# Sangluisme/PSgradientSDF

Hardware: AMD Instinct MI355X
Metric: Gauss-Newton iterations/sec (full PS sweep), 256^3 grid x 50 frames (higher is better)
Workload: dtype f32

## Files before the change

### psgradientsdf_amd/capi.py

```python
from __future__ import annotations

import ctypes as C
import os

import numpy as np

ALBEDO, LIGHT, DIST, POSE, ALL = 1, 2, 4, 8, 15
SH1, SH2, LED = 0, 1, 2
L2, CAUCHY, HUBER, TUKEY, TRUNC_L2 = 0, 1, 2, 3, 4
R_DEPTH, R_NORMAL, R_ALBEDO, R_SHADING, R_RENDERED, R_RESIDUAL, R_VOXEL = 1, 2, 4, 8, 16, 32, 64
R_ALL = 127
_R_PLANES = [("depth", R_DEPTH, 1), ("normal", R_NORMAL, 3), ("albedo", R_ALBEDO, 3), ("shading", R_SHADING, 1),
             ("rendered", R_RENDERED, 3), ("residual", R_RESIDUAL, 3), ("voxel", R_VOXEL, 1)]

_HERE = os.path.dirname(os.path.abspath(__file__))
ENGINE_LIB = os.environ.get("PSGSDF_ENGINE_LIB") or os.path.join(_HERE, "csrc", "libpsgsdf.so")
ENGINE_LIB_DEV = os.path.join(_HERE, "csrc", "libpsgsdf_dev.so")


class GridDesc(C.Structure):
    _fields_ = [("dim", C.c_int32 * 3), ("voxel_size", C.c_float), ("shift", C.c_float * 3), ("truncation", C.c_float)]


class Settings(C.Structure):
# ... 753 lines not shown
        a = np.ascontiguousarray(values, np.float64).copy()
        self._check(self._fn("comm_allreduce_host")(self.ctx, a.ctypes.data_as(C.c_void_p), C.c_int(a.size)), "comm_allreduce_host")
        return a

    def comm_stats(self):
        n = C.c_int64()
        self._check(self._fn("comm_stats")(self.ctx, C.byref(n)), "comm_stats")
        return n.value

    def set_stream(self, stream_ptr):
        self._check(self._fn("set_stream")(self.ctx, C.c_void_p(stream_ptr)), "set_stream")

    def mg_info(self):
        out = (C.c_int32 * 12)()
        self._check(self._fn("mg_info")(self.ctx, out), "mg_info")
        return dict(zip(self._MG_INFO_NAMES, list(out)))

    _MG_INFO_NAMES = ["S", "rows", "row0", "row1", "halo", "F", "rank", "n_ranks", "need_lo", "need_hi", "z0", "z1"]

    def get_tuning(self):
        import json
        f = getattr(self._lib, self._p + "get_tuning"); f.restype = C.c_int
        n = f(self.ctx, None, C.c_size_t(0))
        if n < 0:
            self._check(n, "get_tuning")
        buf = C.create_string_buffer(n + 1)
        f(self.ctx, buf, C.c_size_t(n + 1))
        return json.loads(buf.value.decode())

    def set_profiling(self, on):
        self._check(self._fn("set_profiling")(self.ctx, C.c_int(1 if on else 0)), "set_profiling")

    def watch_kernel(self, name):
        self._check(self._fn("watch_kernel")(self.ctx, name.encode() if name else None), "watch_kernel")

    def reset_kernel_times(self):
        self._check(self._fn("reset_kernel_times")(self.ctx), "reset_kernel_times")

    def kernel_times(self):
        cap = 64
        names = (C.c_char_p * cap)(); ms = (C.c_double * cap)(); n = (C.c_int64 * cap)()
        f = getattr(self._lib, self._p + "kernel_times"); f.restype = C.c_int
        k = f(self.ctx, names, ms, n, C.c_int(cap))
        return {names[i].decode(): (ms[i], n[i]) for i in range(k)}

    def debug_dist_system(self, x=None):
        S = self.info().n_band
        diag = np.empty(S, np.float32); rhs = np.empty(S, np.float32)
        y = np.empty(S, np.float32) if x is not None else None
        xa = np.ascontiguousarray(x, np.float32) if x is not None else None
        self._check(self._fn("debug_dist_system")(self.ctx, diag.ctypes.data_as(C.c_void_p), rhs.ctypes.data_as(C.c_void_p),
                                                   xa.ctypes.data_as(C.c_void_p) if x is not None else None,
                                                   y.ctypes.data_as(C.c_void_p) if x is not None else None), "debug_dist_system")
        return diag, rhs, y

    def debug_time_pcg_pass(self, blocks=0, rows=2, ablate=0, reps=50, stamps=False):
        ms = C.c_double(0)
        st = np.zeros((max(blocks, 1), 8), np.int64) if stamps else None
        self._check(self._fn("debug_time_pcg_pass")(self.ctx, C.c_int(blocks), C.c_int(rows), C.c_int(ablate | (1024 if stamps else 0)), C.c_int(reps), C.byref(ms),
                                                     st.ctypes.data_as(C.c_void_p) if stamps else None), "debug_time_pcg_pass")
        return (ms.value, st) if stamps else ms.value

    def debug_time_pcg_solve(self, passes=16, reps=5):
        ms = C.c_double(0); shape = (C.c_int32 * 2)(); st = (C.c_double * 16)()
        self._check(self._fn("debug_time_pcg_solve")(self.ctx, C.c_int(passes), C.c_int(reps), C.byref(ms), shape, st), "debug_time_pcg_solve")
        return ms.value, (shape[0], shape[1]), [x for x in st]

    def debug_sync_stats(self):
        out = (C.c_int64 * 8)()
        self._check(self._fn("debug_sync_stats")(self.ctx, out), "debug_sync_stats")
        return dict(readbacks_checked=out[0], readbacks_late=out[1], persist_fallbacks=out[2] % 1000000, keyframes_compacted=out[2] // 1000000, speculative_starts=out[3] // 1000000, speculative_undos=out[3] % 1000000,
                    cross_rank_ready=out[4] % 10, halo_pushes=out[4] // 10, cross_rank_solves=out[5], cross_rank_mem_kind=out[6], probe_stale=out[7] // 1000000, probe_timeouts=out[7] % 1000000)

    def debug_rare_rows(self):
        r = C.c_int64(); w = C.c_int64()
        self._check(self._fn("debug_rare_rows")(self.ctx, C.byref(r), C.byref(w)), "debug_rare_rows")
        return r.value, w.value

    def debug_frame_system(self, block):
        i = self.info()
        if block == LIGHT:
            n = i.light_stride; nb = 1 if self._settings.model == LED else i.n_frames
        else:
            n = 6; nb = i.n_frames
        H = np.empty((nb, n, n), np.float64); b = np.empty((nb, n), np.float64)
        self._check(self._fn("debug_frame_system")(self.ctx, C.c_int(block), H.ctypes.data_as(C.c_void_p), b.ctypes.data_as(C.c_void_p)), "debug_frame_system")
        return H, b

    def set_frame_solver(self, mode):
        self._check(self._fn("set_frame_solver")(self.ctx, C.c_int(mode)), "set_frame_solver")

    def frame_solver_stats(self, block):
        it = C.c_int32(); err = C.c_double(); ok = C.c_int32(); ap = C.c_int32()
        self._check(self._fn("get_frame_solver_stats")(self.ctx, C.c_int(block), C.byref(it), C.byref(err), C.byref(ok), C.byref(ap)), "get_frame_solver_stats")
        return {"cg_iters": it.value, "cg_error": err.value, "cg_converged": ok.value, "applied": ap.value}

    def debug_frame_cg(self, H, b, max_it=0):
        H = np.ascontiguousarray(H, np.float32); b = np.ascontiguousarray(b, np.float32)
        nb, n = b.shape
        x = np.empty((nb, n), np.float32); it = C.c_int32(); err = C.c_double(); ok = C.c_int32()
        self._check(self._fn("debug_frame_cg")(self.ctx, C.c_int(nb), C.c_int(n), H.ctypes.data_as(C.c_void_p), b.ctypes.data_as(C.c_void_p), x.ctypes.data_as(C.c_void_p),
                                               C.c_int(max_it), C.byref(it), C.byref(err), C.byref(ok)), "debug_frame_cg")
        return x, it.value, err.value, bool(ok.value)

    def debug_albedo_system(self):
        S = self.info().n_band
        H = np.empty((S, 3), np.float32); b = np.empty((S, 3), np.float32)
        self._check(self._fn("debug_albedo_system")(self.ctx, H.ctypes.data_as(C.c_void_p), b.ctypes.data_as(C.c_void_p)), "debug_albedo_system")
        return H, b


class CommXfer(C.Structure):
    _fields_ = [("ptr_dev", C.c_void_p), ("bytes", C.c_size_t), ("peer", C.c_int)]


ALLREDUCE_FN = C.CFUNCTYPE(C.c_int, C.c_void_p, C.c_void_p, C.c_int, C.c_void_p)
SENDRECV_FN = C.CFUNCTYPE(C.c_int, C.c_void_p, C.POINTER(CommXfer), C.c_int, C.POINTER(CommXfer), C.c_int, C.c_void_p)


class CommOps(C.Structure):
    _fields_ = [("user", C.c_void_p), ("allreduce_f64", ALLREDUCE_FN), ("sendrecv", SENDRECV_FN)]


def comm_unique_id() -> bytes:
    buf = (C.c_uint8 * 128)()
    f = engine_lib().psgsdf_comm_unique_id; f.restype = C.c_int
    rc = f(buf)
    if rc != 0:
        raise PsgsdfError(f"psgsdf_comm_unique_id failed rc={rc} (librccl could not be loaded?)")
    return bytes(buf)


def grid_of(sc) -> GridDesc:
    g = GridDesc()
    g.dim[:] = [int(x) for x in sc.dim]
    g.voxel_size = float(sc.voxel_size)
    g.shift[:] = [float(x) for x in sc.shift]
    g.truncation = float(sc.truncation)
    return g


_engine_lib = {}


def engine_lib(dev: bool = False) -> C.CDLL:
    path = ENGINE_LIB_DEV if dev else ENGINE_LIB
    if path not in _engine_lib:
        if not os.path.exists(path):
            raise PsgsdfError(f"HIP engine {path} is missing: run `python -c 'import __graft_entry__ as g; g.build()'`")
        _engine_lib[path] = C.CDLL(path)
    return _engine_lib[path]


def load_engine(sc_or_grid, K, settings: Settings, device: int = 0, dev: bool = False) -> Api:
    grid = sc_or_grid if isinstance(sc_or_grid, GridDesc) else grid_of(sc_or_grid)
    return Api(engine_lib(dev or os.environ.get("PSGSDF_USE_DEV_LIB") == "1"), "psgsdf_", grid, K, settings, device)
```

### psgradientsdf_amd/csrc/api.hip

```cpp
#include "engine_internal.h"

using namespace psge;

namespace psge {
int host_stage(psgsdf_ctx* c, size_t bytes, void** p) {
    if (c->pin_bytes < bytes) {
        HIPCHK(c, hipStreamSynchronize(c->stream));
        if (c->pin_stage) hipHostFree(c->pin_stage);
        c->pin_stage = nullptr; c->pin_bytes = 0;
        const size_t want = bytes + bytes / 4;
        HIPCHK(c, hipHostMalloc(&c->pin_stage, want, hipHostMallocDefault));
        c->pin_bytes = want;
    }
    *p = c->pin_stage;
    return 0;
}
}

extern "C" {

#ifdef PSGSDF_DEV
const char* psgsdf_version(void) { return "psgsdf-hip gfx950 r5 dev (fault-injection and ablation knobs compiled in: libpsgsdf_dev.so, tests and tools only)"; }
#else
const char* psgsdf_version(void) { return "psgsdf-hip gfx950 r5"; }
#endif

static const char* const kKnobs[] = {
    "PSGSDF_PCG_POLL", "PSGSDF_SPECULATE", "PSGSDF_FOLD_IN_NEXT", "PSGSDF_FUSE_ALBEDO", "PSGSDF_FUSE_PCG_INIT", "PSGSDF_PCG_PERSIST",
    "PSGSDF_PCG_FUSE_APPLY", "PSGSDF_PCG_WINDOW", "PSGSDF_PCG_SOLVE_ROWS", "PSGSDF_PCG_COL16", "PSGSDF_PCG_ROWS", "PSGSDF_PCG_BLOCKS",
    "PSGSDF_FM_SOLVE", "PSGSDF_FRAME_SOLVE", "PSGSDF_FM_ROWS", "PSGSDF_IMG_COMPACT", "PSGSDF_XCD_MAP", "PSGSDF_XCD_STRIPE",
    "PSGSDF_XR", "PSGSDF_XF", "PSGSDF_XS", "PSGSDF_XH", "PSGSDF_XR_MEM", "PSGSDF_XWAIT_LOG2", "PSGSDF_SPECULATE_MR", "PSGSDF_CU_MASK",
    "PSGSDF_WAIT_TIMEOUT_S", "PSGSDF_DESTROY_TIMEOUT_S", "PSGSDF_SOLVE_DUMP", "PSGSDF_AO_CUT", "PSGSDF_COMPARE_CHUNK"};
static const char* const kDevKnobs[] = {"PSGSDF_PCG_ABLATE", "PSGSDF_FAULT_SOLVE", "PSGSDF_FAULT_HALO", "PSGSDF_MBOX_CHECK"};
const char* psgsdf_last_error(const psgsdf_ctx* c) { return c ? c->err : "null context"; }

int psgsdf_create(const psgsdf_grid_desc* grid, const float K[9], const psgsdf_settings* settings, int device, psgsdf_ctx** out) {
    if (!grid || !K || !settings || !out) return PSGSDF_ERR_ARG;
    if (settings->model < 0 || settings->model > 2) return PSGSDF_ERR_ARG;
    int ndev = 0;
    if (hipGetDeviceCount(&ndev) != hipSuccess || ndev <= 0 || device < 0 || device >= ndev) return PSGSDF_ERR_DEVICE;
    if (hipSetDevice(device) != hipSuccess) return PSGSDF_ERR_DEVICE;
    psgsdf_ctx* c = new psgsdf_ctx();
    c->device = device;
    if (const char* e = getenv("PSGSDF_PCG_POLL")) c->pcg_poll = atoi(e) != 0;
    if (const char* e = getenv("PSGSDF_AO_CUT")) c->ao_cut = atoi(e) != 0;
    if (const char* e = getenv("PSGSDF_COMPARE_CHUNK")) c->compare_chunk = std::min(std::max(atoll(e), 1ll), 1ll << 24);
    if (const char* e = getenv("PSGSDF_SPECULATE")) c->speculate = atoi(e) != 0;
    if (const char* e = getenv("PSGSDF_FOLD_IN_NEXT")) c->fold_in_next = atoi(e) != 0;
    if (const char* e = getenv("PSGSDF_FUSE_ALBEDO")) c->fuse_albedo = atoi(e) != 0;
    if (const char* e = getenv("PSGSDF_FUSE_PCG_INIT")) c->fuse_pcg_init = atoi(e) != 0;
    if (const char* e = getenv("PSGSDF_PCG_PERSIST")) c->pcg_persist = atoi(e) != 0;
    if (const char* e = getenv("PSGSDF_AREG_DEVICE")) c->areg_device = atoi(e) != 0;
    if (const char* e = getenv("PSGSDF_PCG_WINDOW")) c->pcg_window = atoi(e) != 0;
    if (const char* e = getenv("PSGSDF_PCG_SOLVE_ROWS")) { const int v = atoi(e); if (v > 0) c->pcg_solve_rows = v; }
    if (const char* e = getenv("PSGSDF_FM_SOLVE")) { c->fm_solve = atoi(e) != 0; c->fm_solve_led = atoi(e) == 1; }
    if (const char* e = getenv("PSGSDF_FRAME_SOLVE")) c->frame_solve = (!strcmp(e, "eigen") || !strcmp(e, "1")) ? 1 : 0;
    if (const char* e = getenv("PSGSDF_XF")) c->xf_enable = atoi(e) != 0;
    if (const char* e = getenv("PSGSDF_XS")) c->xs_enable = atoi(e) != 0;
    if (const char* e = getenv("PSGSDF_XH")) c->xh_enable = atoi(e) != 0;
    if (const char* e = getenv("PSGSDF_XWAIT_LOG2")) { const int l = atoi(e); if (l >= 8 && l <= 30) c->xwait_spins = 1 << l; }
    if (const char* e = getenv("PSGSDF_IMG_COMPACT")) c->img_compact = atoi(e) != 0;
    if (const char* e = getenv("PSGSDF_SPECULATE_MR")) c->speculate_mr = atoi(e) != 0;
    if (const char* e = getenv("PSGSDF_XCD_MAP")) c->xcd_map = atoi(e);
    if (const char* e = getenv("PSGSDF_XCD_STRIPE")) c->xcd_map = (c->xcd_map & 255) | (atoi(e) << 8);
#ifdef PSGSDF_DEV
    if (const char* e = getenv("PSGSDF_PCG_ABLATE")) c->pcg_ablate = atoi(e) & 5;
    if (const char* e = getenv("PSGSDF_MBOX_CHECK")) c->mbox_check = atoi(e) != 0;
    if (const char* e = getenv("PSGSDF_FAULT_SOLVE")) c->fault_solve = atoi(e);
    if (const char* e = getenv("PSGSDF_FAULT_HALO")) c->fault_halo = atoll(e);
#endif
    for (const char* k : kKnobs) if (const char* e = getenv(k)) c->tuning_env.emplace_back(k, e);
    for (const char* k : kDevKnobs) if (const char* e = getenv(k)) {
#ifdef PSGSDF_DEV
        c->tuning_env.emplace_back(k, e);
#else
        c->tuning_ignored.emplace_back(k, e);
#endif
    }
    if (const char* e = getenv("PSGSDF_PCG_FUSE_APPLY")) c->pcg_fuse_apply = atoi(e) != 0;
    if (hipDeviceGetAttribute(&c->num_cu, hipDeviceAttributeMultiprocessorCount, device) != hipSuccess) c->num_cu = 0;
    c->set = *settings; c->reg_n = settings->reg_weight_n; c->reg_l = settings->reg_weight_l; c->reg_r = settings->reg_weight_rho;
    GridP& g = c->grid;
    for (int a = 0; a < 3; ++a) { g.dim[a] = grid->dim[a]; c->shift[a] = grid->shift[a]; }
    g.nvox = (long long)g.dim[0] * g.dim[1] * g.dim[2]; g.koff = 0;
    for (int a = 0; a < 3; ++a) c->gdim[a] = g.dim[a];
    c->gnvox = g.nvox; c->z0 = c->zlo = 0; c->z1 = c->zhi = g.dim[2];
    g.vs = grid->voxel_size; g.vs_inv = 1.f / g.vs; g.T = grid->truncation;
    for (int a = 0; a < 3; ++a) g.origin[a] = c->shift[a] - (float)(0.5 * (double)g.vs) * (float)g.dim[a];
    c->cam.fx = K[0]; c->cam.fy = K[4]; c->cam.cx = K[2]; c->cam.cy = K[5];
    if (const char* e = getenv("PSGSDF_XR")) c->xr_enable = atoi(e) != 0;
    bool stream_ok;
    if (const char* e = getenv("PSGSDF_CU_MASK")) {
        int lo = 0, hi = 0;
        if (sscanf(e, "%d:%d", &lo, &hi) != 2 || lo < 0 || hi <= lo || hi > c->num_cu) { delete c; return PSGSDF_ERR_ARG; }
        std::vector<uint32_t> mask((size_t)(c->num_cu + 31) / 32, 0u);
        for (int i = lo; i < hi; ++i) mask[i / 32] |= 1u << (i % 32);
        stream_ok = hipExtStreamCreateWithCUMask(&c->stream, (uint32_t)mask.size(), mask.data()) == hipSuccess;
        c->cu_mask_lo = lo; c->cu_mask_hi = hi; c->num_cu = hi - lo;
    } else stream_ok = hipStreamCreate(&c->stream) == hipSuccess;
    bool ok = stream_ok
        && hipMalloc(&c->pcg_sc, sizeof(double) * (16 + 8 * (size_t)kPcgMaxBlocks)) == hipSuccess
        && hipMalloc(&c->pcg_part, sizeof(double) * 14 * kPcgMaxBlocks) == hipSuccess
        && hipMalloc(&c->pcg_gran, sizeof(double) * 2 * kSolveGranPlanes * kSolveMaxBlocksHost) == hipSuccess
        && hipMalloc(&c->mg_scal, sizeof(double) * kMgScal) == hipSuccess && hipMalloc(&c->mg_ext, sizeof(double) * 8) == hipSuccess
        && hipMalloc(&c->d_need, 2 * sizeof(int)) == hipSuccess
        && hipMalloc(&c->d_total, sizeof(int)) == hipSuccess
        && hipMalloc(&c->led_light, sizeof(float) * 3) == hipSuccess
        && hipMalloc(&c->fs_stats, sizeof(double) * 8) == hipSuccess && hipMemset(c->fs_stats, 0, sizeof(double) * 8) == hipSuccess
        && hipEventCreate(&c->ev0) == hipSuccess && hipEventCreate(&c->ev1) == hipSuccess;
    if (!ok) { delete c; return PSGSDF_ERR_DEVICE; }
    *out = c;
    return PSGSDF_OK;
}

void psgsdf_destroy(psgsdf_ctx* c) {
    if (!c) return;
    hipSetDevice(c->device);
    if (c->stream) hipStreamSynchronize(c->stream);
    double qt = 15.0; if (const char* e = getenv("PSGSDF_DESTROY_TIMEOUT_S")) qt = atof(e);
    if (xr_quiesce(c, qt)) {
        c->leak_exported = true;
        fprintf(stderr, "psgsdf: rank %d: a peer did not close its mappings of this rank's exchange memory within %.0f s (failed or still running?): that memory is leaked, not freed\n", c->rank, qt);
    }
    free_dense(c);
    hipFree(c->vis_seq); hipFree(c->frame_idx); hipFree(c->img); hipFree(c->img8); hipFree(c->frames); hipFree(c->frames_undo); hipFree(c->led_light); hipFree(c->fs_stats);
    hipFree(c->band_mem); if (!c->leak_exported) hipFree(c->rec_mem); hipFree(c->obs_mem); hipFree(c->stage);
    hipFree(c->ncache); hipFree(c->ntmp); hipFree(c->nout); hipFree(c->ndepth); hipFree(c->track_part); if (c->track_host) hipHostFree(c->track_host); hipFree(c->acc_frame); hipFree(c->frame_part); hipFree(c->frame_done); hipFree(c->part); hipFree(c->pcg_sc); hipFree(c->pcg_part); hipFree(c->pcg_gran); hipFree(c->win_tab); hipFree(c->d_total);
    for (void* p : c->xo_host) if (p) hipHostFree(p);
    if (c->pin_stage) hipHostFree(c->pin_stage);
    if (c->host_buf) hipHostFree(c->host_buf);
    if (c->mbox) hipHostFree(c->mbox);
    if (c->ev0) hipEventDestroy(c->ev0); if (c->ev1) hipEventDestroy(c->ev1);
    for (auto& pr : c->watch_pool) { hipEventDestroy(pr.first); hipEventDestroy(pr.second); }
    if (!c->leak_exported) { hipFree(c->xr); hipFree(c->hx_mem); }
    hipFree(c->xf_table); hipFree(c->vm_order);
    comm_destroy(c);
    hipFree(c->areg_mem); hipFree(c->mg_scal); hipFree(c->mg_ext); hipFree(c->mbox_shadow); hipFree(c->d_need);
    if (c->stream && c->own_stream) hipStreamDestroy(c->stream);
    delete c;
}

static double count_plane(const psgsdf_ctx* c, const float* d, const uint64_t* v, int wpv) {
    const long long plane = (long long)c->gdim[0] * c->gdim[1];
    const float lim = (float)(sqrt(3.0) * (double)c->grid.vs);
    long long m = 0;
    for (long long i = 0; i < plane; ++i) { if (!(fabsf(d[i]) <= lim)) continue; bool seen = false; for (int w = 0; w < wpv && !seen; ++w) seen = v[(size_t)i * wpv + w] != 0; m += seen; }
    return (double)m;
}
static int cut_slabs(psgsdf_ctx* c, std::vector<double>& cnt, int* z0, int* z1) {
    const int nz = c->gdim[2], n = c->n_ranks;
    if (nz < n) return fail(c, PSGSDF_ERR_UNSUPPORTED, "%d z-planes cannot be cut into %d slabs", nz, n);
    if (n > 1) {
        double* d_cnt = nullptr;
        HIPCHK(c, hipMalloc(&d_cnt, sizeof(double) * nz));
        int rc = 0;
        if (hipMemcpyAsync(d_cnt, cnt.data(), sizeof(double) * nz, hipMemcpyHostToDevice, c->stream) != hipSuccess) rc = fail(c, PSGSDF_ERR_DEVICE, "slab histogram upload");
        if (!rc) rc = comm_allreduce(c, d_cnt, nz);
        if (!rc && (hipMemcpyAsync(cnt.data(), d_cnt, sizeof(double) * nz, hipMemcpyDeviceToHost, c->stream) != hipSuccess || hipStreamSynchronize(c->stream) != hipSuccess)) rc = fail(c, PSGSDF_ERR_DEVICE, "slab histogram download");
        hipFree(d_cnt);
        if (rc) return rc;
    }
    double total = 0; for (double x : cnt) total += x;
    if (total <= 0) return fail(c, PSGSDF_ERR_UNSUPPORTED, "the volume has no band candidates to partition");
    std::vector<int> cut(n + 1, 0); cut[n] = nz;
    double run = 0; int r = 1;
    for (int k = 0; k < nz && r < n; ++k) { run += cnt[k]; while (r < n && run >= total * r / n) { cut[r] = k + 1; ++r; } }
    for (int q = 1; q < n; ++q) cut[q] = std::max(cut[q], cut[q - 1] + 1);
    for (int q = n - 1; q >= 1; --q) cut[q] = std::min(cut[q], cut[q + 1] - 1);
    *z0 = cut[c->rank]; *z1 = cut[c->rank + 1];
    return 0;
}
static int choose_slab(psgsdf_ctx* c, const float* dist, const uint64_t* vis_words, int wpv, int* z0, int* z1) {
    const int nz = c->gdim[2], n = c->n_ranks;
    const long long plane = (long long)c->gdim[0] * c->gdim[1];
    std::vector<double> cnt(nz, 0.0);
    for (int k = c->rank; k < nz; k += n) cnt[k] = count_plane(c, dist + (size_t)k * plane, vis_words + (size_t)k * plane * wpv, wpv);
    return cut_slabs(c, cnt, z0, z1);
}

static int upload_planes(psgsdf_ctx* c, int z0, int z1, size_t src_n, size_t src_off, const float* dist, const float* grad_xyz, const float* weight, const float* rgb, const uint64_t* vis_words, int words_per_voxel) {
    { int rc = set_local_grid(c, z0, z1); if (rc) return rc; }
    const long long n = c->grid.nvox;
    free_dense(c);
    if (c->vis_seq) { hipFree(c->vis_seq); c->vis_seq = nullptr; }
    int rc = alloc_dense(c, c->dense, n, 0, true); if (rc) return rc;
    HIPCHK(c, hipMalloc(&c->vis_seq, sizeof(uint64_t) * n * words_per_voxel));
    c->wpv_seq = words_per_voxel;
    HIPCHK(c, hipMemcpyAsync(c->dense.dist, dist + src_off, sizeof(float) * n, hipMemcpyHostToDevice, c->stream));
    for (int a = 0; a < 3; ++a) {
        HIPCHK(c, hipMemcpyAsync(c->dense.g[a], grad_xyz + (size_t)a * src_n + src_off, sizeof(float) * n, hipMemcpyHostToDevice, c->stream));
        HIPCHK(c, hipMemcpyAsync(c->dense.rho[a], rgb + (size_t)a * src_n + src_off, sizeof(float) * n, hipMemcpyHostToDevice, c->stream));
    }
    HIPCHK(c, hipMemcpyAsync(c->dense.weight, weight + src_off, sizeof(float) * n, hipMemcpyHostToDevice, c->stream));
    HIPCHK(c, hipMemcpyAsync(c->vis_seq, vis_words + src_off * words_per_voxel, sizeof(uint64_t) * n * words_per_voxel, hipMemcpyHostToDevice, c->stream));
    HIPCHK(c, hipStreamSynchronize(c->stream));
    c->have_volume = true; c->inited = false;
    return PSGSDF_OK;
}

int psgsdf_upload_volume(psgsdf_ctx* c, const float* dist, const float* grad_xyz, const float* weight, const float* rgb, const uint64_t* vis_words, int words_per_voxel) {
    if (!c || !dist || !grad_xyz || !weight || !rgb || !vis_words || words_per_voxel < 1) return fail(c, PSGSDF_ERR_ARG, "upload_volume: null argument");
    HIPCHK(c, hipSetDevice(c->device));
    int z0 = 0, z1 = c->gdim[2];
    if (c->n_ranks > 1) { int rc = choose_slab(c, dist, vis_words, words_per_voxel, &z0, &z1); if (rc) return rc; }
    const int zlo = std::max(0, z0 - 1);
    return upload_planes(c, z0, z1, (size_t)c->gnvox, (size_t)zlo * c->gdim[0] * c->gdim[1], dist, grad_xyz, weight, rgb, vis_words, words_per_voxel);
}

int psgsdf_slab_plane_count(psgsdf_ctx* c, const float* dist_plane, const uint64_t* vis_plane, int words_per_voxel, double* count) {
    if (!c || !dist_plane || !vis_plane || !count || words_per_voxel < 1) return fail(c, PSGSDF_ERR_ARG, "slab_plane_count: null argument");
    *count = count_plane(c, dist_plane, vis_plane, words_per_voxel);
    return PSGSDF_OK;
}
int psgsdf_plan_slab(psgsdf_ctx* c, const double* plane_counts, int* z0, int* z1) {
    if (!c || !plane_counts || !z0 || !z1) return fail(c, PSGSDF_ERR_ARG, "plan_slab: null argument");
    HIPCHK(c, hipSetDevice(c->device));
    std::vector<double> cnt(plane_counts, plane_counts + c->gdim[2]);
    return cut_slabs(c, cnt, z0, z1);
}
int psgsdf_upload_volume_slab(psgsdf_ctx* c, int z0, int z1, const float* dist, const float* grad_xyz, const float* weight, const float* rgb, const uint64_t* vis_words, int words_per_voxel) {
    if (!c || !dist || !grad_xyz || !weight || !rgb || !vis_words || words_per_voxel < 1) return fail(c, PSGSDF_ERR_ARG, "upload_volume_slab: null argument");
    if (z0 < 0 || z1 > c->gdim[2] || z1 <= z0) return fail(c, PSGSDF_ERR_ARG, "upload_volume_slab: planes [%d, %d) of %d", z0, z1, c->gdim[2]);
    HIPCHK(c, hipSetDevice(c->device));
    const int zlo = std::max(0, z0 - 1), zhi = std::min(c->gdim[2], z1 + 1);
    return upload_planes(c, z0, z1, (size_t)(zhi - zlo) * c->gdim[0] * c->gdim[1], 0, dist, grad_xyz, weight, rgb, vis_words, words_per_voxel);
}

int psgsdf_volume_init(psgsdf_ctx* c, int max_frames) {
    if (!c || max_frames < 1) return fail(c, PSGSDF_ERR_ARG, "volume_init: max_frames");
    if (c->n_ranks > 1 && c->gdim[2] < c->n_ranks) return fail(c, PSGSDF_ERR_UNSUPPORTED, "%d z-planes cannot be cut into %d slabs", c->gdim[2], c->n_ranks);
    { int rc0 = c->n_ranks > 1 ? set_local_grid(c, (int)((long long)c->rank * c->gdim[2] / c->n_ranks), (int)((long long)(c->rank + 1) * c->gdim[2] / c->n_ranks)) : set_local_grid(c, 0, c->gdim[2]); if (rc0) return rc0; }
    HIPCHK(c, hipSetDevice(c->device));
    const long long n = c->grid.nvox;
    free_dense(c);
    if (c->vis_seq) { hipFree(c->vis_seq); c->vis_seq = nullptr; }
    int rc = alloc_dense(c, c->dense, n, 0, true); if (rc) return rc;
    c->wpv_seq = (max_frames + 63) / 64;
    HIPCHK(c, hipMalloc(&c->vis_seq, sizeof(uint64_t) * n * c->wpv_seq));
    launch_fill_f32(c->dense.dist, c->grid.T, n, c->stream);
    for (int a = 0; a < 3; ++a) { HIPCHK(c, hipMemsetAsync(c->dense.g[a], 0, sizeof(float) * n, c->stream)); HIPCHK(c, hipMemsetAsync(c->dense.rho[a], 0, sizeof(float) * n, c->stream)); }
    HIPCHK(c, hipMemsetAsync(c->dense.weight, 0, sizeof(float) * n, c->stream));
    HIPCHK(c, hipMemsetAsync(c->vis_seq, 0, sizeof(uint64_t) * n * c->wpv_seq, c->stream));
    HIPCHK(c, hipStreamSynchronize(c->stream));
    c->have_volume = true; c->inited = false;
    return PSGSDF_OK;
}

int psgsdf_rebalance_slabs(psgsdf_ctx* c) {
    if (!c || !c->have_volume || !c->vis_seq) return fail(c, PSGSDF_ERR_STATE, "rebalance_slabs: volume first");
    if (c->n_ranks <= 1) return PSGSDF_OK;
    if (!c->comm) return fail(c, PSGSDF_ERR_COMM, "rank %d of %d has no communicator (psgsdf_comm_init)", c->rank, c->n_ranks);
    HIPCHK(c, hipSetDevice(c->device));
    const int R = c->n_ranks, nz = c->gdim[2], wpv = c->wpv_seq;
    const size_t plane = (size_t)c->gdim[0] * c->gdim[1];
    const int oz0 = c->z0, oz1 = c->z1, ozlo = c->zlo;
    std::vector<float> hd((size_t)(oz1 - oz0) * plane); std::vector<uint64_t> hv((size_t)(oz1 - oz0) * plane * wpv);
    HIPCHK(c, hipMemcpyAsync(hd.data(), c->dense.dist + (size_t)(oz0 - ozlo) * plane, sizeof(float) * hd.size(), hipMemcpyDeviceToHost, c->stream));
    HIPCHK(c, hipMemcpyAsync(hv.data(), c->vis_seq + (size_t)(oz0 - ozlo) * plane * wpv, sizeof(uint64_t) * hv.size(), hipMemcpyDeviceToHost, c->stream));
    HIPCHK(c, hipStreamSynchronize(c->stream));
    std::vector<double> cnt(nz, 0.0);
    for (int k = oz0; k < oz1; ++k) cnt[k] = count_plane(c, hd.data() + (size_t)(k - oz0) * plane, hv.data() + (size_t)(k - oz0) * plane * wpv, wpv);
    int nz0 = 0, nz1 = nz;
    { int rc = cut_slabs(c, cnt, &nz0, &nz1); if (rc) return rc; }
    std::vector<double> cuts((size_t)4 * R, 0.0);
    cuts[4 * c->rank] = oz0; cuts[4 * c->rank + 1] = oz1; cuts[4 * c->rank + 2] = nz0; cuts[4 * c->rank + 3] = nz1;
    { int rc = host_allreduce(c, cuts, "rebalance_slabs"); if (rc) return rc; }
    DenseView od = c->dense; uint64_t* ovis = c->vis_seq;
    const int nzlo = std::max(0, nz0 - 1), nzhi = std::min(nz, nz1 + 1);
    const long long n = (long long)(nzhi - nzlo) * (long long)plane;
    DenseView nd{};
    uint64_t* nvis = nullptr;
    auto free_new = [&] { hipFree(nd.dist); for (int a = 0; a < 3; ++a) { hipFree(nd.g[a]); hipFree(nd.rho[a]); } hipFree(nd.weight); hipFree(nd.vis); hipFree(nd.row_of); hipFree(nvis); (void)hipGetLastError(); };
    int rc = alloc_dense(c, nd, n, 0, true);
    if (!rc && hipMalloc(&nvis, sizeof(uint64_t) * n * wpv) != hipSuccess) rc = fail(c, PSGSDF_ERR_DEVICE, "rebalance_slabs: out of memory");
    if (rc) { free_new(); return rc; }
    { int rc2 = set_local_grid(c, nz0, nz1); if (rc2) { free_new(); set_local_grid(c, oz0, oz1); return rc2; } }
    c->dense = DenseView{}; c->vis_seq = nullptr;
    float* oarr[8] = {od.dist, od.g[0], od.g[1], od.g[2], od.rho[0], od.rho[1], od.rho[2], od.weight};
    float* narr[8] = {nd.dist, nd.g[0], nd.g[1], nd.g[2], nd.rho[0], nd.rho[1], nd.rho[2], nd.weight};
    std::vector<psgsdf_comm_xfer> sends, recvs;
// ... 362 lines not shown
```

### psgradientsdf_amd/csrc/api_debug.hip

```cpp
#include "engine_internal.h"

using namespace psge;

extern "C" {
int psgsdf_set_profiling(psgsdf_ctx* c, int enabled) { if (!c) return PSGSDF_ERR_ARG; c->profiling = enabled != 0; return PSGSDF_OK; }
int psgsdf_reset_kernel_times(psgsdf_ctx* c) { if (!c) return PSGSDF_ERR_ARG; c->ktimes.clear(); c->watch_used = 0; return PSGSDF_OK; }
int psgsdf_watch_kernel(psgsdf_ctx* c, const char* name) {
    if (!c) return PSGSDF_ERR_ARG;
    hipStreamSynchronize(c->stream);
    std::string w = name ? name : ""; int every = 1;
    const size_t sl = w.find('/');
    if (sl != std::string::npos) { every = std::max(1, atoi(w.c_str() + sl + 1)); w.resize(sl); }
    c->watch = w; c->watch_every = every; c->watch_seen = 0; c->watch_used = 0;
    return PSGSDF_OK;
}
int psgsdf_kernel_times(psgsdf_ctx* c, const char** names, double* ms, int64_t* launches, int cap) {
    if (!c) return 0;
    if (c->watch_used) {
        hipStreamSynchronize(c->stream);
        KTime& k = c->ktimes[c->watch];
        for (size_t i = 0; i < c->watch_used; ++i) { float t = 0; if (hipEventElapsedTime(&t, c->watch_pool[i].first, c->watch_pool[i].second) == hipSuccess) { k.ms += t; k.n += 1; } }
        c->watch_used = 0;
    }
    int n = 0;
// ... 28 lines not shown
    int G, rdef; cgf_shape(band_blocks(c), &G, &rdef);
    if (blocks > 0) G = std::min(blocks, kCgfMaxBlocks);
    if (rows <= 0) rows = rdef;
    launch_cgf_init(a, c->pcg_sc, c->pcg_part, G, c->stream);
    hipEvent_t e0, e1; HIPCHK(c, hipEventCreate(&e0)); HIPCHK(c, hipEventCreate(&e1));
    for (int q = 0; q < 3; ++q) launch_cgf_pass(a, c->pcg_sc, c->pcg_part, G, rows, q, 1 << 30, c->mbox_dev, c->stream, ablate | 16);
    HIPCHK(c, hipEventRecord(e0, c->stream));
    for (int q = 0; q < reps; ++q) launch_cgf_pass(a, c->pcg_sc, c->pcg_part, G, rows, 3 + q, 1 << 30, c->mbox_dev, c->stream, ablate | 16);
    HIPCHK(c, hipEventRecord(e1, c->stream));
    HIPCHK(c, hipStreamSynchronize(c->stream));
    float ms = 0; HIPCHK(c, hipEventElapsedTime(&ms, e0, e1));
    hipEventDestroy(e0); hipEventDestroy(e1);
    *avg_ms = (double)ms / reps;
    if (stamps) {
        HIPCHK(c, hipMemcpy(stamps, c->pcg_sc + 16, sizeof(long long) * 8 * G, hipMemcpyDeviceToHost));
    }
    return PSGSDF_OK;
}

int psgsdf_debug_time_pcg_solve(psgsdf_ctx* c, int passes, int reps, double* ms_per_launch, int32_t* shape, double* stamps ) {
    if (!c || !c->inited || !ms_per_launch || !shape || (passes < 1 && passes != -7) || reps < 1) return fail(c, PSGSDF_ERR_STATE, "init first");
    HIPCHK(c, hipSetDevice(c->device));
    int G = 0, rows = 0;
    if (!cgf_solve_shape(c, &G, &rows)) return fail(c, PSGSDF_ERR_UNSUPPORTED, "the persistent solve does not apply to this context");
    shape[0] = G; shape[1] = rows;
    SweepArgs a = make_args(c, c->reg_l != 0.f);
    a.pcg_fuse_init = 1; a.pcg_init_blocks = band_blocks(c); a.pcg_gran = c->pcg_gran; a.pcg_gran_n = 2 * kSolveGranPlanes * kSolveMaxBlocksHost; a.pcg_asm = 1;
    hipEvent_t e0, e1; HIPCHK(c, hipEventCreate(&e0)); HIPCHK(c, hipEventCreate(&e1));
    float total = 0;
    for (int r = 0; r < reps + 1; ++r) {
        launch_sweep_dist(a, c->stream);
        launch_assemble(a, c->stream);
        HIPCHK(c, hipEventRecord(e0, c->stream));
        a.pcg_epoch = ++c->pcg_solve_serial;
        launch_cgf_solve(a, c->pcg_sc, c->pcg_gran, G, rows, 1 << 30, c->mbox_dev, 0ull, passes, c->stream);
        HIPCHK(c, hipEventRecord(e1, c->stream));
        HIPCHK(c, hipStreamSynchronize(c->stream));
        float ms = 0; HIPCHK(c, hipEventElapsedTime(&ms, e0, e1));
        if (r > 0) total += ms;
        if (c->mbox[3] != 1.0) { hipEventDestroy(e0); hipEventDestroy(e1); return fail(c, PSGSDF_ERR_DEVICE, "persistent solve status %g: a workgroup gave up waiting for the others", c->mbox[3]); }
    }
    hipEventDestroy(e0); hipEventDestroy(e1);
    *ms_per_launch = (double)total / reps;
    if (stamps) for (int i = 0; i < 16; ++i) stamps[i] = c->mbox[8 + i];
    if (const char* dump = getenv("PSGSDF_SOLVE_DUMP")) {
        std::vector<double> h(8 * 256);
        HIPCHK(c, hipMemcpy(h.data(), c->pcg_sc + 16, sizeof(double) * h.size(), hipMemcpyDeviceToHost));
        if (FILE* f = fopen(dump, "w")) { for (int i = 0; i < G; ++i) fprintf(f, "%d %.0f %.0f %.0f %.0f %.0f %.0f %.0f %.0f\n", i, h[i], h[256 + i], h[512 + i], h[768 + i], h[1024 + i], h[1280 + i], h[1536 + i], h[1792 + i]); fclose(f); }
    }
    return PSGSDF_OK;
}

int psgsdf_debug_overlap_probe(psgsdf_ctx* c, int reps, double* out) {
    if (!c || !c->inited || !out || reps < 1) return fail(c, PSGSDF_ERR_STATE, "init first");
    if (c->n_ranks > 1) return fail(c, PSGSDF_ERR_UNSUPPORTED, "overlap probe: one rank");
    HIPCHK(c, hipSetDevice(c->device));
    int G = 0, rows = 0;
    if (!cgf_solve_shape(c, &G, &rows)) return fail(c, PSGSDF_ERR_UNSUPPORTED, "the persistent solve does not apply to this context");
    { int rc = flush(c); if (rc) return rc; }
    SweepArgs a = make_args(c, c->reg_l != 0.f);
    a.pcg_fuse_init = 1; a.pcg_init_blocks = band_blocks(c); a.pcg_gran = c->pcg_gran; a.pcg_gran_n = 2 * kSolveGranPlanes * kSolveMaxBlocksHost; a.pcg_asm = 1;
    SweepArgs quiet = a; quiet.pcg_gran = nullptr; quiet.pcg_gran_n = 0;
    hipStream_t s2; HIPCHK(c, hipStreamCreateWithFlags(&s2, hipStreamNonBlocking));
    hipEvent_t e[4]; for (auto& x : e) HIPCHK(c, hipEventCreate(&x));
    double acc[4] = {0, 0, 0, 0};
    int rc = PSGSDF_OK;
    auto ms = [&](hipEvent_t x, hipEvent_t y) { float t = 0; hipEventElapsedTime(&t, x, y); return (double)t; };
    auto solve = [&](hipStream_t s) { a.pcg_epoch = ++c->pcg_solve_serial; launch_cgf_solve(a, c->pcg_sc, c->pcg_gran, G, rows, 1 << 30, c->mbox_dev, 0ull, 0, s); };
    for (int r = 0; r < reps + 1 && !rc; ++r) {
        hipEventRecord(e[0], c->stream); launch_sweep_dist(a, c->stream); hipEventRecord(e[1], c->stream);
        hipStreamSynchronize(c->stream);
        hipEventRecord(e[2], c->stream); solve(c->stream); hipEventRecord(e[3], c->stream);
        hipStreamSynchronize(c->stream);
        if (c->mbox[3] != 1.0) { rc = fail(c, PSGSDF_ERR_DEVICE, "overlap probe: solve status %g", c->mbox[3]); break; }
        if (r) { acc[0] += ms(e[0], e[1]); acc[1] += ms(e[2], e[3]); }
        hipEventRecord(e[0], c->stream); launch_sweep_dist(a, c->stream); solve(c->stream); hipEventRecord(e[1], c->stream);
        hipStreamSynchronize(c->stream);
        if (r) acc[2] += ms(e[0], e[1]);
        launch_sweep_dist(a, c->stream);
        hipEventRecord(e[0], c->stream); hipStreamWaitEvent(s2, e[0], 0);
        launch_sweep_dist(quiet, c->stream); hipEventRecord(e[1], c->stream);
        solve(s2); hipEventRecord(e[2], s2);
        hipStreamSynchronize(c->stream); hipStreamSynchronize(s2);
        if (c->mbox[3] != 1.0) { rc = fail(c, PSGSDF_ERR_DEVICE, "overlap probe (side by side): solve status %g", c->mbox[3]); break; }
        if (r) acc[3] += std::max(ms(e[0], e[1]), ms(e[0], e[2]));
    }
    for (auto& x : e) hipEventDestroy(x);
    hipStreamDestroy(s2);
    for (int i = 0; i < 4; ++i) out[i] = acc[i] / reps;
    return rc;
}

int psgsdf_debug_rare_rows(psgsdf_ctx* c, int64_t* rows, int64_t* waves) {
    if (!c || !c->inited || !rows || !waves) return fail(c, PSGSDF_ERR_STATE, "init first");
    HIPCHK(c, hipSetDevice(c->device));
    SweepArgs a = make_args(c, c->reg_l != 0.f);
    launch_sweep_dist(a, c->stream);
    launch_assemble(a, c->stream);
    std::vector<int> hx(c->band.S);
    HIPCHK(c, hipMemcpyAsync(hx.data(), c->band.hx, sizeof(int) * hx.size(), hipMemcpyDeviceToHost, c->stream));
    HIPCHK(c, hipStreamSynchronize(c->stream));
    *rows = 0; *waves = 0;
    for (size_t i = 0; i < hx.size(); i += 64) { bool any = false; for (size_t k = i; k < std::min(hx.size(), i + 64); ++k) if (hx[k]) { ++*rows; any = true; } *waves += any; }
    return PSGSDF_OK;
}

int psgsdf_set_frame_solver(psgsdf_ctx* c, int mode) {
    if (!c) return PSGSDF_ERR_ARG;
    if (mode != 0 && mode != 1) return fail(c, PSGSDF_ERR_ARG, "frame solver mode %d (0 = LDL^T per frame, 1 = the reference's global float Jacobi-PCG)", mode);
    c->frame_solve = mode;
    return PSGSDF_OK;
}
int psgsdf_get_frame_solver_stats(psgsdf_ctx* c, int block, int32_t* iterations, double* error, int32_t* converged, int32_t* applied) {
    if (!c) return PSGSDF_ERR_ARG;
    if (block != PSGSDF_LIGHT && block != PSGSDF_POSE) return fail(c, PSGSDF_ERR_ARG, "block must be LIGHT or POSE");
    HIPCHK(c, hipSetDevice(c->device));
    const int kind = block == PSGSDF_POSE ? 1 : 0;
    psgsdf_step_stats st; memset(&st, 0, sizeof(st));
    if (int rc = read_frame_solver_stats(c, kind, &st)) return rc;
    if (iterations) *iterations = st.cg_iters;
    if (error) *error = st.cg_error;
    if (converged) *converged = st.cg_converged;
    if (applied) *applied = st.applied;
    return PSGSDF_OK;
}
int psgsdf_debug_frame_cg(psgsdf_ctx* c, int nb, int n, const float* H, const float* b, float* x, int max_it, int32_t* iterations, double* error, int32_t* converged) {
    if (!c || !H || !b || !x || nb <= 0) return fail(c, PSGSDF_ERR_ARG, "null argument");
    if ((n != 3 && n != 4 && n != 6 && n != 9) || (long long)nb * n > 2048) return fail(c, PSGSDF_ERR_UNSUPPORTED, "block size %d x %d blocks", n, nb);
    HIPCHK(c, hipSetDevice(c->device));
    float *dH = nullptr, *db = nullptr, *dx = nullptr; double* ds = nullptr;
    const size_t nH = (size_t)nb * n * n, nv = (size_t)nb * n;
    int rc = PSGSDF_OK;
    if (hipMalloc(&dH, sizeof(float) * nH) != hipSuccess || hipMalloc(&db, sizeof(float) * nv) != hipSuccess || hipMalloc(&dx, sizeof(float) * nv) != hipSuccess || hipMalloc(&ds, sizeof(double) * 4) != hipSuccess)
        rc = fail(c, PSGSDF_ERR_DEVICE, "out of device memory");
    double st[4] = {0, 0, 0, 0};
    if (!rc && (hipMemcpy(dH, H, sizeof(float) * nH, hipMemcpyHostToDevice) != hipSuccess || hipMemcpy(db, b, sizeof(float) * nv, hipMemcpyHostToDevice) != hipSuccess)) rc = fail(c, PSGSDF_ERR_DEVICE, "upload failed");
    if (!rc && launch_frames_eigen_raw(nb, n, dH, db, dx, ds, max_it, c->stream)) rc = fail(c, PSGSDF_ERR_UNSUPPORTED, "shape");
    if (!rc && (hipStreamSynchronize(c->stream) != hipSuccess || hipMemcpy(x, dx, sizeof(float) * nv, hipMemcpyDeviceToHost) != hipSuccess || hipMemcpy(st, ds, sizeof(st), hipMemcpyDeviceToHost) != hipSuccess))
        rc = fail(c, PSGSDF_ERR_DEVICE, "%s", hipGetErrorString(hipGetLastError()));
    hipFree(dH); hipFree(db); hipFree(dx); hipFree(ds);
    if (rc) return rc;
    if (iterations) *iterations = (int32_t)st[0];
    if (error) *error = st[1];
    if (converged) *converged = (int32_t)st[2];
    return PSGSDF_OK;
}
int psgsdf_debug_frame_system(psgsdf_ctx* c, int block, double* H, double* b) {
    if (!c || !c->inited || !H || !b) return fail(c, PSGSDF_ERR_STATE, "init first");
    HIPCHK(c, hipSetDevice(c->device));
    SweepArgs a = make_args(c, 0);
    const bool led = c->set.model == PSGSDF_LED;
    int n, nb, nh;
    int launched = 0;
    if (block == PSGSDF_LIGHT) { launched = launch_sweep_light(a, c->stream); n = led ? 3 : (c->set.model == PSGSDF_SH2 ? 9 : 4); nb = led ? 1 : c->F; nh = led ? 3 : n * (n + 1) / 2; }
    else if (block == PSGSDF_POSE) { launched = launch_sweep_pose(a, c->stream); n = 6; nb = c->F; nh = 21; }
    else return fail(c, PSGSDF_ERR_ARG, "block must be LIGHT or POSE");
    if (!launched) HIPCHK(c, hipMemsetAsync(c->acc_frame, 0, sizeof(double) * c->acc_frame_n, c->stream));
    std::vector<double> acc(c->acc_frame_n);
    HIPCHK(c, hipMemcpyAsync(acc.data(), c->acc_frame, sizeof(double) * c->acc_frame_n, hipMemcpyDeviceToHost, c->stream));
    HIPCHK(c, hipStreamSynchronize(c->stream));
    if (led && block == PSGSDF_LIGHT) {
        for (int i = 0; i < 9; ++i) H[i] = 0;
        for (int i = 0; i < 3; ++i) { b[i] = 0; for (int f = 0; f < c->F; ++f) { H[i * 3 + i] += acc[(size_t)f * kFrameRow + i]; b[i] += acc[(size_t)f * kFrameRow + 3 + i]; } }
        return PSGSDF_OK;
    }
    for (int k = 0; k < nb; ++k) {
        const double* A = acc.data() + (size_t)k * kFrameRow;
        double* Hk = H + (size_t)k * n * n; double* bk = b + (size_t)k * n;
        for (int i = 0; i < n * n; ++i) Hk[i] = 0;
        int q = 0;
        for (int i = 0; i < n; ++i) for (int j = i; j < n; ++j) { Hk[i * n + j] = A[q]; Hk[j * n + i] = A[q]; ++q; }
        for (int i = 0; i < n; ++i) bk[i] = A[nh + i];
    }
    return PSGSDF_OK;
}

int psgsdf_debug_albedo_system(psgsdf_ctx* c, float* H, float* b) {
    if (!c || !c->inited || !H || !b) return fail(c, PSGSDF_ERR_STATE, "init first");
    HIPCHK(c, hipSetDevice(c->device));
    SweepArgs a = make_args(c, 0);
    launch_sweep_albedo(a, c->stream);
    const int S = c->band.S, Sp = c->band.Spad;
    std::vector<float> h(3 * (size_t)Sp), bb(3 * (size_t)Sp);
    HIPCHK(c, hipMemcpyAsync(h.data(), c->band.aH, sizeof(float) * 3 * Sp, hipMemcpyDeviceToHost, c->stream));
    HIPCHK(c, hipMemcpyAsync(bb.data(), c->band.ab, sizeof(float) * 3 * Sp, hipMemcpyDeviceToHost, c->stream));
    HIPCHK(c, hipStreamSynchronize(c->stream));
    for (int j = 0; j < S; ++j) for (int ch = 0; ch < 3; ++ch) { H[3 * j + ch] = h[(size_t)ch * Sp + j]; b[3 * j + ch] = bb[(size_t)ch * Sp + j]; }
    return PSGSDF_OK;
}

int psgsdf_debug_sync_stats(psgsdf_ctx* c, int64_t out[8]) {
    if (!c || !out) return PSGSDF_ERR_ARG;
    out[0] = c->mbox_checked; out[1] = c->mbox_late; out[2] = c->persist_fallbacks + (c->img_compacted ? 1000000LL : 0); out[3] = c->spec_windows * 1000000LL + c->spec_undos;
    out[4] = (c->xr_ready ? 1 : 0) + 10 * c->n_halo_pushes; out[5] = c->xr_solves; out[6] = c->xr_mem_kind; out[7] = c->xr_probe_stale * 1000000LL + c->xr_probe_timeouts;
    return PSGSDF_OK;
}

int psgsdf_get_tuning(psgsdf_ctx* c, char* json, size_t cap) {
    if (!c) return PSGSDF_ERR_ARG;
    std::string o = "{\"build\": \"";
    o += psgsdf_version(); o += "\", \"env\": {";
    auto esc = [](const std::string& v) { std::string r; for (char ch : v) { if (ch == '"' || ch == '\\') r += '\\'; if ((unsigned char)ch >= 0x20) r += ch; } return r; };
    bool first = true;
    for (auto& kv : c->tuning_env) { o += (first ? "\"" : ", \"") + kv.first + "\": \"" + esc(kv.second) + "\""; first = false; }
    o += "}, \"ignored_dev_only\": {"; first = true;
    for (auto& kv : c->tuning_ignored) { o += (first ? "\"" : ", \"") + kv.first + "\": \"" + esc(kv.second) + "\""; first = false; }
    o += "}, \"effective\": {";
    char buf[1024];
    snprintf(buf, sizeof(buf), "\"pcg_poll\": %d, \"speculate\": %d, \"speculate_mr\": %d, \"fold_in_next\": %d, \"fuse_albedo\": %d, \"fuse_pcg_init\": %d, \"pcg_persist\": %d, "
             "\"pcg_fuse_apply\": %d, \"fm_solve\": %d, \"fm_solve_led\": %d, \"frame_solve\": \"%s\", \"img_compact\": %d, \"xcd_map\": %d, "
             "\"xr\": %d, \"xf\": %d, \"xs\": %d, \"xh\": %d, \"xr_mem_kind\": %d, \"xwait_log2\": %d, \"cu_mask\": [%d, %d], \"mbox_check\": %d, \"pcg_ablate\": %d, \"fault_solve\": %d, \"fault_halo\": %lld, \"ao_cut\": %d, \"compare_chunk\": %lld",
             (int)c->pcg_poll, (int)c->speculate, (int)c->speculate_mr, (int)c->fold_in_next, (int)c->fuse_albedo, (int)c->fuse_pcg_init, (int)c->pcg_persist,
             (int)c->pcg_fuse_apply, (int)c->fm_solve, (int)c->fm_solve_led, c->frame_solve == 1 ? "eigen" : "ldlt", (int)c->img_compact, c->xcd_map,
             (int)c->xr_enable, (int)c->xf_enable, (int)c->xs_enable, (int)c->xh_enable, c->xr_mem_kind, (int)lround(log2((double)c->xwait_spins)), c->cu_mask_lo, c->cu_mask_hi,
             (int)c->mbox_check, c->pcg_ablate, c->fault_solve, c->fault_halo, (int)c->ao_cut, c->compare_chunk);
    o += buf;
    {
        int Gs = 0, Rs = 0;
        const bool shape = cgf_solve_shape(c, &Gs, &Rs);
        const int budget = (shape && c->n_ranks <= 1) ? cgf_solve_window_budget(Rs) : 0;
        const char* why = !c->pcg_window ? "" : c->n_ranks > 1 ? "multi-rank" : c->pcg_ablate ? "timing ablation" : !c->inited ? "no band yet"
                          : !shape ? "no persistent solve on this band" : (c->win_G != Gs || c->win_rows != Rs) ? "no table for this partition" : c->win_max > budget ? "window does not fit" : "";
        snprintf(buf, sizeof(buf), ", \"pcg_window\": %d, \"pcg_solve_rows\": %d, \"solve_window\": {\"workgroups\": %d, \"rows_per_workgroup\": %d, \"window_doubles\": %d, \"budget_doubles\": %d, \"fits\": %d, \"fallback\": \"%s\", \"last_solve_windowed\": %d}",
                 (int)c->pcg_window, c->pcg_solve_rows, shape ? Gs : 0, shape ? Rs : 0, c->win_max, budget, (int)(c->pcg_window && !*why), why, c->last_solve_windowed);
        o += buf;
    }
    o += "}";
    snprintf(buf, sizeof(buf), ", \"last_compare\": {\"queries\": [%lld, %lld], \"pairs\": [%lld, %lld]}", c->cmp_queries[0], c->cmp_queries[1], c->cmp_pairs[0], c->cmp_pairs[1]);
    o += buf;
    snprintf(buf, sizeof(buf), ", \"last_align\": {\"iterations\": %lld, \"evaluations\": %lld, \"queries\": [%lld, %lld], \"pairs\": [%lld, %lld]}", c->aln_iters, c->aln_evals, c->aln_queries[0], c->aln_queries[1],
             c->aln_pairs[0], c->aln_pairs[1]);
    o += buf;
    if (c->n_ranks > 1) {
        snprintf(buf, sizeof(buf), ", \"xr_probe\": {\"rank\": %d, \"n_ranks\": %d, \"kind_chosen\": %d, \"stale_mappings\": %lld, \"fine_grained\": {\"tried\": %lld, \"stale_records_from_lower\": %lld, \"expired_waits_lower\": %lld, \"expired_waits_upper\": %lld}, "
                 "\"uncached\": {\"tried\": %lld, \"stale_records_from_lower\": %lld, \"expired_waits_lower\": %lld, \"expired_waits_upper\": %lld}}",
                 c->rank, c->n_ranks, c->xr_mem_kind, c->xr_stale_maps, c->xr_probe_local[1][3], c->xr_probe_local[1][0], c->xr_probe_local[1][1], c->xr_probe_local[1][2],
                 c->xr_probe_local[2][3], c->xr_probe_local[2][0], c->xr_probe_local[2][1], c->xr_probe_local[2][2]);
        o += buf;
    }
    o += "}";
    if (json && cap) { const size_t n = std::min(cap - 1, o.size()); memcpy(json, o.data(), n); json[n] = 0; }
    return (int)o.size();
}

}
```

### psgradientsdf_amd/csrc/device_common.h

```cpp
#pragma once
#include "engine.h"
#include <float.h>

#ifndef PSG_STRICT
#define PSG_STRICT 0
#endif
#if PSG_STRICT & 1
#pragma clang fp contract(off)
#else
#pragma clang fp contract(fast)
#endif

namespace psg {
#if PSG_STRICT & 8
typedef double obs_acc_t;
#else
typedef float obs_acc_t;
#endif

typedef float f2_t __attribute__((ext_vector_type(2)));
__device__ __forceinline__ float dot3(const float* a, const float* b) { return (a[0] * b[0] + a[1] * b[1]) + a[2] * b[2]; }
__device__ __forceinline__ float norm3(const float* a) { return sqrtf(dot3(a, a)); }
__device__ __forceinline__ void normalized3(const float* v, float* o) {
#pragma clang fp contract(off)
// ... 37 lines not shown
            else hipLaunchKernelGGL((K<2, -1, -1>), grid, block, shmem, stream, __VA_ARGS__); \
        } } while (0)
template <int LOSS = -1>
__device__ __forceinline__ float robust_weight(const Robust& rb, float r) {
#if PSG_STRICT & 2
    switch (LOSS >= 0 ? LOSS : rb.loss) {
        case 1: { float x = r / rb.lambda; return 1.0f / (1.0f + x * x); }
        case 3: { float x = r / rb.lambda; float w = (1.0f - x * x); w = w * w; return (r * r < rb.lambda_sq) ? w : 0.0f; }
        case 2: { float w = rb.lambda * fabsf(1.0f / r); return (r * r < rb.lambda_sq) ? 1.0f : w; }
        case 4: return (r * r < rb.lambda_sq) ? 1.0f : 0.0f;
        default: return 1.0f;
    }
#endif
    switch (LOSS >= 0 ? LOSS : rb.loss) {
        case 1: { float x = r * rb.inv_lambda; return __builtin_amdgcn_rcpf(1.0f + x * x); }
        case 3: { float x = r * rb.inv_lambda; float w = (1.0f - x * x); w = w * w; return (r * r < rb.lambda_sq) ? w : 0.0f; }
        case 2: { float w = rb.lambda * fabsf(__builtin_amdgcn_rcpf(r)); return (r * r < rb.lambda_sq) ? 1.0f : w; }
        case 4: return (r * r < rb.lambda_sq) ? 1.0f : 0.0f;
        default: return 1.0f;
    }
}
template <int LOSS = -1>
__device__ __forceinline__ float robust_loss(const Robust& rb, float r) {
#if PSG_STRICT & 2
    switch (LOSS >= 0 ? LOSS : rb.loss) {
        case 1: { float x = r / rb.lambda; return logf(1.0f + x * x); }
        case 3: { float x = r / rb.lambda; float u = 1.0f - x * x; float v = 1.0f - u * u * u; return (r * r < rb.lambda_sq) ? v : 1.0f; }
        case 2: return (r * r < rb.lambda_sq) ? 0.5f * (r * r) : rb.lambda * (fabsf(r) - 0.5f * rb.lambda * 1.0f);
        case 4: { float x = fminf(fmaxf(r, -rb.lambda), rb.lambda); return x * x; }
        default: return r * r;
    }
#endif
    switch (LOSS >= 0 ? LOSS : rb.loss) {
        case 1: { float x = r * rb.inv_lambda; return __builtin_amdgcn_logf(1.0f + x * x) * 0.693147180559945f; }
        case 3: { float x = r * rb.inv_lambda; float u = 1.0f - x * x; float v = 1.0f - u * u * u; return (r * r < rb.lambda_sq) ? v : 1.0f; }
        case 2: return (r * r < rb.lambda_sq) ? 0.5f * (r * r) : rb.lambda * (fabsf(r) - 0.5f * rb.lambda * 1.0f);
        case 4: { float x = fminf(fmaxf(r, -rb.lambda), rb.lambda); return x * x; }
        default: return r * r;
    }
}

constexpr int kCgfSums = 7;
__device__ __forceinline__ double* fpart(double* part, int k, int kind) { return part + ((size_t)((k & 1) * kCgfSums + kind)) * kPcgMaxBlocks; }

template <int CTRL, int ROW_MASK>
__device__ __forceinline__ double dpp_add(double v) {
    const int lo = __builtin_amdgcn_update_dpp(0, __double2loint(v), CTRL, ROW_MASK, 0xf, false);
    const int hi = __builtin_amdgcn_update_dpp(0, __double2hiint(v), CTRL, ROW_MASK, 0xf, false);
    return v + __hiloint2double(hi, lo);
}
__device__ __forceinline__ double wave_sum(double v) {
    v = dpp_add<0xB1, 0xf>(v);
    v = dpp_add<0x4E, 0xf>(v);
    v = dpp_add<0x141, 0xf>(v);
    v = dpp_add<0x140, 0xf>(v);
    v = dpp_add<0x142, 0xa>(v);
    v = dpp_add<0x143, 0xc>(v);
    return __hiloint2double(__builtin_amdgcn_readlane(__double2hiint(v), 63), __builtin_amdgcn_readlane(__double2loint(v), 63));
}
template <int CTRL>
__device__ __forceinline__ double dpp_get(double v) {
    const int lo = __builtin_amdgcn_update_dpp(0, __double2loint(v), CTRL, 0xf, 0xf, false);
    const int hi = __builtin_amdgcn_update_dpp(0, __double2hiint(v), CTRL, 0xf, 0xf, false);
    return __hiloint2double(hi, lo);
}
__device__ __forceinline__ void wave_sum8(const double (&v)[8], double& t0, double& t1) {
    const int lane = threadIdx.x & 63;
    const bool b0 = lane & 1, b1 = lane & 2;
    double u[4], t[2];
#pragma unroll
    for (int j = 0; j < 4; ++j) { const double keep = b0 ? v[4 + j] : v[j], give = b0 ? v[j] : v[4 + j]; u[j] = keep + dpp_get<0xB1>(give); }
#pragma unroll
    for (int j = 0; j < 2; ++j) { const double keep = b1 ? u[2 + j] : u[j], give = b1 ? u[j] : u[2 + j]; t[j] = keep + dpp_get<0x4E>(give); }
#pragma unroll
    for (int j = 0; j < 2; ++j) {
        t[j] += dpp_get<0x124>(t[j]);
        t[j] += dpp_get<0x128>(t[j]);
        t[j] += __shfl_xor(t[j], 16, 64);
        t[j] += __shfl_xor(t[j], 32, 64);
    }
    t0 = t[0]; t1 = t[1];
}
__device__ __forceinline__ double wave_sum4(const double (&v)[4]) {
    const int lane = threadIdx.x & 63;
    const bool b0 = lane & 1, b1 = lane & 2;
    double u[2];
#pragma unroll
    for (int j = 0; j < 2; ++j) { const double keep = b0 ? v[2 + j] : v[j], give = b0 ? v[j] : v[2 + j]; u[j] = keep + dpp_get<0xB1>(give); }
    const double keep = b1 ? u[1] : u[0], give = b1 ? u[0] : u[1];
    double t = keep + dpp_get<0x4E>(give);
    t += dpp_get<0x124>(t);
    t += dpp_get<0x128>(t);
    t += __shfl_xor(t, 16, 64);
    t += __shfl_xor(t, 32, 64);
    return t;
}
template <int NW>
__device__ __forceinline__ void wave_sum4_store(double t, double* red, int w) {
    const int lane = threadIdx.x & 63;
    if (lane < 4) red[(2 * (lane & 1) + ((lane >> 1) & 1)) * NW + w] = t;
}
template <int NW>
__device__ __forceinline__ void wave_sum8_store(double t0, double t1, double* red, int w) {
    const int lane = threadIdx.x & 63;
    if (lane < 4) { const int base = 4 * (lane & 1) + (lane & 2); red[base * NW + w] = t0; red[(base + 1) * NW + w] = t1; }
}
template <int NV, class T>
__device__ __forceinline__ void wave_sums_to(const T* acc, double* row) {
    const int lane = threadIdx.x & 63;
#pragma unroll
    for (int g = 0; g < (NV + 7) / 8; ++g) {
        double v[8];
#pragma unroll
        for (int q = 0; q < 8; ++q) v[q] = 8 * g + q < NV ? (double)acc[8 * g + q] : 0.0;
        double t0, t1; wave_sum8(v, t0, t1);
        const int k = 8 * g + 4 * (lane & 1) + (lane & 2);
        if (lane < 4) { if (k < NV) row[k] = t0; if (k + 1 < NV) row[k + 1] = t1; }
    }
}
__device__ __forceinline__ float wave_sumf(float v) {
#pragma unroll
    for (int o = 32; o > 0; o >>= 1) v += __shfl_down(v, o, 64);
    return v;
}
__device__ __forceinline__ void block_part_store(double v, double* part_slot, double* red, int bid = -1) {
    v = wave_sum(v);
    int lane = threadIdx.x & 63, w = threadIdx.x >> 6;
    __syncthreads();
    if (lane == 0) red[w] = v;
    __syncthreads();
    if (threadIdx.x == 0) {
        double s = 0;
        for (int i = 0; i < (int)(blockDim.x >> 6); ++i) s += red[i];
        part_slot[bid >= 0 ? bid : (int)blockIdx.x] = s;
    }
}
template <int NT = 0>
__device__ __forceinline__ double block_total(const double* part, int n, double* red) {
    double v = 0;
    if (!NT || threadIdx.x < NT) for (int i = threadIdx.x; i < n; i += NT ? NT : blockDim.x) v += part[i];
    v = wave_sum(v);
    int lane = threadIdx.x & 63, w = threadIdx.x >> 6;
    __syncthreads();
    if (lane == 0 && (!NT || w < NT / 64)) red[w] = v;
    __syncthreads();
    double s = 0;
    for (int i = 0; i < (int)((NT ? NT : blockDim.x) >> 6); ++i) s += red[i];
    return s;
}
__device__ __forceinline__ unsigned xcd_remap(unsigned pid, unsigned G) {
    const unsigned x = pid & 7u, s = pid >> 3, q = G >> 3, rem = G & 7u;
    return x * q + (x < rem ? x : rem) + s;
}
__device__ __forceinline__ void fm_ids(const SweepArgs& a, int& cx, int& f) {
    cx = blockIdx.x; f = blockIdx.y;
    if (a.xcd_map & 1) {
        const unsigned L = xcd_remap(blockIdx.x + gridDim.x * blockIdx.y, gridDim.x * gridDim.y);
        cx = (int)(L / gridDim.y); f = (int)(L - (unsigned)cx * gridDim.y);
    }
}
__device__ __forceinline__ unsigned xcd_remap_striped(unsigned pid, unsigned G, unsigned T) {
    const unsigned Gc = G / (8u * T) * (8u * T);
    if (pid >= Gc) return pid;
    const unsigned x = pid & 7u, s = pid >> 3;
    return ((s / T) * 8u + x) * T + s % T;
}
__device__ __forceinline__ int vm_bid(const SweepArgs& a, int bit = 2, bool per_obs = false) {
    if (bit == 4 && (a.xcd_map & 32) && a.vm_order) return a.vm_order[blockIdx.x];
    if (per_obs && (a.xcd_map & 64) && a.vm_order) return a.vm_order[blockIdx.x];
    if (!(a.xcd_map & bit)) return (int)blockIdx.x;
    const unsigned T = (unsigned)a.xcd_map >> 8;
    return T ? (int)xcd_remap_striped(blockIdx.x, gridDim.x, T) : (int)xcd_remap(blockIdx.x, gridDim.x);
}
#define PART(a, slot) ((a).acc.part + (size_t)(slot) * (a).acc.PB)
__device__ __forceinline__ void mbox_put(double* out, int n, int i, double v, unsigned long long key) {
    out[i] = v;
    if (key) reinterpret_cast<unsigned long long*>(out)[n + i] = (unsigned long long)__double_as_longlong(v) ^ (key + (unsigned long long)i);
}
__device__ __forceinline__ void mbox_commit(unsigned long long key) { if (key) __threadfence_system(); }
__device__ __forceinline__ void store8_system(double* p, double v) { asm volatile("global_store_dwordx2 %0, %1, off sc0 sc1\n\ts_nop 1" :: "v"(p), "v"(v) : "memory"); }
__device__ __forceinline__ void fold_exchange(const XfTable* xf, long long epoch, int n, double* t) {
    const XfTable& x = *xf;
    const int Rk = x.n_ranks, buf = (int)(epoch & 1), lane = (int)(threadIdx.x & 63);
    const double tag = (double)epoch;
    const long long slot = (long long)buf * Rk + x.rank;
    double* const mine = x.region[x.rank];
    for (int s = 0; s < n; ++s) t[s] = __shfl(t[s], 0, 64);
    if (lane == 0) {
        for (int r = 0; r < Rk; ++r) for (int s = 0; s < n; ++s) store8_system(x.region[r] + x.spay + slot * 8 + s, t[s]);
        asm volatile("s_waitcnt vmcnt(0)" ::: "memory");
        for (int r = 0; r < Rk; ++r) __hip_atomic_store(x.region[r] + x.sflg + slot, tag, __ATOMIC_RELAXED, __HIP_MEMORY_SCOPE_SYSTEM);
    }
    bool late = false;
    if (lane < Rk) {
        int spins = 0;
        while (__hip_atomic_load(mine + x.sflg + (long long)buf * Rk + lane, __ATOMIC_RELAXED, __HIP_MEMORY_SCOPE_SYSTEM) != tag) { __builtin_amdgcn_s_sleep(2); if (++spins > x.spin_max) { late = true; break; } }
    }
    const bool any_late = __builtin_amdgcn_ballot_w64(late) != 0ull;
    __builtin_amdgcn_fence(__ATOMIC_ACQUIRE, "");
    for (int s = 0; s < n; ++s) {
        const double v = lane < Rk ? __hip_atomic_load(mine + x.spay + ((long long)buf * Rk + lane) * 8 + s, __ATOMIC_RELAXED, __HIP_MEMORY_SCOPE_SYSTEM) : 0.0;
        double tot = 0.0;
        for (int r = 0; r < Rk; ++r) tot += __shfl(v, r, 64);
        t[s] = any_late ? __builtin_nan("") : tot;
    }
    if (any_late && lane == 0) __hip_atomic_store(mine + kXrLate + 1, tag, __ATOMIC_RELAXED, __HIP_MEMORY_SCOPE_SYSTEM);
}
template <int NT = 0>
__device__ __forceinline__ void fold_pending(const SweepArgs& a, double* red ) {
    if (a.fold.n == 0 || blockIdx.x != 0 || blockIdx.y != 0) return;
    double t[4];
    for (int s = 0; s < a.fold.n; ++s) t[s] = block_total<NT>(PART(a, a.fold.id[s]), a.fold.nblk, red);
    if (threadIdx.x < 64) {
        if (a.fold.xf) fold_exchange(a.fold.xf, a.fold.xf_epoch, a.fold.n, t);
        if (threadIdx.x == 0) {
            for (int s = 0; s < a.fold.n; ++s) mbox_put(a.fold.out, a.fold.n, s, t[s], a.fold.key);
            mbox_commit(a.fold.key);
        }
    }
    __syncthreads();
}

extern __shared__ __align__(16) unsigned char psg_dyn_smem[];
__device__ __forceinline__ const FrameP& frame_at(const FrameP* sf, int f) {
    return *reinterpret_cast<const FrameP*>(reinterpret_cast<const char*>(sf) + __umul24((unsigned)f, (unsigned)sizeof(FrameP)));
}
__device__ __forceinline__ void load_frames(FrameP* sf, const FrameP* frames, int F) {
    const float* src = (const float*)frames; float* dst = (float*)sf;
    for (int i = threadIdx.x; i < F * (int)(sizeof(FrameP) / 4); i += blockDim.x) dst[i] = src[i];
    __syncthreads();
}

struct Proj { float p[3]; float m, n, z_inv; bool ok; };
__device__ __forceinline__ float div_by(float a, float b, float y) { const float q0 = a * y; return __builtin_fmaf(__builtin_fmaf(-q0, b, a), y, q0); }
struct ProjJ { float mj, nj; bool ok; };
__device__ __forceinline__ ProjJ project_jac(const Proj& pr, const Cam& cam) {
#pragma clang fp contract(off)
    ProjJ o;
    o.mj = div_by(cam.fx * pr.p[0], pr.p[2], pr.z_inv) + cam.cx;
    o.nj = div_by(cam.fy * pr.p[1], pr.p[2], pr.z_inv) + cam.cy;
    o.ok = (o.mj >= 0.f && o.mj < (float)cam.W && o.nj >= 0.f && o.nj < (float)cam.H);
    return o;
}

__device__ __forceinline__ Proj project(const float* xs, const FrameP& fp, const Cam& cam) {
#pragma clang fp contract(off)
    Proj o;
    float tmp[3] = {xs[0] - fp.t[0], xs[1] - fp.t[1], xs[2] - fp.t[2]};
#pragma unroll
    for (int i = 0; i < 3; ++i) o.p[i] = (fp.R[0 * 3 + i] * tmp[0] + fp.R[1 * 3 + i] * tmp[1]) + fp.R[2 * 3 + i] * tmp[2];
#if PSG_STRICT & 4
    const float z_inv = (float)(1.0 / (double)o.p[2]);
#else
    const float z_inv = 1.0f / o.p[2];
#endif
    o.z_inv = z_inv;
    o.m = cam.fx * o.p[0] * z_inv + cam.cx;
    o.n = cam.fy * o.p[1] * z_inv + cam.cy;
    o.ok = (o.m >= 0.f && o.m < (float)cam.W && o.n >= 0.f && o.n < (float)cam.H);
    return o;
}

__device__ __forceinline__ const float* pix(const float* img, const Cam& cam, int row, int col) {
    row = row < 0 ? 0 : (row >= cam.H ? cam.H - 1 : row);
    col = col < 0 ? 0 : (col >= cam.W ? cam.W - 1 : col);
    return img + ((size_t)row * cam.W + col) * 3;
}

template <bool GRAD>
__device__ __forceinline__ void interp_taps(const float* a00, const float* a01, const float* a10, const float* a11, float fm, float fn, float gm, float gn, float* I, float* gu, float* gv,
                                            float m = 0.f, float n = 0.f, int x = 0, int y = 0) {
#if PSG_STRICT & 4
    {
#pragma clang fp contract(off)
        const double w1 = ((double)y + 1.0 - (double)n) * (double)(m - (float)x);
        const double w2 = ((double)y + 1.0 - (double)n) * ((double)x + 1.0 - (double)m);
        const float w3 = (n - (float)y) * (m - (float)x);
        const double w4 = (double)(n - (float)y) * ((double)x + 1.0 - (double)m);
#pragma unroll
        for (int ch = 0; ch < 3; ++ch) {
            const float t1 = (float)((double)a10[ch] * w1), t2 = (float)((double)a00[ch] * w2), t3 = a11[ch] * w3, t4 = (float)((double)a01[ch] * w4);
            I[ch] = ((t1 + t2) + t3) + t4;
        }
    }
#else
    const float w1 = (1.0f - fn) * fm, w2 = (1.0f - fn) * (1.0f - fm), w3 = fn * fm, w4 = fn * (1.0f - fm);
#pragma unroll
    for (int ch = 0; ch < 3; ++ch) I[ch] = ((a10[ch] * w1 + a00[ch] * w2) + a11[ch] * w3) + a01[ch] * w4;
#endif
    if (GRAD) {
        const float w01 = gm, w11 = gn, w00 = 1.0f - gm, w10 = 1.0f - gn;
#pragma unroll
        for (int ch = 0; ch < 3; ++ch) {
            gu[ch] = w00 * (a01[ch] - a00[ch]) + w01 * (a11[ch] - a10[ch]);
            gv[ch] = w10 * (a10[ch] - a00[ch]) + w11 * (a11[ch] - a01[ch]);
        }
    }
}
template <bool GRAD, class TEX>
__device__ __forceinline__ void sample_border(const TEX& tex, const Cam& cam, int x, int y, float m, float n, float* I, float* gu, float* gv) {
    float p[3]; tex(x, y, p);
    I[0] = p[0]; I[1] = p[1]; I[2] = p[2];
    if (GRAD) {
        float w01 = m - (float)x, w11 = n - (float)y;
        float w00 = (float)(1.0 - (double)w01), w10 = (float)(1.0 - (double)w11);
        float q_y1[3], q_ym[3], q_x1ym[3], q_x1[3], q_xm[3], q_xmy1[3];
        tex(x, y + 1, q_y1); tex(x, y - 1, q_ym); tex(x + 1, y - 1, q_x1ym); tex(x + 1, y, q_x1); tex(x - 1, y, q_xm); tex(x - 1, y + 1, q_xmy1);
#pragma unroll
        for (int ch = 0; ch < 3; ++ch) {
            if ((x + 1) >= cam.H) gu[ch] = q_y1[ch] - p[ch];
            else { float v0 = -q_ym[ch] + p[ch]; float v1 = -q_x1ym[ch] + q_x1[ch]; gu[ch] = w00 * v0 + w01 * v1; }
            if ((x + 1) >= cam.H && (y + 1) < cam.W) { float v0 = -q_xm[ch] + p[ch]; float v1 = -q_xmy1[ch] + q_y1[ch]; gv[ch] = w10 * v0 + w11 * v1; }
// ... 338 lines not shown
```

### psgradientsdf_amd/csrc/engine.h

```cpp
#pragma once
#include <hip/hip_runtime.h>
#include <stdint.h>

namespace psg {

constexpr int kBlock = 256;
constexpr int kMaxFramesLds = 640;
constexpr int kNQ = 19;
constexpr int kNQCommon = 13;
constexpr int kMaxBasis = 9;

struct FrameP {
    float R[9];
    float t[3];
    float l[9];
    float pad[3];
};

struct Cam { float fx, fy, cx, cy; int W, H; };

struct GridP {
    int dim[3];
    long long nvox;
    float vs, vs_inv;
    float origin[3];
    float T;
    int koff;
};

struct Robust { int loss; float lambda, lambda_sq, inv_lambda; };

struct Band {
    int S, Spad, KW;
    int* lin;
    float* dist;
    float* g[3];
    float* rho[3];
    uint64_t* vis;
    int* nb;
    int* dirb;
    float* nbd;
    int* col;
    unsigned* colp;
    int col16;
    int reach;
    float* gfd[3];
    float4* vp[3];
    float* aH; float* ab;
    float* blk;
    float* H;
    int* hx;
    float* rhs; float* x; float* t;
    float4* rec[2];
    int* obs_ptr;
    int* obs_rows;
    int obs_max;
    long long obs_ptr_total;
};

struct Accum {
    double* frame;
    double* part;
    int PB;
    double* fpart;
    int fcap;
    int* fdone;
};
constexpr int kFrameRow = 64;
constexpr int kPcgMaxBlocks = 2048;
constexpr int kCgfMaxBlocks = 768;

enum { SC_ENERGY = 0, SC_NOBS = 1, SC_EN = 2, SC_EL = 3, SC_ACCEPT = 4, SC_AUX0 = 5, SC_AUX1 = 6, SC_AUX2 = 7, SC_COUNT = 8 };

struct AlbedoReg {
    int* anb;
    int* back;
    float* anrho;
    float* J;
    float* res;
    float* rhs; float* diag; float* diag0; float* x; float* r; float* p; float* q; float* t;
    double* cgs;
    float weight;
};

struct XfTable;
struct FoldReq { int n; int id[4]; int nblk; double* out; unsigned long long key; const XfTable* xf; long long xf_epoch; };

struct ImgSrc {
    const float* f32;
    const unsigned* u8; float scale;
    bool idx32;
};

struct SweepArgs {
    Band b;
    const FrameP* frames;
    ImgSrc im;
    int F;
    Cam cam;
    GridP grid;
    Robust rob;
    Accum acc;
    int model;
    int quirks;
    float reg_n, reg_l;
    int normal_reg, laplacian_reg;
    float damping;
    int row0, row1;
    FoldReq fold;
    AlbedoReg ar;
    double* pcg_part; double* pcg_fs;
    int pcg_asm;
    unsigned pcg_epoch;
    int pcg_ablate;
    int pcg_apply;
    double* pcg_gran; int pcg_gran_n;
    const int* pcg_win;
    int pcg_win_G, pcg_win_rows, pcg_win_max;
    int pcg_fuse_init;
    int pcg_init_blocks;
    int fuse_apply;
    const int* vm_order;
    float* fm_led_light;
    const XfTable* xf;
    long long xf_epoch;
    int xcd_map;
    int fm_solve;
    FrameP* fm_frames; float* fm_undo; double* fm_e_out; unsigned long long fm_e_key;
    const double* gate;
    const double* ext;
};

constexpr int kXrMaxRanks = 32;
constexpr int kXrRankGran = 0, kXrAbort = 2 * 8 * kXrMaxRanks, kXrDoubles = kXrAbort + 8;
constexpr int kXrLate = kXrAbort + 1;
constexpr int kXrNonce = kXrAbort + 7;
struct XrArgs {
    int rank, n_ranks;
    double* region[kXrMaxRanks];
    float4* lo_rec[2]; float4* hi_rec[2];
    float4* lo_base[2];
    int give_lo, give_hi;
    int need_lo, need_hi;
    unsigned epoch;
};
struct XfTable {
    int n_ranks, rank, F, spin_max;
    long long pay, flg;
    long long spay, sflg;
    double* region[32];
};
constexpr int kHxWords = 16;
constexpr unsigned kXrEpochMask = 0x3fffu;

constexpr int kTryPackFlags = 2048;
void launch_normals_cache(int W, int H, int r, double fx_inv, double fy_inv, double cx, double cy, double* work , float* out , hipStream_t s);
void launch_try_pack_f32(const float* rgb, unsigned* rgba, size_t npix, size_t stride, float scale, int* fail , hipStream_t s);
void launch_pack_rgb8(const uint8_t* rgb, unsigned* rgba, size_t npix, hipStream_t s);
void launch_select_vis(const uint64_t* vis_seq, int wpv_seq, uint64_t* vis_key, int KW, const int* frame_idx, int F, long long nvox, hipStream_t s);
void launch_band_flags(const float* dist, const uint64_t* vis_key, int KW, float vs, long long nvox, int* flags, hipStream_t s);
void launch_band_scan(int* flags_inout_rowof, long long nvox, int* block_sums, int* d_total, hipStream_t s);
struct DenseView { float* dist; float* g[3]; float* weight; float* rho[3]; uint64_t* vis; int KW; int* row_of; };
void launch_band_fill(const DenseView& d, const GridP& grid, Band b, int* d_reach, hipStream_t s);
void launch_band_scatter(const DenseView& d, Band b, hipStream_t s);
void launch_derive(const SweepArgs& a, int update_grad, hipStream_t s);
constexpr int kObsChunk = 2048;
void launch_obs_count(const Band& b, int F, int row0, int row1, int* counts, hipStream_t s);
void launch_block_work(const Band& b, int row0, int row1, int* work, hipStream_t s);
void launch_obs_fill(const Band& b, int F, int row0, int row1, const int* offsets, hipStream_t s);
void launch_lower_bound(const int* lin, int S, int target, int* out, hipStream_t s);
struct SlotList { int n; int id[8]; };
void launch_sum_parts(const double* part, int PB, int nblk, const SlotList& slots, double* out, unsigned long long key, hipStream_t s, const XfTable* xf = nullptr, long long xf_epoch = 0);
void launch_frame_cols(const double* frame, int F, int col, double* out, unsigned long long key, hipStream_t s);
void launch_zero_f64(double* p, int n, hipStream_t s);
struct CopySegs { int n; unsigned off[16]; unsigned len[16]; unsigned long long key[16]; };
void launch_copy_segs(const double* src, double* dst, const CopySegs& segs, hipStream_t s);
void launch_marker(double* p, double v, hipStream_t s);
void launch_init_albedo(const SweepArgs& a, hipStream_t s);
void launch_led_light_init(const SweepArgs& a, hipStream_t s);
void launch_energy(const SweepArgs& a, hipStream_t s);
void launch_sweep_albedo(const SweepArgs& a, hipStream_t s);
void launch_apply_albedo(const SweepArgs& a, hipStream_t s);
void launch_restore_albedo(const SweepArgs& a, hipStream_t s);
int launch_sweep_light(const SweepArgs& a, hipStream_t s);
int launch_sweep_pose(const SweepArgs& a, hipStream_t s);
void launch_solve_light(const SweepArgs& a, FrameP* frames, float* led_light, double* e_out, unsigned long long e_key, float* undo, hipStream_t s);
void launch_restore_light(int F, FrameP* frames, float* led_light, const float* undo, hipStream_t s);
void launch_solve_pose(const SweepArgs& a, FrameP* frames, double* e_out, unsigned long long e_key, hipStream_t s);
bool frames_eigen_fits(int model, int F);
void launch_frames_eigen_light(const SweepArgs& a, FrameP* frames, float* led_light, double* e_out, unsigned long long e_key, float* undo, double* stats, hipStream_t s);
void launch_frames_eigen_pose(const SweepArgs& a, FrameP* frames, double* e_out, unsigned long long e_key, double* stats, hipStream_t s);
int launch_frames_eigen_raw(int nb, int n, const float* H, const float* b, float* x, double* stats, int max_it, hipStream_t s);
void launch_sweep_dist(const SweepArgs& a, hipStream_t s);
void launch_assemble(const SweepArgs& a, hipStream_t s);
void launch_cgf_init(const SweepArgs& a, double* fs, double* part, int G, hipStream_t s);
void launch_cgf_pass(const SweepArgs& a, double* fs, double* part, int G, int rows, int k, int kmax, double* mb, hipStream_t s, int ablate = 0);
void launch_cgf_sum(double* part, int G, int k, double* out, hipStream_t s);
constexpr int kSolveGranPlanes = 8;
constexpr int kSolveThreadsHost = 512, kSolveMaxBlocksHost = 256, kSolveMaxRowsHost = 4, kSolveMbSlots = 24;
int cgf_solve_max_blocks(int rows);
void launch_solve_windows(const Band& b, int row0, int row1, int G, int rows_per_wg, int* tab , int* max_total, hipStream_t s);
int cgf_solve_window_budget(int rows_per_wg);
int launch_cgf_solve(const SweepArgs& a, double* fs, double* gran, int G, int rows_per_wg, int kmax, double* mb, unsigned long long mb_key, int force_passes, hipStream_t s, const XrArgs* xr = nullptr);
void launch_areg_tables(const DenseView& d, const GridP& g, const SweepArgs& a, hipStream_t s);
void launch_areg_build(const SweepArgs& a, hipStream_t s);
void launch_areg_system(const SweepArgs& a, hipStream_t s);
void launch_areg_jx(const SweepArgs& a, const float* p, float* t, hipStream_t s);
void launch_areg_jt(const SweepArgs& a, const float* p, const float* t, float* q, hipStream_t s);
void launch_areg_cg_init(const SweepArgs& a, hipStream_t s);
void launch_areg_cg_iteration(const SweepArgs& a, int i, int nblk, float thr, hipStream_t s);
void launch_areg_cg_update(const SweepArgs& a, float alpha, hipStream_t s);
void launch_areg_cg_dir(const SweepArgs& a, float beta, hipStream_t s);
void launch_apply_albedo_delta(const SweepArgs& a, const float* delta, hipStream_t s);
void launch_matvec(const SweepArgs& a, const float* x, float* y, hipStream_t s);
void launch_apply_dist(const SweepArgs& a, hipStream_t s);
void launch_upsample(const DenseView& src, const DenseView& dst, const GridP& g_old, hipStream_t s);
void launch_fill_f32(float* p, float v, long long n, hipStream_t s);
void launch_normals(const float* depth, const float* cache, int W, int H, int r, double* tmp, float* out, hipStream_t s);
void launch_track(const DenseView& d, const GridP& g, const Cam& cam, const FrameP& fp, const float* depth, float z_min, float z_max, double* part, int nblk, int gdimz, int zown0, int zown1, hipStream_t s);
void launch_integrate(const DenseView& d, uint64_t* vis_seq, int wpv_seq, const GridP& g, const Cam& cam, const FrameP& fp,
                      const float* rgb, const float* depth, const float* normals, int counter, float z_min, float z_max, hipStream_t s);

constexpr int kRenderBrick = 8;
constexpr int kRenderTile = 8;
constexpr int kRenderStats = 9;
enum { RP_DEPTH = 0, RP_NORMAL, RP_ALBEDO, RP_SHADING, RP_RENDERED, RP_RESIDUAL, RP_VOXEL, RP_COUNT };
enum { RF_DEPTH = 0, RF_NORMAL = 1, RF_ALBEDO = 4, RF_SHADING = 7, RF_RENDERED = 8, RF_VOXEL = 11, RF_OFF_BAND = 12, RF_COUNT = 13 };
struct RenderArgs {
    DenseView d;
    const float4* vp[3];
    GridP grid;
    const FrameP* frames;
    ImgSrc im; int img_w, img_h;
    Robust rob;
    const unsigned char* bricks;
    const int* bbox;
    int nb[3];
    Cam cam;
    int frame;
    int light_frame;
    FrameP pose;
    int tiles_x, tiles_y;
    float* planes[RP_COUNT];
    double* part;
    int zr[2];
    int slab;
    int f0;
    double* mask;
    unsigned char* mine;
    double* rec;
    long long rec_px;
    int rf[RF_COUNT];
    int n_rf;
};
void launch_render_bricks(const DenseView& d, const GridP& g, float thr, int z0, int z1, unsigned char* bricks, int* bbox, double* marks, hipStream_t s);
void launch_render_box(const double* marks, const int* nb, unsigned char* bricks, int* bbox, hipStream_t s);
void launch_render(const RenderArgs& a, int model, hipStream_t s);
void launch_render_report(const RenderArgs& a, int model, int F, hipStream_t s);
void launch_render_fold(const double* part, int tiles, int F, double* out , hipStream_t s);
void launch_render_ranks(const RenderArgs& a, int model, bool report, int chunk, hipStream_t s);
void launch_render_keep(const RenderArgs& a, hipStream_t s);
void launch_render_composite(const RenderArgs& a, bool report, int chunk, hipStream_t s);

struct WMeshGrid {
    const float* dist; const float* weight; const float* g[3]; const float* rho[3];
    const float* hg[3]; const float* hrho[3];
    int nx, ny, zlo, zh;
    int lo[3], d[3];
    int zc0;
    long long nown;
    float voxel[3], origin[3];
    int poff[3];
};
void launch_wmesh_mark(const WMeshGrid& g, long long ncell, int* cnt, int* flag, hipStream_t s);
void launch_wmesh_or(int* dst, const int* src, long long n, hipStream_t s);
void launch_wmesh_faces(const WMeshGrid& g, long long ncell, const int* offs, int n_faces, const int* num, int first, const int* num_up, int first_up, int* faces, hipStream_t s);
void launch_wmesh_verts(const WMeshGrid& g, const int* num, int n_verts, float* xyz, float* nrm, unsigned char* rgb, hipStream_t s);

void launch_band_fit(const SweepArgs& a, int* n_obs, double* loss, float* sum_r2, hipStream_t s);
void launch_wmesh_fit(const WMeshGrid& g, const int* num, int n_verts, const int* row_of, int row0, int row1, const int* n_obs, const double* loss, const float* sum_r2,
                      int* v_n, float* v_rms, float* v_loss, hipStream_t s);

enum { MC_FIRST = 0, MC_VERTS, MC_FACES, MC_EDGES, MC_BOUNDARY, MC_NONMANIFOLD, MC_AREA, kMcompStats = 8 };
void launch_mcomp_init(int* parent, int nv, hipStream_t s);
void launch_mcomp_hook(const int* faces, int nf, int* parent, hipStream_t s);
void launch_mcomp_flatten(int* parent, int nv, int* flag, hipStream_t s);
void launch_mcomp_vstats(const int* parent, const int* num, int nv, const float* xyz, int* vcomp, long long* stat, unsigned* blo, unsigned* bhi, hipStream_t s);
void launch_mcomp_fstats(const int* faces, int nf, const int* vcomp, const float* xyz, double vs2 , long long* stat, hipStream_t s);
void launch_mcomp_edges(const int* faces, int nf, unsigned long long* keys, int* uses, unsigned long long cap, hipStream_t s);
void launch_mcomp_ecount(const unsigned long long* keys, const int* uses, unsigned long long cap, const int* vcomp, long long* stat, hipStream_t s);
void launch_mcomp_keep(const int* kept, const int* vcomp, int nv, const int* faces, int nf, int* vflag, int* fflag, hipStream_t s);
void launch_mcomp_compact(const int* kept, const int* vcomp, int nv, const int* faces, int nf, const int* vnum, const int* fnum, const float* xyz, const float* nrm,
                          const unsigned char* rgb, float* oxyz, float* onrm, unsigned char* orgb, int* ovcomp, int* ofaces, hipStream_t s);


}
```

### psgradientsdf_amd/csrc/engine.hip

```cpp
#include "engine_internal.h"
#include <chrono>
#include <sched.h>

namespace psge {

int wait_mapped(psgsdf_ctx* c, const std::function<bool()>& ready, const char* what) {
    using clk = std::chrono::steady_clock;
    static const double limit_s = [] { const char* e = getenv("PSGSDF_WAIT_TIMEOUT_S"); double v = e ? atof(e) : 0.0; return v > 0.0 ? v : 120.0; }();
    clk::time_point t0{}, next_query{};
    bool timing = false;
    for (unsigned spin = 1;; ++spin) {
        if (ready()) return 0;
        if (spin & 0x3ffu) continue;
        const clk::time_point now = clk::now();
        if (!timing) { timing = true; t0 = now; next_query = now + std::chrono::milliseconds(20); continue; }
        if (now - t0 > std::chrono::milliseconds(2)) sched_yield();
        if (now < next_query) continue;
        next_query = now + std::chrono::milliseconds(20);
        const hipError_t q = hipStreamQuery(c->stream);
        if (q == hipSuccess) return ready() ? 0 : 1;
        if (q != hipErrorNotReady) return fail(c, PSGSDF_ERR_DEVICE, "%s: stream error while waiting: %s", what, hipGetErrorString(q));
        if (std::chrono::duration<double>(now - t0).count() > limit_s)
            return fail(c, PSGSDF_ERR_DEVICE, "%s: nothing published within %.0f s (PSGSDF_WAIT_TIMEOUT_S)", what, limit_s);
    }
// ... 152 lines not shown
    const long long ep = xs ? ++c->xs_epoch : 0;
    if (n <= 4 && c->fold_in_next) {
        c->pending_fold.n = n; for (int i = 0; i < n; ++i) c->pending_fold.id[i] = slots[i];
        c->pending_fold.nblk = band_blocks(c); c->pending_fold.out = dst; c->pending_fold.key = dkey; c->pending_fold.xf = xf; c->pending_fold.xf_epoch = ep;
    } else {
        SlotList sl; sl.n = n; for (int i = 0; i < n; ++i) sl.id[i] = slots[i];
        launch_sum_parts(c->part, c->PB, band_blocks(c), sl, dst, dkey, c->stream, xf, ep);
    }
    if (xs) c->deferred.push_back({c->mbox + off, n, key, [c, consume](const double* v) { if (std::isnan(v[0])) c->xf_timeout = true; consume(v); }});
    else c->deferred.push_back({c->mbox + off, n, key, std::move(consume)});
    return 0;
}
int read_frame_energy_deferred(psgsdf_ctx* c, int col_e, std::function<void(double, double)> consume) {
    size_t off; unsigned long long key;
    { int rc = mbox_reserve(c, 2, &off, &key); if (rc) return rc; }
    launch_frame_cols(c->acc_frame, c->F, col_e, c->mbox_dev + off, key, c->stream);
    c->deferred.push_back({c->mbox + off, 2, key, [consume](const double* v) { consume(v[0], v[1]); }});
    return 0;
}
int reserve_frame_energy_deferred(psgsdf_ctx* c, std::function<void(double, double)> consume, double** dev_slot, unsigned long long* key_out) {
    size_t off; unsigned long long key;
    { int rc = mbox_reserve(c, 2, &off, &key); if (rc) return rc; }
    *dev_slot = c->mbox_dev + off; *key_out = key;
    c->deferred.push_back({c->mbox + off, 2, key, [consume](const double* v) { consume(v[0], v[1]); }});
    return 0;
}
int ensure_host_buf(psgsdf_ctx* c, size_t n) {
    if (n <= c->host_buf_n) return 0;
    if (c->host_buf) hipHostFree(c->host_buf);
    c->host_buf = nullptr; c->host_buf_n = 0;
    HIPCHK(c, hipHostMalloc(&c->host_buf, sizeof(double) * n));
    c->host_buf_n = n;
    return 0;
}

void free_dense(psgsdf_ctx* c) {
    hipFree(c->dense.dist); for (int a = 0; a < 3; ++a) { hipFree(c->dense.g[a]); hipFree(c->dense.rho[a]); }
    hipFree(c->dense.weight); hipFree(c->dense.vis); hipFree(c->dense.row_of); hipFree(c->block_sums);
    c->dense = DenseView{}; c->block_sums = nullptr;
}
int alloc_dense(psgsdf_ctx* c, DenseView& d, long long nvox, int KW, bool with_rowof) {
    HIPCHK(c, hipMalloc(&d.dist, sizeof(float) * nvox));
    for (int a = 0; a < 3; ++a) { HIPCHK(c, hipMalloc(&d.g[a], sizeof(float) * nvox)); HIPCHK(c, hipMalloc(&d.rho[a], sizeof(float) * nvox)); }
    HIPCHK(c, hipMalloc(&d.weight, sizeof(float) * nvox));
    d.KW = KW;
    if (KW > 0) HIPCHK(c, hipMalloc(&d.vis, sizeof(uint64_t) * nvox * KW));
    if (with_rowof) HIPCHK(c, hipMalloc(&d.row_of, sizeof(int) * nvox));
    return 0;
}

int build_band(psgsdf_ctx* c) {
    if (!c->deferred.empty() || c->pending_fold.n) { int rc = flush(c); if (rc) return rc; }
    if (xr_quiesce(c, 120.0)) return fail(c, PSGSDF_ERR_COMM, "band rebuild: a rank never closed its mappings of this rank's record planes (lost or failed peer?)");
    if (c->n_ranks > 1 && c->comm) { int rc = xr_probe(c); if (rc) return rc; }
    c->persist_off = false;
    const long long nvox = c->grid.nvox;
    const int KW = c->dense.KW;
    if (!c->block_sums) HIPCHK(c, hipMalloc(&c->block_sums, sizeof(int) * ((nvox + 1023) / 1024 + 1)));
    timed(c, "band_flags", [&] { launch_band_flags(c->dense.dist, c->dense.vis, KW, c->grid.vs, nvox, c->dense.row_of, c->stream); });
    timed(c, "band_scan", [&] { launch_band_scan(c->dense.row_of, nvox, c->block_sums, c->d_total, c->stream); });
    int S = 0;
    HIPCHK(c, hipMemcpyAsync(&S, c->d_total, sizeof(int), hipMemcpyDeviceToHost, c->stream));
    HIPCHK(c, hipStreamSynchronize(c->stream));
    const int Spad = ((S + kBlock - 1) / kBlock) * kBlock + kBlock;
    const size_t n4 = 1 + 1 + 3 + 3 + 6 + 6 + kNQ + 12 + 6 + 14 + kNQ + 4 + 9 + 1 + 3;
    const size_t bytes = (n4 * 4 + (size_t)KW * 8) * Spad + 256;
    if (c->band_mem) { hipFree(c->band_mem); c->band_mem = nullptr; }
    if (c->rec_mem) { hipFree(c->rec_mem); c->rec_mem = nullptr; }
    HIPCHK(c, hipMalloc(&c->band_mem, bytes));
    HIPCHK(c, hipMemsetAsync(c->band_mem, 0, bytes, c->stream));
    { int rc = xr_alloc(c, &c->rec_mem, 2 * sizeof(float4) * (size_t)Spad, false); if (rc) return rc; }
    HIPCHK(c, hipMemsetAsync(c->rec_mem, 0, 2 * sizeof(float4) * (size_t)Spad, c->stream));
    c->band_bytes = bytes;
    char* p = (char*)c->band_mem;
    auto take = [&](size_t elems, size_t esz) { void* r = p; p += elems * esz * Spad; return r; };
    Band& b = c->band;
    b.S = S; b.Spad = Spad; b.KW = KW;
    b.vis = (uint64_t*)take(KW, 8);
    b.rec[0] = (float4*)c->rec_mem; b.rec[1] = b.rec[0] + Spad;
    b.lin = (int*)take(1, 4);
    b.dist = (float*)take(1, 4);
    for (int a = 0; a < 3; ++a) b.g[a] = (float*)take(1, 4);
    for (int a = 0; a < 3; ++a) b.rho[a] = (float*)take(1, 4);
    b.nb = (int*)take(6, 4); b.nbd = (float*)take(6, 4); b.col = (int*)take(kNQ, 4); b.colp = (unsigned*)take(9, 4); b.dirb = (int*)take(1, 4);
    for (int a = 0; a < 3; ++a) b.gfd[a] = (float*)take(1, 4);
    for (int a = 0; a < 3; ++a) b.vp[a] = (float4*)take(4, 4);
    b.aH = (float*)take(3, 4); b.ab = (float*)take(3, 4);
    b.blk = (float*)take(14, 4); b.H = (float*)take(kNQ, 4);
    b.hx = (int*)take(1, 4);
    b.rhs = (float*)take(1, 4); b.x = (float*)take(1, 4); b.t = (float*)take(1, 4);
    if ((size_t)(p - (char*)c->band_mem) > bytes) return fail(c, PSGSDF_ERR_DEVICE, "band arena overrun: %zu > %zu bytes", (size_t)(p - (char*)c->band_mem), bytes);
    HIPCHK(c, hipMemsetAsync(c->d_total, 0, sizeof(int), c->stream));
    timed(c, "band_fill", [&] { launch_band_fill(c->dense, c->grid, b, c->d_total, c->stream); });
    {
        int reach = 0;
        HIPCHK(c, hipMemcpyAsync(&reach, c->d_total, sizeof(int), hipMemcpyDeviceToHost, c->stream));
        HIPCHK(c, hipStreamSynchronize(c->stream));
        b.col16 = reach <= 32767; b.reach = reach;
        if (const char* e = getenv("PSGSDF_PCG_COL16")) if (atoi(e) == 0) b.col16 = 0;
    }
    {
        c->row0 = 0; c->row1 = S;
        c->halo = 0; c->need[0] = c->need[1] = 0; c->give[0] = c->give[1] = 0; c->halo_active = false;
        if (c->n_ranks > 1 && !c->comm) return fail(c, PSGSDF_ERR_COMM, "rank %d of %d has no communicator (psgsdf_comm_init)", c->rank, c->n_ranks);
        if (3 * c->n_ranks > kMgScal) return fail(c, PSGSDF_ERR_UNSUPPORTED, "at most %d ranks", kMgScal / 3);
        if (c->n_ranks > 1) {
            const long long plane = (long long)c->grid.dim[0] * c->grid.dim[1];
            int rr[2] = {0, S};
            if (S > 0) {
                launch_lower_bound(b.lin, S, (int)((c->z0 - c->zlo) * plane), c->d_need, c->stream);
                launch_lower_bound(b.lin, S, (int)((c->z1 - c->zlo) * plane), c->d_need + 1, c->stream);
                HIPCHK(c, hipMemcpyAsync(rr, c->d_need, 2 * sizeof(int), hipMemcpyDeviceToHost, c->stream));
                HIPCHK(c, hipStreamSynchronize(c->stream));
            }
            c->row0 = rr[0]; c->row1 = rr[1];
            c->need[0] = c->row0; c->need[1] = S - c->row1; c->halo = std::max(c->need[0], c->need[1]);
            std::vector<double> info(3 * (size_t)c->n_ranks, 0.0);
            info[3 * c->rank] = c->need[0]; info[3 * c->rank + 1] = c->need[1]; info[3 * c->rank + 2] = c->row1 - c->row0;
            HIPCHK(c, hipMemcpyAsync(c->mg_scal, info.data(), sizeof(double) * info.size(), hipMemcpyHostToDevice, c->stream));
            int rcc = comm_allreduce(c, c->mg_scal, (int)info.size()); if (rcc) return rcc;
            HIPCHK(c, hipMemcpyAsync(info.data(), c->mg_scal, sizeof(double) * info.size(), hipMemcpyDeviceToHost, c->stream));
            HIPCHK(c, hipStreamSynchronize(c->stream));
            const int own = c->row1 - c->row0;
            if (c->rank > 0) c->give[0] = std::min((int)info[3 * (c->rank - 1) + 1], own);
            if (c->rank < c->n_ranks - 1) c->give[1] = std::min((int)info[3 * (c->rank + 1)], own);
            c->S_global = 0;
            for (int r = 0; r < c->n_ranks; ++r) {
                if (info[3 * r] != 0.0 || info[3 * r + 1] != 0.0) c->halo_active = true;
                if (info[3 * r + 2] == 0.0) return fail(c, PSGSDF_ERR_UNSUPPORTED, "rank %d of %d owns no band rows: use fewer ranks", r, c->n_ranks);
                c->S_global += (long long)info[3 * r + 2];
            }
            int hrc = comm_halo(c, b.dirb, 1, 1); if (hrc) return hrc;
            if ((hrc = xr_setup(c, info))) return hrc;
        } else c->S_global = S;
    }
    if (c->areg_mem) { hipFree(c->areg_mem); c->areg_mem = nullptr; c->ar = AlbedoReg{}; }
    if (c->reg_r != 0.f) {
        const size_t planes = 3 + 1 + 9 + 12 + 3 + 8 * 3 + 1;
        HIPCHK(c, hipMalloc(&c->areg_mem, planes * 4 * (size_t)Spad));
        HIPCHK(c, hipMemsetAsync(c->areg_mem, 0, planes * 4 * (size_t)Spad, c->stream));
        char* q = (char*)c->areg_mem;
        auto tk = [&](size_t n) { void* r = q; q += n * 4 * (size_t)Spad; return r; };
        AlbedoReg& ar = c->ar;
        ar.anb = (int*)tk(3); ar.back = (int*)tk(1); ar.anrho = (float*)tk(9); ar.J = (float*)tk(12); ar.res = (float*)tk(3);
        ar.rhs = (float*)tk(3); ar.diag = (float*)tk(3); ar.diag0 = (float*)tk(3); ar.x = (float*)tk(3); ar.r = (float*)tk(3); ar.p = (float*)tk(3); ar.q = (float*)tk(3); ar.t = (float*)tk(3); ar.cgs = (double*)tk(1);
        SweepArgs at{}; at.b = b; at.ar = ar;
        launch_areg_tables(c->dense, c->grid, at, c->stream);
        if (int hrc = comm_halo(c, ar.back, 1, 1)) return hrc;
    }
    {
        const int nch = (c->row1 - c->row0 + kObsChunk - 1) / kObsChunk, F = c->F;
        if (c->obs_mem) { hipFree(c->obs_mem); c->obs_mem = nullptr; }
        b.obs_ptr = nullptr; b.obs_rows = nullptr; b.obs_max = 0; b.obs_ptr_total = 0;
        if (nch > 0 && F > 0) {
            int* d_counts = nullptr;
            HIPCHK(c, hipMalloc(&d_counts, sizeof(int) * (size_t)nch * F));
            launch_obs_count(b, F, c->row0, c->row1, d_counts, c->stream);
            std::vector<int> cnt((size_t)nch * F), off((size_t)nch * F), ptr(F + 1);
            HIPCHK(c, hipMemcpyAsync(cnt.data(), d_counts, sizeof(int) * cnt.size(), hipMemcpyDeviceToHost, c->stream));
            HIPCHK(c, hipStreamSynchronize(c->stream));
            int run = 0, mx = 0;
            for (int f = 0; f < F; ++f) { ptr[f] = run; for (int k = 0; k < nch; ++k) { off[(size_t)f * nch + k] = run; run += cnt[(size_t)f * nch + k]; } mx = std::max(mx, run - ptr[f]); }
            ptr[F] = run;
            HIPCHK(c, hipMalloc(&c->obs_mem, sizeof(int) * ((size_t)run + F + 2)));
            b.obs_ptr = (int*)c->obs_mem; b.obs_rows = b.obs_ptr + (F + 1); b.obs_max = mx; b.obs_ptr_total = run;
            HIPCHK(c, hipMemcpyAsync(b.obs_ptr, ptr.data(), sizeof(int) * (F + 1), hipMemcpyHostToDevice, c->stream));
            HIPCHK(c, hipMemcpyAsync(d_counts, off.data(), sizeof(int) * off.size(), hipMemcpyHostToDevice, c->stream));
            launch_obs_fill(b, F, c->row0, c->row1, d_counts, c->stream);
            HIPCHK(c, hipStreamSynchronize(c->stream));
            hipFree(d_counts);
        }
    }
    {
        if (c->vm_order) { hipFree(c->vm_order); c->vm_order = nullptr; }
        const int nb = (c->row1 - c->row0 + kBlock - 1) / kBlock;
        if (nb > 1) {
            int* d_work = nullptr;
            HIPCHK(c, hipMalloc(&d_work, sizeof(int) * nb));
            launch_block_work(b, c->row0, c->row1, d_work, c->stream);
            std::vector<int> work(nb), order(nb);
            HIPCHK(c, hipMemcpyAsync(work.data(), d_work, sizeof(int) * nb, hipMemcpyDeviceToHost, c->stream));
            HIPCHK(c, hipStreamSynchronize(c->stream));
            for (int i = 0; i < nb; ++i) order[i] = i;
            std::stable_sort(order.begin(), order.end(), [&](int x, int y) { return work[x] > work[y]; });
            HIPCHK(c, hipMalloc(&c->vm_order, sizeof(int) * nb));
            HIPCHK(c, hipMemcpyAsync(c->vm_order, order.data(), sizeof(int) * nb, hipMemcpyHostToDevice, c->stream));
            HIPCHK(c, hipStreamSynchronize(c->stream));
            hipFree(d_work);
        }
    }
    {
        c->win_G = c->win_rows = c->win_max = 0;
        int Gs = 0, Rs = 0;
        if (c->pcg_window && c->n_ranks <= 1 && cgf_solve_shape(c, &Gs, &Rs)) {
            if (!c->win_tab) HIPCHK(c, hipMalloc(&c->win_tab, sizeof(int) * (6 * kSolveMaxBlocksHost + 1)));
            int* d_max = c->win_tab + 6 * kSolveMaxBlocksHost;
            launch_solve_windows(b, c->row0, c->row1, Gs, Rs, c->win_tab, d_max, c->stream);
            int mx = 0;
            HIPCHK(c, hipMemcpyAsync(&mx, d_max, sizeof(int), hipMemcpyDeviceToHost, c->stream));
            HIPCHK(c, hipStreamSynchronize(c->stream));
            c->win_G = Gs; c->win_rows = Rs; c->win_max = mx;
        }
    }
    c->any_empty_slab = false;
    if (c->n_ranks > 1 && c->comm) {
        std::vector<double> e(1, (c->row1 <= c->row0 || b.obs_max <= 0) ? 1.0 : 0.0);
        if (int hrc = host_allreduce(c, e, "empty slabs")) return hrc;
        c->any_empty_slab = e[0] != 0.0;
    }
    {
        if (c->frame_part) { hipFree(c->frame_part); c->frame_part = nullptr; }
        if (c->frame_done) { hipFree(c->frame_done); c->frame_done = nullptr; }
        c->frame_cap = (b.obs_max + kBlock * 4 - 1) / (kBlock * 4) + 1;
        const int F = std::max(c->F, 1);
        HIPCHK(c, hipMalloc(&c->frame_part, sizeof(double) * (size_t)F * c->frame_cap * kFrameRow));
        HIPCHK(c, hipMalloc(&c->frame_done, sizeof(int) * (F + 1)));
        HIPCHK(c, hipMemsetAsync(c->frame_done, 0, sizeof(int) * (F + 1), c->stream));
    }
    if (c->part) { hipFree(c->part); c->part = nullptr; }
    c->PB = Spad / kBlock + 1;
    HIPCHK(c, hipMalloc(&c->part, sizeof(double) * SC_COUNT * c->PB));
    HIPCHK(c, hipMemsetAsync(c->part, 0, sizeof(double) * SC_COUNT * c->PB, c->stream));
    {
        const size_t need = 4096;
        if (need > c->mbox_alloc) {
            if (c->mbox) hipHostFree(c->mbox);
            c->mbox = nullptr; c->mbox_n = 0; c->mbox_alloc = 0;
            HIPCHK(c, hipHostMalloc(&c->mbox, sizeof(double) * need, hipHostMallocMapped));
            HIPCHK(c, hipHostGetDevicePointer((void**)&c->mbox_dev, c->mbox, 0));
            c->mbox_alloc = need; c->mbox_n = need - 2;
            memset(c->mbox, 0, sizeof(double) * need); c->flush_seq = 0;
        }
        if (slab_mode(c) && !c->mbox_shadow) {
            HIPCHK(c, hipMalloc(&c->mbox_shadow, sizeof(double) * c->mbox_alloc));
            HIPCHK(c, hipMemsetAsync(c->mbox_shadow, 0, sizeof(double) * c->mbox_alloc, c->stream));
        }
        c->mbox_used = 0; c->deferred.clear(); c->mg_segs.clear();
    }
    return ensure_host_buf(c, (size_t)SC_COUNT * c->PB + (size_t)c->F * kFrameRow + 4096 + 64);
}

int derive(psgsdf_ctx* c, int update_grad) {
    SweepArgs a = make_args(c, 0);
    timed(c, "derive", [&] { launch_derive(a, update_grad, c->stream); });
    const int slots[2] = {SC_EN, SC_EL}; double s[2];
    int rc = read_parts(c, slots, 2, s); if (rc) return rc;
    c->en_sum = s[0]; c->el_sum = s[1];
    return 0;
}


int ps_energy(psgsdf_ctx* c, double* E, int64_t* nobs) {
    SweepArgs a = make_args(c, 0);
    take_fold(c, a, (1u << SC_ENERGY) | (1u << SC_NOBS) | (1u << SC_AUX0) | (1u << SC_AUX1) | (1u << SC_AUX2));
    timed(c, "energy", [&] { launch_energy(a, c->stream); });
    const int slots[2] = {SC_ENERGY, SC_NOBS}; double s[2];
    int rc = read_parts(c, slots, 2, s); if (rc) return rc;
    *E = band_mean(c, s[0]); if (nobs) *nobs = (int64_t)s[1];
    return 0;
}

}
```

### psgradientsdf_amd/csrc/engine_internal.h

```cpp
#pragma once
#include "engine.h"
#include "../../include/psgsdf.h"

#include <math.h>
#include <float.h>
#include <stdarg.h>
#include <stdio.h>
#include <stdlib.h>
#include <string.h>
#include <algorithm>
#include <functional>
#include <memory>
#include <map>
#include <string>
#include <vector>

namespace psge {
constexpr int kMgScal = 96;
struct KTime { double ms = 0; int64_t n = 0; };
struct Comm;
struct MgSeg { unsigned off, n; unsigned long long key; };
struct Deferred { const double* src; int n; unsigned long long key; std::function<void(const double*)> consume; };
enum XoSlot {
    XO_MESH_XYZ, XO_MESH_RGB,
    XO_PC_XYZN, XO_PC_RGB,
    XO_SDF,
    XO_IMESH_XYZ, XO_IMESH_NORMALS, XO_IMESH_RGB, XO_IMESH_FACES,
    XO_VERTEX_COMPONENT, XO_COMPONENTS,
    XO_LOD_VERTEX_MAP,
    XO_FIT_NOBS, XO_FIT_LOSS, XO_FIT_R2,
    XO_VFIT_NOBS, XO_VFIT_RMS, XO_VFIT_LOSS,
    XO_BAKE_UV, XO_BAKE_ALBEDO, XO_BAKE_NORMAL, XO_BAKE_DISPLACEMENT, XO_BAKE_VOXEL, XO_BAKE_FACE,
    XO_AO_DIRS, XO_AO_MASK, XO_AO_OCCLUSION,
    XO_BAKE_AO_MASK, XO_BAKE_AO_OCCLUSION,
    XO_PHOTO, XO_PHOTO_RGB, XO_PHOTO_NOBS, XO_PHOTO_STATUS,
    XO_CMP_VDIST, XO_CMP_VNEAREST, XO_CMP_VSIDE, XO_CMP_RDIST, XO_CMP_RNEAREST, XO_CMP_RSIDE,
    XO_ALN_XYZ,
    XO_CURV_VALID, XO_CURV_MEAN, XO_CURV_GAUSS, XO_CURV_K1, XO_CURV_K2, XO_CURV_DIR1,
    XO_VCURV_VALID, XO_VCURV_MEAN, XO_VCURV_GAUSS, XO_VCURV_K1, XO_VCURV_K2,
    XO_BAKE_CURV_MEAN, XO_BAKE_CURV_VALID,
    XO_FILL_LIN, XO_FILL_DIST, XO_FILL_GRAD, XO_FILL_RGB, XO_FILL_ROUND,
    XO_FILL_VERTEX,
    XO_COUNT
};
}
using psge::KTime;
using namespace psg;

struct psgsdf_ctx {
    int device = 0;
    hipStream_t stream = nullptr;
    psgsdf_settings set{};
    float reg_n = 0, reg_l = 0;
    GridP grid{};
    int gdim[3]{}; long long gnvox = 0;
    int z0 = 0, z1 = 0;
    int zlo = 0, zhi = 0;
    long long S_global = 0;
    float shift[3]{};
    Cam cam{};
    DenseView dense{};
    uint64_t* vis_seq = nullptr; int wpv_seq = 0;
    int* block_sums = nullptr; int* d_total = nullptr;
    bool have_volume = false;
    int F = 0;
    int* frame_idx = nullptr;
    float* img = nullptr;
    FrameP* frames = nullptr;
    std::vector<FrameP> frames_h;
    float* led_light = nullptr;
    bool have_frames = false;
    void* band_mem = nullptr; size_t band_bytes = 0;
    void* rec_mem = nullptr;
    void* obs_mem = nullptr;
    float* stage = nullptr; size_t stage_px = 0;
    void* pin_stage = nullptr; size_t pin_bytes = 0;
    float* ncache = nullptr; double* ntmp = nullptr; float* nout = nullptr; float* ndepth = nullptr; int ncache_w = 0, ncache_h = 0;
    double* track_part = nullptr; double* track_host = nullptr;
    Band band{};
    bool inited = false;
    double* acc_frame = nullptr; size_t acc_frame_n = 0;
    double* frame_part = nullptr; int frame_cap = 0;
    int* frame_done = nullptr;
    double* part = nullptr; int PB = 0;
    double* pcg_sc = nullptr; int pcg_cap = 4096;
    double* pcg_part = nullptr;
    double* pcg_gran = nullptr;
    unsigned pcg_solve_serial = 0;
    int pcg_ablate = 0;
    bool pcg_fuse_apply = true;
    bool pcg_persist = true;
    bool pcg_window = true;
    int pcg_solve_rows = 0;
    int* win_tab = nullptr;
    int win_G = 0, win_rows = 0, win_max = 0;
    int last_solve_windowed = -1;
    bool persist_off = false;
    int num_cu = 0;
    int last_cg_iters = 0;
    bool want_counts = true;
    double* host_buf = nullptr; size_t host_buf_n = 0;
    double* mbox = nullptr; double* mbox_dev = nullptr; size_t mbox_n = 0, mbox_used = 0;
    size_t mbox_alloc = 0; double flush_seq = 0;
    std::vector<psge::Deferred> deferred;
    unsigned long long mbox_serial = 0;
    bool mbox_check = true;
    psgsdf_iter_cb observer = nullptr; void* observer_user = nullptr;
    int on_iter_period = 1;
    bool speculate = true;
    bool spec_undo = false, spec_albedo_saved = false, spec_light_saved = false;
    FrameP* frames_undo = nullptr;
    long long spec_windows = 0, spec_undos = 0;
    int fault_solve = 0, solves_seen = 0;
    long long persist_fallbacks = 0;
    long long mbox_checked = 0, mbox_late = 0;
    double en_sum = 0, el_sum = 0;
    int rank = 0, n_ranks = 1;
    int row0 = 0, row1 = 0, halo = 0;
    psge::Comm* comm = nullptr;
    bool xr_enable = true;
    bool xr_ready = false; long long xr_solves = 0;
    double* xr = nullptr;
    int xr_mem_kind = -1;
    long long xr_probe_stale = 0, xr_probe_timeouts = 0;
    long long xr_probe_local[3][4] = {{0, 0, 0, 0}, {0, 0, 0, 0}, {0, 0, 0, 0}};
    bool xr_mapped = false;
    std::shared_ptr<void> comm_keep;
    unsigned long long xr_openers = 0;
    long long xr_serial = 0, xr_closed_off = 0;
    void* xo_host[psge::XO_COUNT] = {}; size_t xo_bytes[psge::XO_COUNT] = {};
    long long xr_stale_maps = 0;
    bool leak_exported = false;
    std::vector<double*> xr_peer;
    void* band_peer[2] = {nullptr, nullptr};
    std::vector<void*> xr_opened;
    XrArgs xr_args{};
    int cu_mask_lo = -1, cu_mask_hi = -1;
    double* mg_scal = nullptr;
    double* mg_ext = nullptr;
    double* mbox_shadow = nullptr;
    std::vector<psge::MgSeg> mg_segs;
    int give[2] = {0, 0};
    bool halo_active = false;
    long long n_collectives = 0;
    float reg_r = 0.f;
    void* areg_mem = nullptr; AlbedoReg ar{};
    bool areg_device = true; int areg_last_iters = 0;
    double er_sum = 0;
    FoldReq pending_fold{};
    bool fuse_pcg_init = true;
    bool fuse_albedo = true;
    bool fold_in_next = true;
    int xwait_spins = 1 << 24;
    long long fault_halo = 0;
    bool xh_enable = true;
    void* hx_mem = nullptr;
    char* hx_peer[2] = {nullptr, nullptr};
    size_t hx_peer_par[2] = {0, 0}, hx_peer_off[2] = {0, 0}, hx_par = 0;
    long long hx_flag_off = 0, hx_epoch = 0, n_halo_pushes = 0;
    bool hx_ready = false;
    bool xs_enable = true;
    long long xs_epoch = 0;
    bool xf_enable = true;
    XfTable* xf_table = nullptr;
    long long xf_epoch = 0;
    size_t xr_doubles = 0;
    bool any_empty_slab = false;
    bool xf_timeout = false;
    bool img_compact = true;
    bool img_compacted = false;
    bool speculate_mr = true;
    int* vm_order = nullptr;
    int xcd_map = 163;
    bool fm_solve = true;
    bool fm_solve_led = true;
    bool fm_solved = false;
    int frame_solve = 0;
    double* fs_stats = nullptr;
    double fs_last[2][4] = {{0, 0, 1, 1}, {0, 0, 1, 1}};
    bool albedo_applied = false;
    unsigned* img8 = nullptr; float img_scale = 0.f;
    double* frame_e_slot = nullptr; unsigned long long frame_e_key = 0;
    bool ao_cut = true;
    long long compare_chunk = 1ll << 24;
    long long cmp_pairs[2] = {0, 0}, cmp_queries[2] = {0, 0};
    long long aln_evals = 0, aln_iters = 0, aln_pairs[2] = {0, 0}, aln_queries[2] = {0, 0};
    bool pcg_poll = true;
    int need[2] = {0, 0}; int* d_need = nullptr;
    bool own_stream = true;
    bool profiling = false;
    std::map<std::string, KTime> ktimes;
    std::vector<const char*> kt_names;
    hipEvent_t ev0 = nullptr, ev1 = nullptr;
    std::string watch;
    std::vector<std::pair<hipEvent_t, hipEvent_t>> watch_pool;
    size_t watch_used = 0; int watch_every = 1; size_t watch_seen = 0;
    std::vector<std::pair<std::string, std::string>> tuning_env, tuning_ignored;
    char err[512] = {0};
};

namespace psge {
using namespace psg;

int fail(psgsdf_ctx* c, int code, const char* fmt, ...);
inline unsigned long long dbits(double v) { unsigned long long u; memcpy(&u, &v, 8); return u; }
#define HIPCHK(c, expr) do { hipError_t _e = (expr); if (_e != hipSuccess) return fail(c, PSGSDF_ERR_DEVICE, "%s: %s (%s:%d)", #expr, hipGetErrorString(_e), __FILE__, __LINE__); } while (0)

struct DevMem {
    explicit DevMem(psgsdf_ctx* wait_for = nullptr) : c(wait_for) {}
    DevMem(const DevMem&) = delete;
    DevMem& operator=(const DevMem&) = delete;
    ~DevMem() { if (c) hipStreamSynchronize(c->stream); for (void* q : p) hipFree(q); }
    template <class T> bool get(T** out, size_t count) {
        void* q = nullptr;
        const bool ok = hipMalloc(&q, std::max<size_t>(8, sizeof(T) * count)) == hipSuccess;
        if (ok) p.push_back(q);
        *out = (T*)q;
        return ok;
    }
private:
    psgsdf_ctx* c; std::vector<void*> p;
};

template <class Fn> void timed(psgsdf_ctx* c, const char* name, Fn&& fn) {
    if (!c->profiling) {
        if (!c->watch.empty() && c->watch == name && (c->watch_seen++ % c->watch_every) == 0) {
            if (c->watch_used == c->watch_pool.size()) {
                hipEvent_t a, b; hipEventCreate(&a); hipEventCreate(&b); c->watch_pool.emplace_back(a, b);
            }
            auto& pr = c->watch_pool[c->watch_used++];
            hipEventRecord(pr.first, c->stream);
            fn();
            hipEventRecord(pr.second, c->stream);
            return;
        }
        fn(); return;
// ... 72 lines not shown
```

### psgradientsdf_amd/csrc/loop.hip

```cpp
#include "engine_internal.h"
#include <climits>

namespace psge {

constexpr int kCgfSumsHost = 7;
void cgf_shape(int nblk, int* G, int* rows) {
    nblk = std::max(1, nblk);
    int r = 1, cap = kCgfMaxBlocks;
    if (const char* e = getenv("PSGSDF_PCG_ROWS")) { int v = atoi(e); if (v >= 1 && v <= 2) r = v; }
    if (const char* e = getenv("PSGSDF_PCG_BLOCKS")) { int v = atoi(e); if (v > 0 && v <= kCgfMaxBlocks) cap = v; }
    const int per = (nblk + r - 1) / r;
    const int trips = (per + cap - 1) / cap;
    *G = (per + trips - 1) / trips; *rows = r;
}

bool cgf_solve_shape(psgsdf_ctx* c, int* G, int* rows_per_wg, bool any_ranks) {
    if (!c->pcg_persist || c->persist_off || (c->n_ranks > 1 && !c->xr_ready && !any_ranks) || !c->band.col16 || !c->fuse_pcg_init || c->num_cu <= 0 || band_blocks(c) > kPcgMaxBlocks) return false;
    const int n = c->row1 - c->row0, cap = std::min(c->num_cu, kSolveMaxBlocksHost);
    if (n <= 0) return false;
    int g = std::min(cap, (n + kSolveThreadsHost - 1) / kSolveThreadsHost);
    g = std::max(8, g / 8 * 8);
    if (g > cap) g = cap;
    int per = ((n + g - 1) / g + 63) / 64 * 64;
    if (c->pcg_solve_rows > 0 && c->n_ranks <= 1) {
// ... 89 lines not shown
        for (int q = 0; q < n; ++q) {
            if (mr) { int rc = comm_halo(c, c->band.rec[(k + q + 1) & 1], 1, 4); if (rc) return rc; }
            timed(c, "pcg_pass", [&] { launch_cgf_pass(ap, c->pcg_sc, c->pcg_part, G, rows, k + q, cap, c->mbox_dev + off + q, c->stream); });
            if (mr) {
                launch_cgf_sum(c->pcg_part, G, k + q, c->mg_ext, c->stream);
                int rc = comm_allreduce(c, c->mg_ext, kCgfSumsHost); if (rc) return rc;
            }
        }
        if (tail && c->pcg_poll && !c->profiling) { tail(c->pcg_sc + (gate_on_converged ? 2 : 1)); if (tail_ran) *tail_ran = true; }
        bool drained = !c->pcg_poll;
        if (drained) { int rc = flush(c); if (rc) return rc; }
        for (int q = 0; q < n && iters < 0; ++q) {
            const int kk = k + q;
            if (!drained && st[q] == -1.0) {
                const int w = wait_mapped(c, [st, q] { return st[q] != -1.0; }, "pcg_solve");
                if (w < 0) return w;
                drained = w == 1;
            }
            double v = st[q];
            if (v == -1.0) {
                HIPCHK(c, hipStreamSynchronize(c->stream));
                v = st[q];
            }
            if (v == -1.0) return fail(c, PSGSDF_ERR_DEVICE, "PCG kernel %d published nothing", kk);
            if (std::isnan(v)) return fail(c, PSGSDF_ERR_DEVICE, "PCG kernel %d published NaN: the distance system (or the sums another rank contributed) contains NaN", kk);
            if (kk == 0) {
                rhsN = (float)v;
                if (rhsN == 0.f) { iters = 0; break; }
                threshold = fmaxf(FLT_EPSILON * FLT_EPSILON * rhsN, FLT_MIN);
                rn2_last = rhsN;
                continue;
            }
            rn2_last = (float)v;
            if (rn2_last < threshold) iters = kk - 1;
            else if (kk == cap) iters = cap;
        }
        if (!drained && c->pending_fold.n) { int rc = flush(c); if (rc) return rc; drained = true; }
        if (!drained) { int rc = deliver(c); if (rc) return rc; }
        if (rhsN == 0.f) { *iters_out = 0; *success_out = 1; *err_out = 0; c->last_cg_iters = 0; return 0; }
        if (iters >= 0) break;
        k += n;
        chunk = 4;
    }
    double err = sqrt((double)rn2_last / (double)rhsN);
    *iters_out = iters; *err_out = err; *success_out = err <= (double)FLT_EPSILON;
    c->last_cg_iters = iters;
    return 0;
}

int albedo_reg_energy(psgsdf_ctx* c, double* Er) {
    SweepArgs a = make_args(c, 0);
    int rc = comm_halo(c, c->band.rho[0], 3, 1); if (rc) return rc;
    launch_areg_build(a, c->stream);
    const int slots[1] = {SC_AUX0}; double s[1];
    if ((rc = read_parts(c, slots, 1, s))) return rc;
    c->er_sum = s[0]; *Er = band_mean(c, s[0]);
    return 0;
}
int albedo_reg_solve(psgsdf_ctx* c, const SweepArgs& a, int* iters_out, int* ok_out, double* err_out) {
    const AlbedoReg& ar = a.ar;
    int rc = comm_halo(c, c->band.rho[0], 3, 1); if (rc) return rc;
    launch_areg_build(a, c->stream);
    if ((rc = comm_halo(c, ar.J, 15, 1))) return rc;
    launch_areg_system(a, c->stream);
    launch_areg_cg_init(a, c->stream);
    const int two[2] = {SC_AUX0, SC_AUX1}, one[1] = {SC_AUX0}; double s[2];
    if ((rc = read_parts(c, two, 2, s))) return rc;
    const float rhsN = (float)s[0];
    *iters_out = 0; *ok_out = 1; *err_out = 0;
    if (rhsN == 0.f) return 0;
    const float thr = fmaxf(FLT_EPSILON * FLT_EPSILON * rhsN, FLT_MIN);
    float res2 = rhsN, absNew = (float)s[1];
    const int maxIters = c->set.cg_max_it > 0 ? c->set.cg_max_it : (int)std::min<long long>(6 * c->S_global, INT_MAX);
    int i = 0;
    if (res2 >= thr && c->areg_device && !slab_mode(c)) {
        const double init[5] = {0.0, 0.0, (double)rhsN, s[1], 0.0};
        HIPCHK(c, hipMemcpyAsync(ar.cgs, init, sizeof(init), hipMemcpyHostToDevice, c->stream));
        HIPCHK(c, hipStreamSynchronize(c->stream));
        const int nblk = band_blocks(c);
        int chunk = std::min(64, std::max(4, c->areg_last_iters + 2));
        double got[5] = {0, 0, 0, 0, 0};
        while (i < maxIters) {
            const int n = std::min(chunk, maxIters - i);
            for (int q = 0; q < n; ++q) launch_areg_cg_iteration(a, i + q, nblk, thr, c->stream);
            HIPCHK(c, hipMemcpyAsync(got, ar.cgs, sizeof(got), hipMemcpyDeviceToHost, c->stream));
            HIPCHK(c, hipStreamSynchronize(c->stream));
            res2 = (float)got[2];
            if (got[0] != 0.0) { i = (int)got[1]; break; }
            i += n; chunk = 4;
        }
        if (!(res2 == res2)) return fail(c, PSGSDF_ERR_DEVICE, "the regularised albedo solve produced NaN");
        c->areg_last_iters = i;
    } else if (res2 >= thr) {
        while (i < maxIters) {
            if ((rc = comm_halo(c, ar.p, 3, 1))) return rc;
            launch_areg_jx(a, ar.p, ar.t, c->stream);
            if ((rc = comm_halo(c, ar.t, 3, 1))) return rc;
            launch_areg_jt(a, ar.p, ar.t, ar.q, c->stream);
            if ((rc = read_parts(c, one, 1, s))) return rc;
            const float alpha = absNew / (float)s[0];
            launch_areg_cg_update(a, alpha, c->stream);
            if ((rc = read_parts(c, two, 2, s))) return rc;
            res2 = (float)s[0];
            if (res2 < thr) break;
            const float absOld = absNew; absNew = (float)s[1];
            launch_areg_cg_dir(a, absNew / absOld, c->stream);
            ++i;
        }
    }
    *iters_out = i; *err_out = sqrt((double)res2 / (double)rhsN); *ok_out = *err_out <= (double)FLT_EPSILON;
    return 0;
}

int step_begin(psgsdf_ctx* c, int block, int laplacian_reg, psgsdf_step_stats* st, std::function<void(double, double)> deferred_consumer, bool may_apply) {
    memset(st, 0, sizeof(*st));
    st->block = block;
    SweepArgs a = make_args(c, laplacian_reg);
    const bool led = c->set.model == PSGSDF_LED;
    double e_sum = 0, nobs = 0;
    int rc;
    switch (block) {
        case PSGSDF_ALBEDO: case PSGSDF_DIST: {
            if (block == PSGSDF_ALBEDO) {
                c->albedo_applied = may_apply && c->reg_r == 0.f && c->fuse_albedo;
                a.fuse_apply = c->albedo_applied ? (c->spec_undo ? 2 : 1) : 0;
                if (c->albedo_applied && c->spec_undo) c->spec_albedo_saved = true;
                take_fold(c, a, (1u << SC_ENERGY) | (1u << SC_NOBS) | (c->albedo_applied ? (1u << SC_ACCEPT) : 0u));
                timed(c, "sweep_albedo", [&] { launch_sweep_albedo(a, c->stream); });
            }
            else {
                materialize_fold(c);
                { int Gs, Rs; if (c->fuse_pcg_init && band_blocks(c) <= kPcgMaxBlocks && cgf_solve_shape(c, &Gs, &Rs)) { a.pcg_gran = c->pcg_gran; a.pcg_gran_n = 2 * kSolveGranPlanes * kSolveMaxBlocksHost; a.pcg_asm = 1; } }
                timed(c, "sweep_dist", [&] { launch_sweep_dist(a, c->stream); });
            }
            const int slots[2] = {SC_ENERGY, SC_NOBS}; double s[2];
            if (deferred_consumer) return read_parts_deferred(c, slots, 2, [deferred_consumer](const double* v) { deferred_consumer(v[0], v[1]); });
            if ((rc = read_parts(c, slots, 2, s))) return rc;
            e_sum = s[0]; nobs = s[1];
            break;
        }
        case PSGSDF_LIGHT: case PSGSDF_POSE: {
            int col, launched = 0;
            const bool xf = c->n_ranks > 1 && c->xf_enable && c->xr_ready && c->xf_table && !c->any_empty_slab;
            const bool fuse = deferred_consumer && c->fm_solve && c->frame_solve == 0 && (!slab_mode(c) || c->n_ranks == 1 || xf) && !c->profiling && (block == PSGSDF_POSE || !led || c->fm_solve_led) && c->row1 > c->row0 && c->band.obs_max > 0;
            double* fm_slot = nullptr; unsigned long long fm_key = 0;
            if (fuse) {
                if ((rc = reserve_frame_energy_deferred(c, xf ? std::function<void(double, double)>([c, deferred_consumer](double e, double n) { if (std::isnan(e)) c->xf_timeout = true; deferred_consumer(e, n); }) : deferred_consumer, &fm_slot, &fm_key))) return rc;
                a.fm_solve = 1; a.fm_frames = c->frames; a.fm_led_light = c->led_light; a.fm_e_out = fm_slot; a.fm_e_key = fm_key;
                if (xf) { a.xf = c->xf_table; a.xf_epoch = ++c->xf_epoch; }
                a.fm_undo = (block == PSGSDF_LIGHT && c->spec_undo) ? (float*)c->frames_undo : nullptr;
            }
            if (block == PSGSDF_LIGHT) {
                take_fold(c, a, 0u);
                timed(c, "sweep_light", [&] { launched = launch_sweep_light(a, c->stream); });
                const int n = led ? 3 : (c->set.model == PSGSDF_SH2 ? 9 : 4), nh = led ? 3 : n * (n + 1) / 2;
                col = nh + n;
            } else { take_fold(c, a, 0u); timed(c, "sweep_pose", [&] { launched = launch_sweep_pose(a, c->stream); }); col = 27; }
            if (fuse) {
                if (launched) { c->fm_solved = true; return 0; }
                c->frame_e_slot = fm_slot; c->frame_e_key = fm_key;
            }
            if (!launched) {
                HIPCHK(c, hipMemsetAsync(c->acc_frame, 0, sizeof(double) * c->acc_frame_n, c->stream));
                fold_by_kernel(c, a.fold);
            }
            if (fuse) return 0;
            if ((rc = comm_allreduce(c, c->acc_frame, c->F * kFrameRow))) return rc;
            if (deferred_consumer) return reserve_frame_energy_deferred(c, deferred_consumer, &c->frame_e_slot, &c->frame_e_key);
            if ((rc = read_frame_energy(c, col, &e_sum, &nobs))) return rc;
            break;
        }
        default: return fail(c, PSGSDF_ERR_ARG, "unknown block %d", block);
    }
    st->e_in = band_mean(c, e_sum);
    st->n_obs = (int64_t)nobs;
    return 0;
}
int read_frame_solver_stats(psgsdf_ctx* c, int kind, psgsdf_step_stats* st) {
    HIPCHK(c, hipMemcpyAsync(c->fs_last[kind], c->fs_stats + 4 * kind, sizeof(double) * 4, hipMemcpyDeviceToHost, c->stream));
    HIPCHK(c, hipStreamSynchronize(c->stream));
    if (st) { st->cg_iters = (int)c->fs_last[kind][0]; st->cg_error = c->fs_last[kind][1]; st->cg_converged = (int)c->fs_last[kind][2]; st->applied = (int)c->fs_last[kind][3]; }
    return 0;
}
int step_finish(psgsdf_ctx* c, int block, int laplacian_reg, psgsdf_step_stats* st, bool defer_reg_sums) {
    SweepArgs a = make_args(c, laplacian_reg);
    const bool led = c->set.model == PSGSDF_LED;
    int rc;
    switch (block) {
        case PSGSDF_ALBEDO: {
            const int slots[1] = {SC_ACCEPT}; double s[1];
            if (c->reg_r != 0.f) {
                int iters = 0, ok = 1; double err = 0;
                if ((rc = albedo_reg_solve(c, a, &iters, &ok, &err))) return rc;
                const int apply = (led || ok) ? 1 : 0;
                if (apply) timed(c, "apply_albedo", [&] { launch_apply_albedo_delta(a, c->ar.x, c->stream); });
                if (apply && c->want_counts) { if ((rc = read_parts(c, slots, 1, s))) return rc; st->n_accepted = (int64_t)s[0]; }
                st->cg_iters = iters; st->cg_converged = ok; st->cg_error = err; st->applied = apply;
                break;
            }
            if (!c->albedo_applied) {
                take_fold(c, a, 1u << SC_ACCEPT);
                timed(c, "apply_albedo", [&] { launch_apply_albedo(a, c->stream); });
            }
            c->albedo_applied = false;
            if (c->want_counts) { if ((rc = read_parts(c, slots, 1, s))) return rc; st->n_accepted = (int64_t)s[0]; }
            st->cg_iters = 1; st->cg_converged = 1; st->applied = 1;
            break;
        }
        case PSGSDF_LIGHT:
            if (c->fm_solved) c->fm_solved = false;
            else if (c->frame_solve == 1) {
                if (!frames_eigen_fits(c->set.model, c->F)) return fail(c, PSGSDF_ERR_UNSUPPORTED, "PSGSDF_FRAME_SOLVE=eigen holds at most 2048 unknowns in its one workgroup (%d keyframes)", c->F);
                timed(c, "solve_light_eigen", [&] { launch_frames_eigen_light(a, c->frames, c->led_light, c->frame_e_slot, c->frame_e_key, c->spec_undo ? (float*)c->frames_undo : nullptr, c->fs_stats, c->stream); });
            }
            else timed(c, "solve_light", [&] { launch_solve_light(a, c->frames, c->led_light, c->frame_e_slot, c->frame_e_key, c->spec_undo ? (float*)c->frames_undo : nullptr, c->stream); });
            if (c->spec_undo) c->spec_light_saved = true;
            c->frame_e_slot = nullptr; c->frame_e_key = 0;
            st->cg_converged = 1; st->applied = 1; st->n_accepted = led ? 1 : c->F;
            if (c->frame_solve == 1 && c->want_counts) { if ((rc = read_frame_solver_stats(c, 0, st))) return rc; }
            break;
        case PSGSDF_POSE:
            if (c->fm_solved) c->fm_solved = false;
            else if (c->frame_solve == 1) {
                if (!frames_eigen_fits(c->set.model, c->F)) return fail(c, PSGSDF_ERR_UNSUPPORTED, "PSGSDF_FRAME_SOLVE=eigen holds at most 2048 unknowns in its one workgroup (%d keyframes)", c->F);
                timed(c, "solve_pose_eigen", [&] { launch_frames_eigen_pose(a, c->frames, c->frame_e_slot, c->frame_e_key, c->fs_stats + 4, c->stream); });
            }
            else timed(c, "solve_pose", [&] { launch_solve_pose(a, c->frames, c->frame_e_slot, c->frame_e_key, c->stream); });
            c->frame_e_slot = nullptr; c->frame_e_key = 0;
            st->cg_converged = 1; st->applied = 1; st->n_accepted = c->F;
            if (c->frame_solve == 1 && c->want_counts) { if ((rc = read_frame_solver_stats(c, 1, st))) return rc; st->n_accepted = st->applied ? c->F : 0; }
            break;
        case PSGSDF_DIST: {
            take_fold(c, a, 0u);
            if (c->fuse_pcg_init && band_blocks(c) <= kPcgMaxBlocks) { a.pcg_fuse_init = 1; a.pcg_init_blocks = band_blocks(c); }
            bool apply_in_solve = false;
            { int Gs, Rs; if (a.pcg_fuse_init && cgf_solve_shape(c, &Gs, &Rs)) { a.pcg_gran = c->pcg_gran; a.pcg_gran_n = 2 * kSolveGranPlanes * kSolveMaxBlocksHost; a.pcg_asm = 1; apply_in_solve = c->pcg_fuse_apply && Gs <= band_blocks(c); } }
            if ((rc = comm_halo(c, c->band.blk, 14, 1))) return rc;
            if (!a.pcg_asm) { timed(c, "assemble", [&] { launch_assemble(a, c->stream); }); a.fold.n = 0; }
            int iters = 0, ok = 1; double err = 0;
            const bool only_on_success = !led && c->set.ref_quirks;
            if (apply_in_solve) a.pcg_apply = only_on_success ? 2 : 1;
            bool tail_ran = false; int tail_rc = 0;
            auto tail = [&](const double* gate) {
                SweepArgs ag = a; ag.fold.n = 0; ag.gate = gate;
                if (!a.pcg_apply) timed(c, "apply_dist", [&] { launch_apply_dist(ag, c->stream); });
                if (int hrc = comm_halo(c, c->band.dist, 1, 1)) tail_rc = hrc;
                SweepArgs a2 = make_args(c, 0); a2.gate = gate;
                timed(c, "derive", [&] { launch_derive(a2, 1, c->stream); });
            };
            if ((rc = pcg_solve(c, a, &iters, &ok, &err, tail, only_on_success, &tail_ran))) return rc;
            if (tail_rc) return tail_rc;
            int apply = 1;
            if (only_on_success && !ok) apply = 0;
            if (apply) {
                if (!tail_ran) { tail(nullptr); if (tail_rc) return tail_rc; }
                const int slots[3] = {SC_ACCEPT, SC_EN, SC_EL}; double s[3];
                if (defer_reg_sums) { if ((rc = read_parts_deferred(c, slots, 3, [c](const double* v) { c->en_sum = v[1]; c->el_sum = v[2]; }))) return rc; }
                else { if ((rc = read_parts(c, slots, 3, s))) return rc; st->n_accepted = (int64_t)s[0]; c->en_sum = s[1]; c->el_sum = s[2]; }
            }
            st->cg_iters = iters; st->cg_converged = ok; st->cg_error = err; st->applied = apply;
            break;
        }
        default: return fail(c, PSGSDF_ERR_ARG, "unknown block %d", block);
    }
    return 0;
}
int do_step(psgsdf_ctx* c, int block, int laplacian_reg, psgsdf_step_stats* st) {
    psgsdf_step_stats tmp; if (!st) st = &tmp;
    int rc = step_begin(c, block, laplacian_reg, st); if (rc) return rc;
    return step_finish(c, block, laplacian_reg, st);
}


void close_iteration(psgsdf_ctx* c, LoopState& L, psgsdf_iter_stats* rec, int pending_slot, float E, bool early_exit_semantics) {
    L.E = E;
    if (pending_slot >= 0) rec->e_after[pending_slot] = (double)E;
    rec->e_n = L.E_n; rec->e_l = L.E_l; rec->e_r = L.E_r;
    rec->e_total = (double)total_energy(c, L.E, L.E_n, L.E_l, L.E_r);
    rec->reg_weight_n = c->reg_n; rec->reg_weight_l = c->reg_l;
    float Et = (float)rec->e_total;
    rec->rel_diff = (double)(fabsf(L.E_prev - Et) / L.E_prev);
    rec->converged = rec->rel_diff < (double)c->set.conv_threshold;
    rec->diverged = early_exit_semantics ? (!rec->converged && (L.E_prev < Et)) : (L.E_prev < Et);
}

int run_loop(psgsdf_ctx* c, int flags, LoopState& L, int max_iters, bool full, psgsdf_iter_stats* stats, int stats_cap, int* n_done, int* result,
             psgsdf_iter_cb on_iter, void* user) {
    const bool led = c->set.model == PSGSDF_LED;
    const int order[4] = {led ? PSGSDF_LIGHT : PSGSDF_ALBEDO, led ? PSGSDF_ALBEDO : PSGSDF_LIGHT, PSGSDF_DIST, PSGSDF_POSE};
    psgsdf_iter_stats rec; memset(&rec, 0, sizeof(rec));
    psgsdf_iter_stats prev; int prev_slot = -1; bool have_prev = false;
    struct CountsOff { psgsdf_ctx* c; bool old; CountsOff(psgsdf_ctx* c_) : c(c_), old(c_->want_counts) { c->want_counts = false; } ~CountsOff() { c->want_counts = old; } } counts_off(c);
    int done = 0, iter = 0; if (result) *result = 0;
    bool stop = false;
    auto finalize = [&](psgsdf_iter_stats& r, int it) -> int {
        const bool term = full && (r.converged || r.diverged);
        float E_last = (float)r.e_total;
        if (full && !term && it == 5 && c->set.upsample) {
            if (c->reg_l == 0.0f) c->reg_l = 1.0f;
            L.laplacian_reg = 1;
            int rc = do_upsample(c); if (rc) return rc;
            L.E_l = (float)band_mean(c, c->el_sum);
            c->reg_l *= L.E / L.E_l;
            E_last = total_energy(c, L.E, L.E_n, L.E_l, L.E_r);
            r.upsampled = 1;
        }
        if (full && !term && c->set.upsample && (led ? it == 15 : it > 15)) c->reg_l = 0.0f;
        L.E_prev = E_last;
        if (stats && done < stats_cap) stats[done] = r;
        done++;
// ... 169 lines not shown
```

### psgradientsdf_amd/csrc/sweeps.hip

```cpp
#include "device_common.h"

#ifndef PSG_FM_PIPE
#define PSG_FM_PIPE 3
#endif
#ifndef PSG_POSE_WAVES
#define PSG_POSE_WAVES 1
#endif

namespace psg {

__global__ void __launch_bounds__(kBlock) k_init_albedo(SweepArgs a) {
#pragma clang fp contract(off)
    FrameP* sf = reinterpret_cast<FrameP*>(psg_dyn_smem);
    load_frames(sf, a.frames, a.F);
    const Band& b = a.b;
    int j = a.row0 + blockIdx.x * blockDim.x + threadIdx.x;
    if (j >= a.row1) return;
    const float4 p0 = b.vp[0][j];
    float xs[3] = {p0.x, p0.y, p0.z};
    int count = 0; float rho[3] = {0, 0, 0};
    FOR_EACH_VISIBLE_FRAME(b, j, a.F, f) {
        Proj pr = project(xs, frame_at(sf, f), a.cam);
        if (!pr.ok) continue;
        float I[3];
        sample<false>(a.im, f, a.cam, pr.m, pr.n, I, nullptr, nullptr);
        rho[0] += I[0]; rho[1] += I[1]; rho[2] += I[2]; count++;
    }
    if (count) {
#pragma unroll
        for (int k = 0; k < 3; ++k) set_rho(b, j, k, rho[k] / (float)count);
    }
}
void launch_init_albedo(const SweepArgs& a, hipStream_t s) {
    if (a.row1 > a.row0) hipLaunchKernelGGL(k_init_albedo, dim3((a.row1 - a.row0 + kBlock - 1) / kBlock), dim3(kBlock), a.F * sizeof(FrameP), s, a);
}

template <int MODEL, int LOSS, int IMG, bool LED_INIT = false>
__global__ void __launch_bounds__(kBlock) k_energy(SweepArgs a) {
    { __shared__ double fred[kBlock / 64]; fold_pending(a, fred); }
    constexpr int NB = ModelTraits<MODEL>::NB;
    FrameP* sf = reinterpret_cast<FrameP*>(psg_dyn_smem);
    __shared__ double red[kBlock / 64];
    load_frames(sf, a.frames, a.F);
    const Band& b = a.b;
    const int bid = vm_bid(a, 2, true);
    int j = a.row0 + bid * blockDim.x + threadIdx.x;
    double E = 0, nobs = 0, sI[3] = {0, 0, 0}, sR[3] = {0, 0, 0};
    obs_acc_t Ef = 0;
    if (j < a.row1) {
        Vox v; load_vox(b, j, v);
        float shfd[kMaxBasis];
        if (!ModelTraits<MODEL>::LED) SH<NB == 3 ? 4 : NB>(v.nfd, shfd);
        FOR_EACH_VISIBLE_FRAME(b, j, a.F, f) {
            const FrameP& fp = frame_at(sf, f);
            Proj pr = project(v.xs, fp, a.cam);
            if (!pr.ok) continue;
            float I[3], ren[3];
            sample<false, IMG>(a.im, f, a.cam, pr.m, pr.n, I, nullptr, nullptr);
            rendered<MODEL>(fp, pr, v.nfd, shfd, v.rho, ren);
            if (LED_INIT) {
#pragma unroll
                for (int ch = 0; ch < 3; ++ch) { sI[ch] += (double)I[ch]; sR[ch] += (double)ren[ch]; }
            } else {
                float l = 0.f;
#pragma unroll
                for (int ch = 0; ch < 3; ++ch) l += robust_loss<LOSS>(a.rob, I[ch] - ren[ch]);
                Ef += (obs_acc_t)l; nobs += 1.0;
            }
        }
    }
    E = (double)Ef;
    if (LED_INIT) {
        block_part_store(sI[0], PART(a, SC_AUX0), red, bid); block_part_store(sI[1], PART(a, SC_AUX1), red, bid); block_part_store(sI[2], PART(a, SC_AUX2), red, bid);
        block_part_store(sR[0], PART(a, SC_EN), red, bid); block_part_store(sR[1], PART(a, SC_EL), red, bid); block_part_store(sR[2], PART(a, SC_ACCEPT), red, bid);
    } else {
        block_part_store(E, PART(a, SC_ENERGY), red, bid);
        block_part_store(nobs, PART(a, SC_NOBS), red, bid);
    }
}
void launch_energy(const SweepArgs& a, hipStream_t s) {
    if (a.row1 <= a.row0) return;
    dim3 g((a.row1 - a.row0 + kBlock - 1) / kBlock), bl(kBlock);
    PSG_LAUNCH_SWEEP(k_energy, a, false, g, bl, a.F * sizeof(FrameP), s, a);
}
void launch_led_light_init(const SweepArgs& a, hipStream_t s) {
    if (a.row1 > a.row0) hipLaunchKernelGGL((k_energy<2, -1, -1, true>), dim3((a.row1 - a.row0 + kBlock - 1) / kBlock), dim3(kBlock), a.F * sizeof(FrameP), s, a);
}

template <int MODEL, int LOSS, int IMG>
__global__ void __launch_bounds__(kBlock) k_sweep_albedo(SweepArgs a) {
    { __shared__ double fred[kBlock / 64]; fold_pending(a, fred); }
    constexpr int NB = ModelTraits<MODEL>::NB;
    FrameP* sf = reinterpret_cast<FrameP*>(psg_dyn_smem);
    __shared__ double red[kBlock / 64];
    load_frames(sf, a.frames, a.F);
    const Band& b = a.b;
    const int bid = vm_bid(a, 2, true);
    int j = a.row0 + bid * blockDim.x + threadIdx.x;
    double E = 0, nobs = 0, cnt = 0;
    if (j < a.row1) {
        Vox v; load_vox(b, j, v);
        float shfd[kMaxBasis], shg[kMaxBasis];
        if (!ModelTraits<MODEL>::LED) { SH<NB == 3 ? 4 : NB>(v.nfd, shfd); SH<NB == 3 ? 4 : NB>(v.gn, shg); }
        obs_acc_t Hd[3] = {0, 0, 0}, bd[3] = {0, 0, 0};
        obs_acc_t Ef = 0; int nobs_i = 0;
        FOR_EACH_VISIBLE_FRAME(b, j, a.F, f) {
            const FrameP& fp = frame_at(sf, f);
            Proj pr = project(v.xs, fp, a.cam);
            if (!pr.ok) continue;
            float I[3], ren[3], J[3];
            sample<false, IMG>(a.im, f, a.cam, pr.m, pr.n, I, nullptr, nullptr);
            rendered<MODEL>(fp, pr, v.nfd, shfd, v.rho, ren);
            rho_jac<MODEL>(fp, pr, v.gn, shg, J);
            float l = 0.f;
#pragma unroll
            for (int ch = 0; ch < 3; ++ch) {
                float r = I[ch] - ren[ch]; float w = robust_weight<LOSS>(a.rob, r);
                float jw = J[ch] * w;
                Hd[ch] += (obs_acc_t)(jw * J[ch]); bd[ch] += (obs_acc_t)(jw * r);
                l += robust_loss<LOSS>(a.rob, r);
            }
            Ef += (obs_acc_t)l; nobs_i += 1;
        }
        E = (double)Ef; nobs = (double)nobs_i;
        if (a.fuse_apply) {
            if (a.fuse_apply == 2) {
#pragma unroll
                for (int ch = 0; ch < 3; ++ch) b.aH[(size_t)ch * b.Spad + j] = v.rho[ch];
            }
#pragma unroll
            for (int ch = 0; ch < 3; ++ch) {
                float h = (float)Hd[ch];
                if (a.damping != 0.0f) h += a.damping * h;
                const float delta = (h != 0.f) ? (float)bd[ch] / h : 0.f;
                const float nv = v.rho[ch] - delta;
                if (nv > 0.0f && nv < 1.0f) { set_rho(b, j, ch, nv); cnt += 1.0; }
            }
        } else {
#pragma unroll
            for (int ch = 0; ch < 3; ++ch) { b.aH[(size_t)ch * b.Spad + j] = (float)Hd[ch]; b.ab[(size_t)ch * b.Spad + j] = (float)bd[ch]; }
        }
    }
    block_part_store(E, PART(a, SC_ENERGY), red, bid);
    block_part_store(nobs, PART(a, SC_NOBS), red, bid);
    if (a.fuse_apply) block_part_store(cnt, PART(a, SC_ACCEPT), red, bid);
}
void launch_sweep_albedo(const SweepArgs& a, hipStream_t s) {
    if (a.row1 <= a.row0) return;
    dim3 g((a.row1 - a.row0 + kBlock - 1) / kBlock), bl(kBlock);
    PSG_LAUNCH_SWEEP(k_sweep_albedo, a, false, g, bl, a.F * sizeof(FrameP), s, a);
}
__global__ void __launch_bounds__(kBlock) k_apply_albedo(SweepArgs a) {
    { __shared__ double fred[kBlock / 64]; fold_pending(a, fred); }
    __shared__ double red[kBlock / 64];
    const Band& b = a.b;
    int j = a.row0 + blockIdx.x * blockDim.x + threadIdx.x;
    double cnt = 0;
    if (j < a.row1) {
#pragma unroll
        for (int ch = 0; ch < 3; ++ch) {
            float h = b.aH[(size_t)ch * b.Spad + j];
            if (a.damping != 0.0f) h += a.damping * h;
            float delta = (h != 0.f) ? b.ab[(size_t)ch * b.Spad + j] / h : 0.f;
            float v = b.rho[ch][j] - delta;
            if (v > 0.0f && v < 1.0f) { set_rho(b, j, ch, v); cnt += 1.0; }
        }
    }
    block_part_store(cnt, PART(a, SC_ACCEPT), red);
}
__global__ void __launch_bounds__(kBlock) k_restore_albedo(SweepArgs a) {
    const Band& b = a.b;
    int j = a.row0 + blockIdx.x * blockDim.x + threadIdx.x;
    if (j >= a.row1) return;
#pragma unroll
    for (int ch = 0; ch < 3; ++ch) set_rho(b, j, ch, b.aH[(size_t)ch * b.Spad + j]);
}
void launch_restore_albedo(const SweepArgs& a, hipStream_t s) {
    if (a.row1 > a.row0) hipLaunchKernelGGL(k_restore_albedo, dim3((a.row1 - a.row0 + kBlock - 1) / kBlock), dim3(kBlock), 0, s, a);
}
void launch_apply_albedo(const SweepArgs& a, hipStream_t s) {
    if (a.row1 > a.row0) hipLaunchKernelGGL(k_apply_albedo, dim3((a.row1 - a.row0 + kBlock - 1) / kBlock), dim3(kBlock), 0, s, a);
}

static int fm_rows(const SweepArgs& a, int slots_per_cu) {
    if (const char* e = getenv("PSGSDF_FM_ROWS")) { int v = atoi(e); if (v >= 4 && v <= 64) return v; }
    const long long total = a.b.obs_ptr_total > 0 ? a.b.obs_ptr_total : (long long)a.b.obs_max * a.F;
    const long long slots = 256LL * slots_per_cu;
    long long r = (total + (long long)(0.92 * slots) * kBlock - 1) / ((long long)(0.92 * slots) * kBlock);
    return (int)std::min<long long>(std::max<long long>(r, 4), 64);
}

template <int N> __device__ void solve_spd(const double* Hin, const double* bin, double* x);

__device__ __forceinline__ double ldrow(const double* p) { return __hip_atomic_load(p, __ATOMIC_RELAXED, __HIP_MEMORY_SCOPE_AGENT); }
template <int NB>
__device__ __forceinline__ void frame_solve_light_sh(FrameP* frames, int f, const double* acc, float* undo) {
    constexpr int NH = NB * (NB + 1) / 2;
    if (undo) for (int i = 0; i < 9; ++i) undo[f * 9 + i] = frames[f].l[i];
    double Hd[NB * NB], bd[NB], xd[NB];
    int q = 0;
    for (int i = 0; i < NB; ++i) for (int k = i; k < NB; ++k) { double v = (double)(float)ldrow(acc + q++); Hd[i * NB + k] = v; Hd[k * NB + i] = v; }
    for (int i = 0; i < NB; ++i) bd[i] = (double)(float)ldrow(acc + NH + i);
    solve_spd<NB>(Hd, bd, xd);
    for (int i = 0; i < NB; ++i) frames[f].l[i] -= (float)xd[i];
}
__device__ __forceinline__ void frame_solve_pose(const SweepArgs& a, FrameP* frames, int f, const double* acc) {
    double Hd[36], bd[6], xd[6];
    int q = 0;
    for (int i = 0; i < 6; ++i) for (int k = i; k < 6; ++k) {
        float v = (float)ldrow(acc + q++);
        if (i == k && a.damping != 0.0f) v += a.damping * v;
        Hd[i * 6 + k] = (double)v; Hd[k * 6 + i] = (double)v;
    }
    for (int i = 0; i < 6; ++i) bd[i] = (double)(float)ldrow(acc + 21 + i);
    solve_spd<6>(Hd, bd, xd);
    float xi[6];
    for (int i = 0; i < 6; ++i) xi[i] = (float)xd[i];
    pose_update(frames, f, xi);
}

template <int NV, int KIND, int MODEL>
__device__ __forceinline__ void frame_tail(const SweepArgs& a, double* lds, bool solve_all) {
    if (solve_all) {
        for (int ff = threadIdx.x; ff < a.F; ff += blockDim.x) {
            const double* row = a.acc.frame + (size_t)ff * kFrameRow;
            if (KIND == 0) { if (!ModelTraits<MODEL>::LED) frame_solve_light_sh<ModelTraits<MODEL>::NB == 3 ? 4 : ModelTraits<MODEL>::NB>(a.fm_frames, ff, row, a.fm_undo); }
            else frame_solve_pose(a, a.fm_frames, ff, row);
        }
        __syncthreads();
    }
    if (KIND == 0 && ModelTraits<MODEL>::LED) {
        constexpr int NHL = 3;
        __shared__ float s_dl[3];
        if (a.fm_undo) {
            for (int i = threadIdx.x; i < a.F * 9; i += blockDim.x) a.fm_undo[i] = a.fm_frames[i / 9].l[i % 9];
            if (threadIdx.x < 3) a.fm_undo[a.F * 9 + threadIdx.x] = a.fm_led_light[threadIdx.x];
        }
        __shared__ double srow[6 * kMaxFramesLds];
        for (int i = threadIdx.x; i < 6 * a.F; i += blockDim.x) { const int ff = i / 6, c6 = i % 6; srow[c6 * kMaxFramesLds + ff] = __hip_atomic_load(a.acc.frame + (size_t)ff * kFrameRow + (c6 < 3 ? c6 : NHL + c6 - 3), __ATOMIC_RELAXED, __HIP_MEMORY_SCOPE_AGENT); }
        __syncthreads();
        if (threadIdx.x < 3) {
            const int ch = threadIdx.x;
            double hs = 0, bs = 0;
            for (int ff = 0; ff < a.F; ++ff) { hs += srow[ch * kMaxFramesLds + ff]; bs += srow[(3 + ch) * kMaxFramesLds + ff]; }
            float h = (float)hs; const float bb = (float)bs;
            if (a.damping != 0.0f) h += a.damping * h;
            double Hd[1] = {(double)h}, bd[1] = {(double)bb}, xd[1];
            solve_spd<1>(Hd, bd, xd);
            s_dl[ch] = (float)xd[0];
        }
        __syncthreads();
        for (int ff = threadIdx.x; ff < a.F; ff += blockDim.x) {
#pragma unroll
            for (int ch = 0; ch < 3; ++ch) { const float nl = a.fm_frames[ff].l[ch] - s_dl[ch]; a.fm_frames[ff].l[ch] = nl; if (ff == 0) a.fm_led_light[ch] = nl; }
        }
    }
    if (a.fm_e_out) {
        constexpr int col_e = NV - 2;
        double e = 0, n = 0;
        for (int ff = threadIdx.x; ff < a.F; ff += blockDim.x) {
            e += __hip_atomic_load(a.acc.frame + (size_t)ff * kFrameRow + col_e, __ATOMIC_RELAXED, __HIP_MEMORY_SCOPE_AGENT);
            n += __hip_atomic_load(a.acc.frame + (size_t)ff * kFrameRow + col_e + 1, __ATOMIC_RELAXED, __HIP_MEMORY_SCOPE_AGENT);
        }
        e = wave_sum(e); n = wave_sum(n);
        const int lane = threadIdx.x & 63, w = threadIdx.x >> 6;
        __syncthreads();
        if (lane == 0) { lds[2 * w] = e; lds[2 * w + 1] = n; }
        __syncthreads();
        if (threadIdx.x == 0) { double te = 0, tn = 0; for (int i = 0; i < (int)(blockDim.x >> 6); ++i) { te += lds[2 * i]; tn += lds[2 * i + 1]; } mbox_put(a.fm_e_out, 2, 0, te, a.fm_e_key); mbox_put(a.fm_e_out, 2, 1, tn, a.fm_e_key); mbox_commit(a.fm_e_key); }
    }
}

template <int NV, int KIND, int MODEL>
__device__ __forceinline__ void frame_rows_publish(const SweepArgs& a, int cx, int f, double* lds ) {
    __shared__ int s_last;
    double* dst = a.acc.fpart + ((size_t)f * a.acc.fcap + cx) * kFrameRow;
    if (threadIdx.x < NV) {
        double s = 0;
        for (int i = 0; i < kBlock / 64; ++i) s += lds[i * NV + threadIdx.x];
        __hip_atomic_store(dst + threadIdx.x, s, __ATOMIC_RELAXED, __HIP_MEMORY_SCOPE_AGENT);
    }
    if (threadIdx.x < 64) {
        asm volatile("s_waitcnt vmcnt(0)" ::: "memory");
        if (threadIdx.x == 0) s_last = __hip_atomic_fetch_add(a.acc.fdone + f, 1, __ATOMIC_RELAXED, __HIP_MEMORY_SCOPE_AGENT) == (int)gridDim.x - 1;
    }
    __syncthreads();
    if (!s_last) return;
    if (threadIdx.x == 0) __hip_atomic_store(a.acc.fdone + f, 0, __ATOMIC_RELAXED, __HIP_MEMORY_SCOPE_AGENT);
    const bool solve = a.fm_solve != 0;
    if (threadIdx.x < NV) {
        const double* p = a.acc.fpart + (size_t)f * a.acc.fcap * kFrameRow + threadIdx.x;
        double s = 0;
        for (int c = 0; c < (int)gridDim.x; c += 16) {
            double v[16];
#pragma unroll
            for (int j = 0; j < 16; ++j) v[j] = c + j < (int)gridDim.x ? __hip_atomic_load(p + (size_t)(c + j) * kFrameRow, __ATOMIC_RELAXED, __HIP_MEMORY_SCOPE_AGENT) : 0.0;
#pragma unroll
            for (int j = 0; j < 16; ++j) s += v[j];
        }
        if (solve && a.xf) {
            const XfTable& t = *a.xf;
            const int Rk = t.n_ranks, buf = (int)(a.xf_epoch & 1);
            const long long slot = ((long long)buf * Rk + t.rank) * t.F + f;
            for (int r = 0; r < Rk; ++r) store8_system(t.region[r] + t.pay + slot * kFrameRow + threadIdx.x, s);
            asm volatile("s_waitcnt vmcnt(0)" ::: "memory");
            if (threadIdx.x == 0) for (int r = 0; r < Rk; ++r) __hip_atomic_store(t.region[r] + t.flg + slot, (double)a.xf_epoch, __ATOMIC_RELAXED, __HIP_MEMORY_SCOPE_SYSTEM);
        }
        else if (solve) { __hip_atomic_store(a.acc.frame + (size_t)f * kFrameRow + threadIdx.x, s, __ATOMIC_RELAXED, __HIP_MEMORY_SCOPE_AGENT); lds[threadIdx.x] = s; }
        else a.acc.frame[(size_t)f * kFrameRow + threadIdx.x] = s;
    }
    if (!solve) return;
    if (a.xf) return;
    __syncthreads();
    if (threadIdx.x == 0) {
        if (KIND == 0) { if (!ModelTraits<MODEL>::LED) frame_solve_light_sh<ModelTraits<MODEL>::NB == 3 ? 4 : ModelTraits<MODEL>::NB>(a.fm_frames, f, lds, a.fm_undo); }
        else frame_solve_pose(a, a.fm_frames, f, lds);
    }
    if (threadIdx.x < 64) {
        asm volatile("s_waitcnt vmcnt(0)" ::: "memory");
        if (threadIdx.x == 0) s_last = __hip_atomic_fetch_add(a.acc.fdone + a.F, 1, __ATOMIC_RELAXED, __HIP_MEMORY_SCOPE_AGENT) == (int)gridDim.y - 1;
    }
    __syncthreads();
    if (!s_last) return;
    if (threadIdx.x == 0) __hip_atomic_store(a.acc.fdone + a.F, 0, __ATOMIC_RELAXED, __HIP_MEMORY_SCOPE_AGENT);
    frame_tail<NV, KIND, MODEL>(a, lds, false);
}

constexpr int kGatherFrames = 16;
template <int NV, int KIND, int MODEL>
__global__ void __launch_bounds__(kBlock) k_frame_gather(SweepArgs a) {
    __shared__ double lds[(kBlock / 64) * NV > 2 * (kBlock / 64) ? (kBlock / 64) * NV : 2 * (kBlock / 64)];
    __shared__ unsigned char s_late[kGatherFrames];
    __shared__ int s_last;
    const XfTable& t = *a.xf;
    const int Rk = t.n_ranks, buf = (int)(a.xf_epoch & 1);
    const double tag = (double)a.xf_epoch;
    double* const mine = t.region[t.rank];
    const int f0 = blockIdx.x * kGatherFrames, nf = min(kGatherFrames, a.F - f0);
    if (threadIdx.x < kGatherFrames) s_late[threadIdx.x] = 0;
    __syncthreads();
    for (int q = threadIdx.x; q < nf * Rk; q += blockDim.x) {
        const int ff = f0 + q / Rk, r = q - (q / Rk) * Rk;
        const double* fp = mine + t.flg + ((long long)buf * Rk + r) * t.F + ff;
        int spins = 0; bool late = false;
        while (__hip_atomic_load(fp, __ATOMIC_RELAXED, __HIP_MEMORY_SCOPE_SYSTEM) != tag) { __builtin_amdgcn_s_sleep(2); if (++spins > t.spin_max) { late = true; break; } }
        if (late) {
            s_late[ff - f0] = 1;
            __hip_atomic_store(mine + kXrLate, tag, __ATOMIC_RELAXED, __HIP_MEMORY_SCOPE_SYSTEM);
            __hip_atomic_store(mine + kXrLate + 3, (double)(r * 1000 + ff), __ATOMIC_RELAXED, __HIP_MEMORY_SCOPE_SYSTEM);
        }
    }
    __builtin_amdgcn_fence(__ATOMIC_ACQUIRE, "");
    __syncthreads();
    for (int i = threadIdx.x; i < nf * NV; i += blockDim.x) {
        const int fl = i / NV, l = i - fl * NV, ff = f0 + fl;
        const double* p0 = mine + t.pay + ((long long)buf * Rk * t.F + ff) * kFrameRow + l;
        double tot = 0.0;
        for (int r0 = 0; r0 < Rk; r0 += 8) {
            double v[8];
#pragma unroll
            for (int j = 0; j < 8; ++j) v[j] = r0 + j < Rk ? __hip_atomic_load(p0 + (long long)(r0 + j) * t.F * kFrameRow, __ATOMIC_RELAXED, __HIP_MEMORY_SCOPE_SYSTEM) : 0.0;
#pragma unroll
            for (int j = 0; j < 8; ++j) tot += v[j];
        }
        if (s_late[fl]) tot = __builtin_nan("");
        __hip_atomic_store(a.acc.frame + (size_t)ff * kFrameRow + l, tot, __ATOMIC_RELAXED, __HIP_MEMORY_SCOPE_AGENT);
    }
    asm volatile("s_waitcnt vmcnt(0)" ::: "memory");
    __syncthreads();
    if (threadIdx.x == 0) s_last = __hip_atomic_fetch_add(a.acc.fdone + a.F, 1, __ATOMIC_RELAXED, __HIP_MEMORY_SCOPE_AGENT) == (int)gridDim.x - 1;
    __syncthreads();
    if (!s_last) return;
    if (threadIdx.x == 0) __hip_atomic_store(a.acc.fdone + a.F, 0, __ATOMIC_RELAXED, __HIP_MEMORY_SCOPE_AGENT);
    frame_tail<NV, KIND, MODEL>(a, lds, true);
}
template <int KIND>
static void launch_frame_gather(const SweepArgs& a, hipStream_t s) {
    const dim3 g((a.F + kGatherFrames - 1) / kGatherFrames), bl(kBlock);
    constexpr int NVP = 21 + 6 + 2;
    if (KIND == 1) {
        if (a.model == 0) hipLaunchKernelGGL((k_frame_gather<NVP, 1, 0>), g, bl, 0, s, a);
        else if (a.model == 1) hipLaunchKernelGGL((k_frame_gather<NVP, 1, 1>), g, bl, 0, s, a);
        else hipLaunchKernelGGL((k_frame_gather<NVP, 1, 2>), g, bl, 0, s, a);
    } else {
        if (a.model == 0) hipLaunchKernelGGL((k_frame_gather<16, 0, 0>), g, bl, 0, s, a);
        else if (a.model == 1) hipLaunchKernelGGL((k_frame_gather<56, 0, 1>), g, bl, 0, s, a);
        else hipLaunchKernelGGL((k_frame_gather<8, 0, 2>), g, bl, 0, s, a);
    }
}

template <int MODEL, int LOSS, int IMG>
__global__ void __launch_bounds__(kBlock) k_sweep_light(SweepArgs a, int rows) {
    { __shared__ double fred[kBlock / 64]; fold_pending(a, fred); }
    constexpr int NB = ModelTraits<MODEL>::NB;
    constexpr bool LED = ModelTraits<MODEL>::LED;
    constexpr int NH = LED ? 3 : NB * (NB + 1) / 2;
    constexpr int NV = NH + NB + 2;
    __shared__ FrameP sfp;
    __shared__ double lds[(kBlock / 64) * NV];
    int cx, f; fm_ids(a, cx, f);
    if (threadIdx.x < (int)(sizeof(FrameP) / 4)) ((float*)&sfp)[threadIdx.x] = ((const float*)(a.frames + f))[threadIdx.x];
    __syncthreads();
    const Band& b = a.b;
    const FrameP& fp = sfp;
    ImgSrc img = a.im;
    if (img.u8) img.u8 += (size_t)f * a.cam.H * a.cam.W; else img.f32 += (size_t)f * a.cam.H * a.cam.W * 3;
    img.idx32 = true;
    obs_acc_t acc[NV];
#pragma unroll
    for (int k = 0; k < NV; ++k) acc[k] = 0;
    const int beg = b.obs_ptr[f], end = b.obs_ptr[f + 1];
    auto accumulate = [&](const Vox& v, const Proj& pr, const float* I) {
        float shfd[kMaxBasis], shg[kMaxBasis];
        if (!LED) { SH<NB == 3 ? 4 : NB>(v.nfd, shfd); SH<NB == 3 ? 4 : NB>(v.gn, shg); }
        float ren[3];
        rendered<MODEL>(fp, pr, v.nfd, shfd, v.rho, ren);
        float refl = 0.f;
        if (LED) { float Rp[3]; mul3(fp.R, pr.p, Rp); refl = dot3(v.gn, Rp); float pn = norm3(pr.p); double pd = (double)pn; refl /= (float)(pd * pd * pd); }
        float l = 0.f, w2 = 0.f, r1 = 0.f;
#pragma unroll
        for (int ch = 0; ch < 3; ++ch) {
            float r = I[ch] - ren[ch]; float w = robust_weight<LOSS>(a.rob, r);
            l += robust_loss<LOSS>(a.rob, r);
            if (LED) {
                float J = refl * v.rho[ch]; float jw = J * w;
                acc[ch] += (obs_acc_t)(jw * J); acc[NH + ch] += (obs_acc_t)(jw * r);
            } else {
#if PSG_STRICT & 16
                float Jc[kMaxBasis];
#pragma unroll
                for (int i = 0; i < NB; ++i) Jc[i] = -v.rho[ch] * shg[i];
                int q = 0;
#pragma unroll
                for (int i = 0; i < NB; ++i) {
                    const float jw = Jc[i] * w;
#pragma unroll
                    for (int k = i; k < NB; ++k) acc[q++] += (obs_acc_t)(jw * Jc[k]);
                    acc[NH + i] += (obs_acc_t)(jw * r);
                }
#else
                w2 += w * (v.rho[ch] * v.rho[ch]);
                r1 -= w * (v.rho[ch] * r);
#endif
            }
        }
#if !(PSG_STRICT & 16)
        if (!LED) {
            int q = 0;
#pragma unroll
            for (int i = 0; i < NB; ++i) {
                const float sw = shg[i] * w2;
#pragma unroll
                for (int k = i; k < NB; ++k) acc[q++] += (obs_acc_t)(sw * shg[k]);
                acc[NH + i] += (obs_acc_t)(shg[i] * r1);
            }
        }
#endif
        acc[NH + NB] += (obs_acc_t)l; acc[NH + NB + 1] += 1;
    };
    const int e0 = beg + cx * (kBlock * rows) + threadIdx.x;
    if constexpr (IMG >= 0 && !(PSG_STRICT & 4) && (PSG_FM_PIPE & 1)) {
        fm_for_each_obs<IMG>(b, fp, a.cam, img, e0, end, rows, [&](const ObsPend<IMG>& P) {
            float I[3];
            taps_colour<IMG, false>(img, a.cam, P.ts, P.pr.m, P.pr.n, P.pr.m, P.pr.n, I, nullptr, nullptr);
            accumulate(P.v, P.pr, I);
            return true;
        }, [&](const Vox&, const Proj&) {});
    } else {
    int e = e0;
    int j_cur = e < end ? b.obs_rows[e] : -1;
    int j_nxt = (rows > 1 && e + kBlock < end) ? b.obs_rows[e + kBlock] : -1;
    Vox vn;
    if (j_cur >= 0) load_vox(b, j_cur, vn);
    for (int it = 0; it < rows && j_cur >= 0; ++it, e += kBlock) {
        const Vox v = vn;
        const int j_nn = (it + 2 < rows && e + 2 * kBlock < end) ? b.obs_rows[e + 2 * kBlock] : -1;
        if (j_nxt >= 0) load_vox(b, j_nxt, vn);
        j_cur = j_nxt; j_nxt = j_nn;
        Proj pr = project(v.xs, fp, a.cam);
        if (!pr.ok) continue;
        float I[3];
        sample<false, IMG>(img, 0, a.cam, pr.m, pr.n, I, nullptr, nullptr);
        accumulate(v, pr, I);
    }
    }
    const int w = threadIdx.x >> 6;
    wave_sums_to<NV>(acc, lds + w * NV);
    __syncthreads();
    frame_rows_publish<NV, 0, MODEL>(a, cx, f, lds);
}
int launch_sweep_light(const SweepArgs& a, hipStream_t s) {
    if (a.b.S <= 0 || a.F <= 0 || a.b.obs_max <= 0) return 0;
    const int rows = fm_rows(a, a.model == 1 ? 3 : ((PSG_FM_PIPE & 1) ? 4 : 5));
    const int chunk = kBlock * rows;
    dim3 g((a.b.obs_max + chunk - 1) / chunk, a.F), bl(kBlock);
    PSG_LAUNCH_SWEEP(k_sweep_light, a, true, g, bl, 0, s, a, rows);
    if (a.xf && a.fm_solve) launch_frame_gather<0>(a, s);
    return (int)g.x;
}

template <int MODEL, int LOSS, int IMG>
__global__ void __launch_bounds__(kBlock, PSG_POSE_WAVES) k_sweep_pose(SweepArgs a, int rows) {
    { __shared__ double fred[kBlock / 64]; fold_pending(a, fred); }
    constexpr int NB = ModelTraits<MODEL>::NB;
    constexpr bool LED = ModelTraits<MODEL>::LED;
    constexpr int NV = 21 + 6 + 2;
    __shared__ FrameP sfp;
    __shared__ double lds[(kBlock / 64) * NV];
    int cx, f; fm_ids(a, cx, f);
    if (threadIdx.x < (int)(sizeof(FrameP) / 4)) ((float*)&sfp)[threadIdx.x] = ((const float*)(a.frames + f))[threadIdx.x];
    __syncthreads();
    const Band& b = a.b;
    const FrameP& fp = sfp;
    ImgSrc img = a.im;
    if (img.u8) img.u8 += (size_t)f * a.cam.H * a.cam.W; else img.f32 += (size_t)f * a.cam.H * a.cam.W * 3;
    img.idx32 = true;
    obs_acc_t acc[NV];
#pragma unroll
    for (int k = 0; k < NV; ++k) acc[k] = 0;
    const int beg = b.obs_ptr[f], end = b.obs_ptr[f + 1];
    auto accumulate = [&](const Vox& v, const Proj& pr, const ProjJ& pj, const float* I, const float* gu, const float* gv) {
        float shfd[kMaxBasis];
        if (!LED) SH<NB == 3 ? 4 : NB>(v.nfd, shfd);
        float ren[3];
        rendered<MODEL>(fp, pr, v.nfd, shfd, v.rho, ren);
        const PiRows pi = pi_rows(a.cam, pr);
        const float* p = pr.p;
        float J[18];
#if PSG_STRICT & 16
        {
            float G[9];
#pragma unroll
            for (int ch = 0; ch < 3; ++ch) { G[ch * 3 + 0] = gu[ch] * pi.p00 + gv[ch] * 0.0f; G[ch * 3 + 1] = gu[ch] * 0.0f + gv[ch] * pi.p11; G[ch * 3 + 2] = gu[ch] * pi.p02 + gv[ch] * pi.p12; }
            const float sk[9] = {0, -p[2], p[1], p[2], 0, -p[0], -p[1], p[0], 0};
#pragma unroll
            for (int ch = 0; ch < 3; ++ch)
#pragma unroll
                for (int k = 0; k < 3; ++k) {
                    const float sg = (G[ch * 3 + 0] * fp.R[k * 3 + 0] + G[ch * 3 + 1] * fp.R[k * 3 + 1]) + G[ch * 3 + 2] * fp.R[k * 3 + 2];
                    J[ch * 6 + k] = -sg;
                    J[ch * 6 + 3 + k] = (G[ch * 3 + 0] * sk[0 * 3 + k] + G[ch * 3 + 1] * sk[1 * 3 + k]) + G[ch * 3 + 2] * sk[2 * 3 + k];
                }
            if (LED) {
                const float pn = norm3(p); const double pd = (double)pn; const float l3 = (float)(pd * pd * pd);
#pragma unroll
                for (int ch = 0; ch < 3; ++ch) {
                    const float sl = -(v.rho[ch] * fp.l[ch] / l3);
#pragma unroll
                    for (int k = 0; k < 3; ++k) J[ch * 6 + k] += sl * v.gn[k];
                }
            }
        }
#else
        float U[3], V[3]; pi_rows_world(pi, fp.R, U, V);
        const float AS[3] = {-(pi.p02 * p[1]), pi.p02 * p[0] - pi.p00 * p[2], pi.p00 * p[1]};
        const float BS[3] = {pi.p11 * p[2] - pi.p12 * p[1], pi.p12 * p[0], -(pi.p11 * p[0])};
        if (!LED) {
            float A6[6], B6[6];
#pragma unroll
            for (int k = 0; k < 3; ++k) { A6[k] = -U[k]; B6[k] = -V[k]; A6[3 + k] = AS[k]; B6[3 + k] = BS[k]; }
            float aa = 0.f, ab = 0.f, bb = 0.f, ra = 0.f, rb = 0.f, l = 0.f;
#pragma unroll
            for (int ch = 0; ch < 3; ++ch) {
                const float r = I[ch] - ren[ch]; float w = robust_weight<LOSS>(a.rob, r);
                l += robust_loss<LOSS>(a.rob, r);
                w = pj.ok ? w : 0.f;
                const float wu = w * gu[ch], wv = w * gv[ch];
                aa += wu * gu[ch]; ab += wu * gv[ch]; bb += wv * gv[ch]; ra += wu * r; rb += wv * r;
            }
            int q = 0;
#pragma unroll
            for (int i = 0; i < 6; ++i) {
                const float Pi = aa * A6[i] + ab * B6[i], Qi = ab * A6[i] + bb * B6[i];
#pragma unroll
                for (int k = i; k < 6; ++k) { acc[q] += (obs_acc_t)(Pi * A6[k]); acc[q] += (obs_acc_t)(Qi * B6[k]); ++q; }
                acc[21 + i] += (obs_acc_t)(ra * A6[i]); acc[21 + i] += (obs_acc_t)(rb * B6[i]);
            }
            acc[27] += (obs_acc_t)l; acc[28] += 1;
            return;
        }
#pragma unroll
        for (int ch = 0; ch < 3; ++ch)
#pragma unroll
            for (int k = 0; k < 3; ++k) {
                J[ch * 6 + k] = -(gu[ch] * U[k] + gv[ch] * V[k]);
                J[ch * 6 + 3 + k] = gu[ch] * AS[k] + gv[ch] * BS[k];
            }
        {
            float pn = norm3(p); double pd = (double)pn; float l3 = (float)(pd * pd * pd);
            const float yl3 = 1.0f / l3;
#pragma unroll
            for (int ch = 0; ch < 3; ++ch) {
                float s = -div_by(v.rho[ch] * fp.l[ch], l3, yl3);
#pragma unroll
                for (int k = 0; k < 3; ++k) J[ch * 6 + k] += s * v.gn[k];
            }
        }
#endif
        float l = 0.f;
#pragma unroll
        for (int ch = 0; ch < 3; ++ch) {
            float r = I[ch] - ren[ch]; float w = robust_weight<LOSS>(a.rob, r);
            l += robust_loss<LOSS>(a.rob, r);
            w = pj.ok ? w : 0.f;
            int q = 0;
#pragma unroll
            for (int i = 0; i < 6; ++i) {
                float jw = J[ch * 6 + i] * w;
#pragma unroll
                for (int k = i; k < 6; ++k) acc[q++] += (obs_acc_t)(jw * J[ch * 6 + k]);
                acc[21 + i] += (obs_acc_t)(jw * r);
            }
        }
        acc[27] += (obs_acc_t)l; acc[28] += 1;
    };
    const int e0 = beg + cx * (kBlock * rows) + threadIdx.x;
    if constexpr (IMG >= 0 && !(PSG_STRICT & 4) && (PSG_FM_PIPE & 2)) {
        fm_for_each_obs<IMG>(b, fp, a.cam, img, e0, end, rows, [&](const ObsPend<IMG>& P) {
            const ProjJ pj = project_jac(P.pr, a.cam);
            float I[3], gu[3], gv[3];
            if (!taps_colour<IMG, true>(img, a.cam, P.ts, P.pr.m, P.pr.n, pj.mj, pj.nj, I, gu, gv)) return false;
            accumulate(P.v, P.pr, pj, I, gu, gv);
            return true;
        }, [&](const Vox& v, const Proj& pr) {
            const ProjJ pj = project_jac(pr, a.cam);
            float I[3], gu[3], gv[3];
            sample<true, IMG>(img, 0, a.cam, pr.m, pr.n, pj.mj, pj.nj, I, gu, gv);
            accumulate(v, pr, pj, I, gu, gv);
        });
    } else {
    int e = e0;
    int j_cur = e < end ? b.obs_rows[e] : -1;
    int j_nxt = (rows > 1 && e + kBlock < end) ? b.obs_rows[e + kBlock] : -1;
    Vox vn;
    if (j_cur >= 0) load_vox(b, j_cur, vn);
    for (int it = 0; it < rows && j_cur >= 0; ++it, e += kBlock) {
        const Vox v = vn;
        const int j_nn = (it + 2 < rows && e + 2 * kBlock < end) ? b.obs_rows[e + 2 * kBlock] : -1;
        if (j_nxt >= 0) load_vox(b, j_nxt, vn);
        j_cur = j_nxt; j_nxt = j_nn;
        Proj pr = project(v.xs, fp, a.cam);
        if (!pr.ok) continue;
        float I[3], gu[3], gv[3];
        const ProjJ pj = project_jac(pr, a.cam);
        sample<true, IMG>(img, 0, a.cam, pr.m, pr.n, pj.mj, pj.nj, I, gu, gv);
        accumulate(v, pr, pj, I, gu, gv);
    }
    }
    const int w = threadIdx.x >> 6;
    wave_sums_to<NV>(acc, lds + w * NV);
    __syncthreads();
    frame_rows_publish<NV, 1, MODEL>(a, cx, f, lds);
}
int launch_sweep_pose(const SweepArgs& a, hipStream_t s) {
    if (a.b.S <= 0 || a.F <= 0 || a.b.obs_max <= 0) return 0;
    const int rows = fm_rows(a, ((PSG_FM_PIPE & 2) && PSG_POSE_WAVES < 4) ? 3 : 4);
    const int chunk = kBlock * rows;
    dim3 g((a.b.obs_max + chunk - 1) / chunk, a.F), bl(kBlock);
    PSG_LAUNCH_SWEEP(k_sweep_pose, a, true, g, bl, 0, s, a, rows);
    if (a.xf && a.fm_solve) launch_frame_gather<1>(a, s);
    return (int)g.x;
}

template <int N>
__device__ void solve_spd(const double* Hin, const double* bin, double* x) {
    double L[N * N], D[N], y[N];
    double scale = 0;
    for (int i = 0; i < N; ++i) scale = fmax(scale, fabs(Hin[i * N + i]));
    const double tiny = scale * 1e-12;
    for (int i = 0; i < N * N; ++i) L[i] = 0;
    for (int j = 0; j < N; ++j) {
        double d = Hin[j * N + j];
        for (int k = 0; k < j; ++k) d -= L[j * N + k] * L[j * N + k] * D[k];
        D[j] = d; L[j * N + j] = 1.0;
        for (int i = j + 1; i < N; ++i) {
            double s = Hin[i * N + j];
            for (int k = 0; k < j; ++k) s -= L[i * N + k] * L[j * N + k] * D[k];
            L[i * N + j] = (d > tiny) ? s / d : 0.0;
        }
    }
    for (int i = 0; i < N; ++i) { double s = bin[i]; for (int k = 0; k < i; ++k) s -= L[i * N + k] * y[k]; y[i] = s; }
    for (int i = 0; i < N; ++i) y[i] = (D[i] > tiny) ? y[i] / D[i] : 0.0;
    for (int i = N - 1; i >= 0; --i) { double s = y[i]; for (int k = i + 1; k < N; ++k) s -= L[k * N + i] * x[k]; x[i] = s; }
}

__device__ __forceinline__ void frame_rows_finish(const SweepArgs& a, int col_e, double* e_out, unsigned long long e_key, double* red) {
    __syncthreads();
    if (e_out) {
        double e = 0, n = 0;
        for (int f = threadIdx.x; f < a.F; f += blockDim.x) { e += a.acc.frame[(size_t)f * kFrameRow + col_e]; n += a.acc.frame[(size_t)f * kFrameRow + col_e + 1]; }
        e = wave_sum(e); n = wave_sum(n);
        const int lane = threadIdx.x & 63, w = threadIdx.x >> 6;
        if (lane == 0) { red[2 * w] = e; red[2 * w + 1] = n; }
        __syncthreads();
        if (threadIdx.x == 0) { double te = 0, tn = 0; for (int i = 0; i < (int)(blockDim.x >> 6); ++i) { te += red[2 * i]; tn += red[2 * i + 1]; } mbox_put(e_out, 2, 0, te, e_key); mbox_put(e_out, 2, 1, tn, e_key); mbox_commit(e_key); }
        __syncthreads();
    }
}

template <int MODEL>
__global__ void __launch_bounds__(kBlock) k_solve_light(SweepArgs a, FrameP* frames, float* led_light, double* e_out, unsigned long long e_key, float* undo) {
    if (undo) {
        for (int i = threadIdx.x; i < a.F * 9; i += blockDim.x) undo[i] = frames[i / 9].l[i % 9];
        if (threadIdx.x < 3) undo[a.F * 9 + threadIdx.x] = led_light[threadIdx.x];
        __syncthreads();
    }
    constexpr int NB = ModelTraits<MODEL>::NB;
    constexpr bool LED = ModelTraits<MODEL>::LED;
    constexpr int NH = LED ? 3 : NB * (NB + 1) / 2;
    __shared__ double red[2 * kBlock / 64];
    if (LED) {
        constexpr int kStage = 512;
        __shared__ double srow[6 * kStage];
        const bool staged = a.F <= kStage;
        if (staged) {
            for (int i = threadIdx.x; i < 6 * a.F; i += blockDim.x) { const int ff = i / 6, c6 = i % 6; srow[c6 * kStage + ff] = a.acc.frame[(size_t)ff * kFrameRow + (c6 < 3 ? c6 : NH + c6 - 3)]; }
            __syncthreads();
        }
        float dl[3];
#pragma unroll
        for (int ch = 0; ch < 3; ++ch) {
            double hs = 0, bs = 0;
            if (staged) { for (int ff = 0; ff < a.F; ++ff) { hs += srow[ch * kStage + ff]; bs += srow[(3 + ch) * kStage + ff]; } }
            else for (int ff = 0; ff < a.F; ++ff) { hs += a.acc.frame[(size_t)ff * kFrameRow + ch]; bs += a.acc.frame[(size_t)ff * kFrameRow + NH + ch]; }
            float h = (float)hs, bb = (float)bs;
            if (a.damping != 0.0f) h += a.damping * h;
            double Hd[1] = {(double)h}, bd[1] = {(double)bb}, xd[1];
            solve_spd<1>(Hd, bd, xd);
            dl[ch] = (float)xd[0];
        }
        for (int f = threadIdx.x; f < a.F; f += blockDim.x) {
#pragma unroll
            for (int ch = 0; ch < 3; ++ch) { const float nl = frames[f].l[ch] - dl[ch]; frames[f].l[ch] = nl; if (f == 0) led_light[ch] = nl; }
        }
    } else {
        for (int f = threadIdx.x; f < a.F; f += blockDim.x) frame_solve_light_sh<NB>(frames, f, a.acc.frame + (size_t)f * kFrameRow, nullptr);
    }
    frame_rows_finish(a, NH + NB, e_out, e_key, red);
}
__global__ void __launch_bounds__(kBlock) k_restore_light(int F, FrameP* frames, float* led_light, const float* undo) {
    for (int i = threadIdx.x; i < F * 9; i += blockDim.x) frames[i / 9].l[i % 9] = undo[i];
    if (threadIdx.x < 3) led_light[threadIdx.x] = undo[F * 9 + threadIdx.x];
}
void launch_restore_light(int F, FrameP* frames, float* led_light, const float* undo, hipStream_t s) { if (F > 0) hipLaunchKernelGGL(k_restore_light, dim3(1), dim3(kBlock), 0, s, F, frames, led_light, undo); }
void launch_solve_light(const SweepArgs& a, FrameP* frames, float* led_light, double* e_out, unsigned long long e_key, float* undo, hipStream_t s) {
    if (a.F <= 0) return;
    dim3 g(1), bl(kBlock);
    if (a.model == 0) hipLaunchKernelGGL((k_solve_light<0>), g, bl, 0, s, a, frames, led_light, e_out, e_key, undo);
    else if (a.model == 1) hipLaunchKernelGGL((k_solve_light<1>), g, bl, 0, s, a, frames, led_light, e_out, e_key, undo);
    else hipLaunchKernelGGL((k_solve_light<2>), g, bl, 0, s, a, frames, led_light, e_out, e_key, undo);
}

__global__ void __launch_bounds__(kBlock) k_solve_pose(SweepArgs a, FrameP* frames, double* e_out, unsigned long long e_key) {
    __shared__ double red[2 * kBlock / 64];
    for (int f = threadIdx.x; f < a.F; f += blockDim.x) frame_solve_pose(a, frames, f, a.acc.frame + (size_t)f * kFrameRow);
    frame_rows_finish(a, 27, e_out, e_key, red);
}
void launch_solve_pose(const SweepArgs& a, FrameP* frames, double* e_out, unsigned long long e_key, hipStream_t s) {
    if (a.F > 0) hipLaunchKernelGGL(k_solve_pose, dim3(1), dim3(kBlock), 0, s, a, frames, e_out, e_key);
}

}
```

Measured before the change: 3183.

## Deal frame-major sweep workgroups per frame from observation counts and occupancy

Replaces the uniform 2D grid (max-observations chunks × frames) for the light and pose sweeps with a 1D grid built from a host-computed table. Each frame gets its own workgroup count and rows per workgroup, chosen from its observation count so the total fits the occupancy-derived slot budget. This removes empty or idle workgroups on frames with few observations and improves load balance. The cost is an occupancy query, a table upload and a stream sync when the band changes, one extra indirection per workgroup, and a new failure path when no table is available.

```diff
diff --git a/psgradientsdf_amd/capi.py b/psgradientsdf_amd/capi.py
--- a/psgradientsdf_amd/capi.py
+++ b/psgradientsdf_amd/capi.py
@@ -929,6 +929,21 @@
     return _engine_lib[path]
 
 
+def debug_fm_deal(counts, slots: int, fcap: int, knob_rows: int = 0):
+    n = np.ascontiguousarray(counts, dtype=np.int32)
+    F = int(n.size)
+    f = engine_lib().psgsdf_debug_fm_deal; f.restype = C.c_longlong
+    f.argtypes = [C.c_void_p, C.c_int, C.c_longlong, C.c_int, C.c_int, C.c_void_p, C.c_void_p, C.c_longlong, C.c_void_p]
+    fr = np.zeros((F, 3), np.int32); info = np.zeros(5, np.int32)
+    G = f(n.ctypes.data, F, int(slots), int(fcap), int(knob_rows), fr.ctypes.data, None, 0, info.ctypes.data)
+    if G < 0:
+        return None
+    wg = np.zeros((int(G), 2), np.int32)
+    assert f(n.ctypes.data, F, int(slots), int(fcap), int(knob_rows), fr.ctypes.data, wg.ctypes.data, int(G), info.ctypes.data) == G
+    return {"first": fr[:, 0].copy(), "k": fr[:, 1].copy(), "rows": fr[:, 2].copy(), "wg": wg, "r": int(info[0]), "slots": int(info[1]),
+            "workgroups": int(info[2]), "rows_min": int(info[3]), "rows_max": int(info[4])}
+
+
 def load_engine(sc_or_grid, K, settings: Settings, device: int = 0, dev: bool = False) -> Api:
     grid = sc_or_grid if isinstance(sc_or_grid, GridDesc) else grid_of(sc_or_grid)
     return Api(engine_lib(dev or os.environ.get("PSGSDF_USE_DEV_LIB") == "1"), "psgsdf_", grid, K, settings, device)
diff --git a/psgradientsdf_amd/csrc/api.hip b/psgradientsdf_amd/csrc/api.hip
--- a/psgradientsdf_amd/csrc/api.hip
+++ b/psgradientsdf_amd/csrc/api.hip
@@ -125,7 +125,7 @@
     free_dense(c);
     hipFree(c->vis_seq); hipFree(c->frame_idx); hipFree(c->img); hipFree(c->img8); hipFree(c->frames); hipFree(c->frames_undo); hipFree(c->led_light); hipFree(c->fs_stats);
     hipFree(c->band_mem); if (!c->leak_exported) hipFree(c->rec_mem); hipFree(c->obs_mem); hipFree(c->stage);
-    hipFree(c->ncache); hipFree(c->ntmp); hipFree(c->nout); hipFree(c->ndepth); hipFree(c->track_part); if (c->track_host) hipHostFree(c->track_host); hipFree(c->acc_frame); hipFree(c->frame_part); hipFree(c->frame_done); hipFree(c->part); hipFree(c->pcg_sc); hipFree(c->pcg_part); hipFree(c->pcg_gran); hipFree(c->win_tab); hipFree(c->d_total);
+    hipFree(c->ncache); hipFree(c->ntmp); hipFree(c->nout); hipFree(c->ndepth); hipFree(c->track_part); if (c->track_host) hipHostFree(c->track_host); hipFree(c->acc_frame); hipFree(c->frame_part); hipFree(c->frame_done); fm_plan_free(c->fm); hipFree(c->part); hipFree(c->pcg_sc); hipFree(c->pcg_part); hipFree(c->pcg_gran); hipFree(c->win_tab); hipFree(c->d_total);
     for (void* p : c->xo_host) if (p) hipHostFree(p);
     if (c->pin_stage) hipHostFree(c->pin_stage);
     if (c->host_buf) hipHostFree(c->host_buf);
diff --git a/psgradientsdf_amd/csrc/api_debug.hip b/psgradientsdf_amd/csrc/api_debug.hip
--- a/psgradientsdf_amd/csrc/api_debug.hip
+++ b/psgradientsdf_amd/csrc/api_debug.hip
@@ -204,9 +204,10 @@
     const bool led = c->set.model == PSGSDF_LED;
     int n, nb, nh;
     int launched = 0;
-    if (block == PSGSDF_LIGHT) { launched = launch_sweep_light(a, c->stream); n = led ? 3 : (c->set.model == PSGSDF_SH2 ? 9 : 4); nb = led ? 1 : c->F; nh = led ? 3 : n * (n + 1) / 2; }
-    else if (block == PSGSDF_POSE) { launched = launch_sweep_pose(a, c->stream); n = 6; nb = c->F; nh = 21; }
+    if (block == PSGSDF_LIGHT) { launched = launch_sweep_light(a, c->fm, c->stream); n = led ? 3 : (c->set.model == PSGSDF_SH2 ? 9 : 4); nb = led ? 1 : c->F; nh = led ? 3 : n * (n + 1) / 2; }
+    else if (block == PSGSDF_POSE) { launched = launch_sweep_pose(a, c->fm, c->stream); n = 6; nb = c->F; nh = 21; }
     else return fail(c, PSGSDF_ERR_ARG, "block must be LIGHT or POSE");
+    if (launched < 0) return fail(c, PSGSDF_ERR_DEVICE, "frame-major sweep: no workgroup table");
     if (!launched) HIPCHK(c, hipMemsetAsync(c->acc_frame, 0, sizeof(double) * c->acc_frame_n, c->stream));
     std::vector<double> acc(c->acc_frame_n);
     HIPCHK(c, hipMemcpyAsync(acc.data(), c->acc_frame, sizeof(double) * c->acc_frame_n, hipMemcpyDeviceToHost, c->stream));
@@ -225,6 +226,17 @@
         for (int i = 0; i < n; ++i) bk[i] = A[nh + i];
     }
     return PSGSDF_OK;
+}
+
+long long psgsdf_debug_fm_deal(const int32_t* counts, int F, long long slots, int fcap, int knob_rows, int32_t* frames_out, int32_t* wg_out, long long wg_cap, int32_t* info_out) {
+    if (!counts || !frames_out || F <= 0) return -1;
+    std::vector<FmFrame> fr((size_t)F);
+    FmDealInfo info{};
+    const long long G = fm_deal(counts, F, slots, fcap, knob_rows, fr.data(), wg_out, wg_cap, &info);
+    if (G < 0) return G;
+    for (int f = 0; f < F; ++f) { frames_out[3 * f] = fr[f].first; frames_out[3 * f + 1] = fr[f].k; frames_out[3 * f + 2] = fr[f].rows; }
+    if (info_out) { info_out[0] = info.r; info_out[1] = info.slots; info_out[2] = info.workgroups; info_out[3] = info.rows_min; info_out[4] = info.rows_max; }
+    return G;
 }
 
 int psgsdf_debug_albedo_system(psgsdf_ctx* c, float* H, float* b) {
@@ -277,6 +289,15 @@
                  (int)c->pcg_window, c->pcg_solve_rows, shape ? Gs : 0, shape ? Rs : 0, c->win_max, budget, (int)(c->pcg_window && !*why), why, c->last_solve_windowed);
         o += buf;
     }
+    {
+        const FmDeal& dl = c->fm.deal[0]; const FmDeal& dp = c->fm.deal[1];
+        const bool vl = dl.gen == c->fm.gen && dl.gen != 0, vp = dp.gen == c->fm.gen && dp.gen != 0;
+        snprintf(buf, sizeof(buf), ", \"fm_deal\": {\"num_cu\": %d, \"light\": {\"per_cu\": %d, \"slots\": %d, \"workgroups\": %d, \"rows_min\": %d, \"rows_max\": %d}, "
+                 "\"pose\": {\"per_cu\": %d, \"slots\": %d, \"workgroups\": %d, \"rows_min\": %d, \"rows_max\": %d}}", c->num_cu,
+                 vl ? dl.per_cu : 0, vl ? dl.info.slots : 0, vl ? dl.info.workgroups : 0, vl ? dl.info.rows_min : 0, vl ? dl.info.rows_max : 0,
+                 vp ? dp.per_cu : 0, vp ? dp.info.slots : 0, vp ? dp.info.workgroups : 0, vp ? dp.info.rows_min : 0, vp ? dp.info.rows_max : 0);
+        o += buf;
+    }
     o += "}";
     snprintf(buf, sizeof(buf), ", \"last_compare\": {\"queries\": [%lld, %lld], \"pairs\": [%lld, %lld]}", c->cmp_queries[0], c->cmp_queries[1], c->cmp_pairs[0], c->cmp_pairs[1]);
     o += buf;
diff --git a/psgradientsdf_amd/csrc/device_common.h b/psgradientsdf_amd/csrc/device_common.h
--- a/psgradientsdf_amd/csrc/device_common.h
+++ b/psgradientsdf_amd/csrc/device_common.h
@@ -213,12 +213,12 @@
     const unsigned x = pid & 7u, s = pid >> 3, q = G >> 3, rem = G & 7u;
     return x * q + (x < rem ? x : rem) + s;
 }
-__device__ __forceinline__ void fm_ids(const SweepArgs& a, int& cx, int& f) {
-    cx = blockIdx.x; f = blockIdx.y;
-    if (a.xcd_map & 1) {
-        const unsigned L = xcd_remap(blockIdx.x + gridDim.x * blockIdx.y, gridDim.x * gridDim.y);
-        cx = (int)(L / gridDim.y); f = (int)(L - (unsigned)cx * gridDim.y);
-    }
+__device__ __forceinline__ void fm_ids(const SweepArgs& a, int& cx, int& f, int& k, int& rows) {
+    const unsigned L = (a.xcd_map & 1) ? xcd_remap(blockIdx.x, gridDim.x) : blockIdx.x;
+    const int2 w = a.fm_wg[L];
+    f = w.x; cx = w.y;
+    const int4 e = a.fm_fr[f];
+    k = e.y; rows = e.z;
 }
 __device__ __forceinline__ unsigned xcd_remap_striped(unsigned pid, unsigned G, unsigned T) {
     const unsigned Gc = G / (8u * T) * (8u * T);
diff --git a/psgradientsdf_amd/csrc/engine.h b/psgradientsdf_amd/csrc/engine.h
--- a/psgradientsdf_amd/csrc/engine.h
+++ b/psgradientsdf_amd/csrc/engine.h
@@ -127,6 +127,8 @@
     int xcd_map;
     int fm_solve;
     FrameP* fm_frames; float* fm_undo; double* fm_e_out; unsigned long long fm_e_key;
+    const int2* fm_wg;
+    const int4* fm_fr;
     const double* gate;
     const double* ext;
 };
@@ -182,8 +184,26 @@
 void launch_sweep_albedo(const SweepArgs& a, hipStream_t s);
 void launch_apply_albedo(const SweepArgs& a, hipStream_t s);
 void launch_restore_albedo(const SweepArgs& a, hipStream_t s);
-int launch_sweep_light(const SweepArgs& a, hipStream_t s);
-int launch_sweep_pose(const SweepArgs& a, hipStream_t s);
+struct FmFrame { int first, k, rows; };
+struct FmDealInfo { int r, slots, workgroups, rows_min, rows_max; };
+constexpr int kFmRowsMin = 4, kFmRowsMax = 64;
+long long fm_deal(const int* n, int F, long long slots, int fcap, int knob_rows, FmFrame* fr, int* wg, long long wg_cap, FmDealInfo* info);
+struct FmDeal {
+    const void* fn = nullptr; int per_cu = 0;
+    unsigned gen = 0; int knob = 0, num_cu = 0;
+    FmDealInfo info{};
+    int* dev = nullptr; size_t dev_ints = 0;
+    int* host = nullptr; size_t host_ints = 0;
+};
+struct FmPlan {
+    int* n = nullptr; int F = 0;
+    int num_cu = 0, fcap = 0; unsigned gen = 0;
+    FmDeal deal[2];
+};
+void fm_plan_free(FmPlan& p);
+void fm_plan_prepare(const SweepArgs& a, FmPlan& p, hipStream_t s);
+int launch_sweep_light(const SweepArgs& a, FmPlan& p, hipStream_t s);
+int launch_sweep_pose(const SweepArgs& a, FmPlan& p, hipStream_t s);
 void launch_solve_light(const SweepArgs& a, FrameP* frames, float* led_light, double* e_out, unsigned long long e_key, float* undo, hipStream_t s);
 void launch_restore_light(int F, FrameP* frames, float* led_light, const float* undo, hipStream_t s);
 void launch_solve_pose(const SweepArgs& a, FrameP* frames, double* e_out, unsigned long long e_key, hipStream_t s);
diff --git a/psgradientsdf_amd/csrc/engine.hip b/psgradientsdf_amd/csrc/engine.hip
--- a/psgradientsdf_amd/csrc/engine.hip
+++ b/psgradientsdf_amd/csrc/engine.hip
@@ -328,6 +328,8 @@
         const int nch = (c->row1 - c->row0 + kObsChunk - 1) / kObsChunk, F = c->F;
         if (c->obs_mem) { hipFree(c->obs_mem); c->obs_mem = nullptr; }
         b.obs_ptr = nullptr; b.obs_rows = nullptr; b.obs_max = 0; b.obs_ptr_total = 0;
+        free(c->fm.n); c->fm.n = nullptr; c->fm.F = 0; ++c->fm.gen;
+        if (c->fm.gen == 0) c->fm.gen = 1;
         if (nch > 0 && F > 0) {
             int* d_counts = nullptr;
             HIPCHK(c, hipMalloc(&d_counts, sizeof(int) * (size_t)nch * F));
@@ -338,6 +340,8 @@
             int run = 0, mx = 0;
             for (int f = 0; f < F; ++f) { ptr[f] = run; for (int k = 0; k < nch; ++k) { off[(size_t)f * nch + k] = run; run += cnt[(size_t)f * nch + k]; } mx = std::max(mx, run - ptr[f]); }
             ptr[F] = run;
+            c->fm.n = (int*)malloc(sizeof(int) * (size_t)F); c->fm.F = c->fm.n ? F : 0;
+            for (int f = 0; f < c->fm.F; ++f) c->fm.n[f] = ptr[f + 1] - ptr[f];
             HIPCHK(c, hipMalloc(&c->obs_mem, sizeof(int) * ((size_t)run + F + 2)));
             b.obs_ptr = (int*)c->obs_mem; b.obs_rows = b.obs_ptr + (F + 1); b.obs_max = mx; b.obs_ptr_total = run;
             HIPCHK(c, hipMemcpyAsync(b.obs_ptr, ptr.data(), sizeof(int) * (F + 1), hipMemcpyHostToDevice, c->stream));
@@ -387,7 +391,9 @@
     {
         if (c->frame_part) { hipFree(c->frame_part); c->frame_part = nullptr; }
         if (c->frame_done) { hipFree(c->frame_done); c->frame_done = nullptr; }
-        c->frame_cap = (b.obs_max + kBlock * 4 - 1) / (kBlock * 4) + 1;
+        c->frame_cap = (b.obs_max + kBlock * kFmRowsMin - 1) / (kBlock * kFmRowsMin) + 1;
+        c->fm.fcap = c->frame_cap; c->fm.num_cu = c->num_cu;
+        if (b.obs_max > 0) fm_plan_prepare(make_args(c, 0), c->fm, c->stream);
         const int F = std::max(c->F, 1);
         HIPCHK(c, hipMalloc(&c->frame_part, sizeof(double) * (size_t)F * c->frame_cap * kFrameRow));
         HIPCHK(c, hipMalloc(&c->frame_done, sizeof(int) * (F + 1)));
diff --git a/psgradientsdf_amd/csrc/engine_internal.h b/psgradientsdf_amd/csrc/engine_internal.h
--- a/psgradientsdf_amd/csrc/engine_internal.h
+++ b/psgradientsdf_amd/csrc/engine_internal.h
@@ -82,6 +82,7 @@
     double* acc_frame = nullptr; size_t acc_frame_n = 0;
     double* frame_part = nullptr; int frame_cap = 0;
     int* frame_done = nullptr;
+    FmPlan fm;
     double* part = nullptr; int PB = 0;
     double* pcg_sc = nullptr; int pcg_cap = 4096;
     double* pcg_part = nullptr;
diff --git a/psgradientsdf_amd/csrc/loop.hip b/psgradientsdf_amd/csrc/loop.hip
--- a/psgradientsdf_amd/csrc/loop.hip
+++ b/psgradientsdf_amd/csrc/loop.hip
@@ -265,10 +265,11 @@
             }
             if (block == PSGSDF_LIGHT) {
                 take_fold(c, a, 0u);
-                timed(c, "sweep_light", [&] { launched = launch_sweep_light(a, c->stream); });
+                timed(c, "sweep_light", [&] { launched = launch_sweep_light(a, c->fm, c->stream); });
                 const int n = led ? 3 : (c->set.model == PSGSDF_SH2 ? 9 : 4), nh = led ? 3 : n * (n + 1) / 2;
                 col = nh + n;
-            } else { take_fold(c, a, 0u); timed(c, "sweep_pose", [&] { launched = launch_sweep_pose(a, c->stream); }); col = 27; }
+            } else { take_fold(c, a, 0u); timed(c, "sweep_pose", [&] { launched = launch_sweep_pose(a, c->fm, c->stream); }); col = 27; }
+            if (launched < 0) return fail(c, PSGSDF_ERR_DEVICE, "frame-major sweep: no workgroup table (occupancy query, allocation or upload failed)");
             if (fuse) {
                 if (launched) { c->fm_solved = true; return 0; }
                 c->frame_e_slot = fm_slot; c->frame_e_key = fm_key;
diff --git a/psgradientsdf_amd/csrc/sweeps.hip b/psgradientsdf_amd/csrc/sweeps.hip
--- a/psgradientsdf_amd/csrc/sweeps.hip
+++ b/psgradientsdf_amd/csrc/sweeps.hip
@@ -1,4 +1,8 @@
 #include "device_common.h"
+#include <limits.h>
+#include <stdlib.h>
+#include <algorithm>
+#include <vector>
 
 #ifndef PSG_FM_PIPE
 #define PSG_FM_PIPE 3
@@ -182,12 +186,82 @@
     if (a.row1 > a.row0) hipLaunchKernelGGL(k_apply_albedo, dim3((a.row1 - a.row0 + kBlock - 1) / kBlock), dim3(kBlock), 0, s, a);
 }
 
-static int fm_rows(const SweepArgs& a, int slots_per_cu) {
-    if (const char* e = getenv("PSGSDF_FM_ROWS")) { int v = atoi(e); if (v >= 4 && v <= 64) return v; }
-    const long long total = a.b.obs_ptr_total > 0 ? a.b.obs_ptr_total : (long long)a.b.obs_max * a.F;
-    const long long slots = 256LL * slots_per_cu;
-    long long r = (total + (long long)(0.92 * slots) * kBlock - 1) / ((long long)(0.92 * slots) * kBlock);
-    return (int)std::min<long long>(std::max<long long>(r, 4), 64);
+long long fm_deal(const int* n, int F, long long slots, int fcap, int knob_rows, FmFrame* fr, int* wg, long long wg_cap, FmDealInfo* info) {
+    if (!n || !fr || F <= 0 || fcap <= 0) return -1;
+    auto cdiv = [](long long x, long long y) { return (x + y - 1) / y; };
+    long long nmax = 0;
+    for (int f = 0; f < F; ++f) { if (n[f] < 0) return -1; nmax = std::max<long long>(nmax, n[f]); }
+    int r = kFmRowsMax;
+    if (knob_rows >= kFmRowsMin && knob_rows <= kFmRowsMax) {
+        r = knob_rows;
+        const long long k = std::max<long long>(1, cdiv(nmax, (long long)kBlock * r));
+        if (k > fcap) return -1;
+        for (int f = 0; f < F; ++f) { fr[f].k = (int)k; fr[f].rows = r; }
+    } else {
+        const long long r_cap = std::max<long long>(kFmRowsMin, cdiv(nmax, (long long)kBlock * fcap));
+        if (r_cap > kFmRowsMax) return -1;
+        for (int t = (int)r_cap; t <= kFmRowsMax; ++t) {
+            long long sum = 0;
+            for (int f = 0; f < F; ++f) sum += std::max<long long>(1, cdiv(n[f], (long long)kBlock * t));
+            if (sum <= slots) { r = t; break; }
+        }
+        for (int f = 0; f < F; ++f) {
+            const long long k = std::max<long long>(1, cdiv(n[f], (long long)kBlock * r));
+            fr[f].k = (int)k; fr[f].rows = (int)std::max<long long>(kFmRowsMin, cdiv(n[f], (long long)kBlock * k));
+        }
+    }
+    long long G = 0; int kmax = 0, rmin = kFmRowsMax, rmax = 0;
+    for (int f = 0; f < F; ++f) { G += fr[f].k; kmax = std::max(kmax, fr[f].k); rmin = std::min(rmin, fr[f].rows); rmax = std::max(rmax, fr[f].rows); }
+    if (wg) {
+        if (G > wg_cap) return -1;
+        long long q = 0;
+        for (int cx = 0; cx < kmax; ++cx)
+            for (int f = 0; f < F; ++f) if (cx < fr[f].k) { if (cx == 0) fr[f].first = (int)q; wg[2 * q] = f; wg[2 * q + 1] = cx; ++q; }
+    } else for (int f = 0; f < F; ++f) fr[f].first = f;
+    if (info) { info->r = r; info->slots = (int)std::min<long long>(slots, INT_MAX); info->workgroups = (int)std::min<long long>(G, INT_MAX); info->rows_min = rmin; info->rows_max = rmax; }
+    return G;
+}
+void fm_plan_free(FmPlan& p) {
+    for (FmDeal& d : p.deal) { if (d.dev) hipFree(d.dev); free(d.host); d = FmDeal{}; }
+    free(p.n); p.n = nullptr; p.F = 0;
+}
+static int fm_prepare(FmPlan& p, int kind, const void* fn, int F, hipStream_t s) {
+    FmDeal& d = p.deal[kind];
+    if (!p.n || p.F != F || p.gen == 0) return -1;
+    int knob = 0;
+    if (const char* e = getenv("PSGSDF_FM_ROWS")) { const int v = atoi(e); if (v >= kFmRowsMin && v <= kFmRowsMax) knob = v; }
+    if (d.fn != fn) {
+        int per_cu = 0;
+        if (hipOccupancyMaxActiveBlocksPerMultiprocessor(&per_cu, fn, kBlock, 0) != hipSuccess || per_cu <= 0) return -1;
+        d.fn = fn; d.per_cu = per_cu; d.gen = 0;
+    }
+    if (d.gen == p.gen && d.knob == knob && d.num_cu == p.num_cu) return d.info.workgroups;
+    const long long slots = (long long)std::max(p.num_cu, 0) * d.per_cu;
+    std::vector<FmFrame> fr((size_t)F);
+    FmDealInfo info{};
+    const long long G = fm_deal(p.n, F, slots, p.fcap, knob, fr.data(), nullptr, 0, &info);
+    if (G <= 0 || G > INT_MAX / 4) return -1;
+    const size_t ints = 2 * (size_t)G + 4 * (size_t)F;
+    if (ints > d.host_ints) { free(d.host); d.host = (int*)malloc(sizeof(int) * ints); d.host_ints = d.host ? ints : 0; if (!d.host) return -1; }
+    if (ints > d.dev_ints) { if (d.dev) hipFree(d.dev); d.dev = nullptr; d.dev_ints = 0; if (hipMalloc(&d.dev, sizeof(int) * ints) != hipSuccess) return -1; d.dev_ints = ints; }
+    if (fm_deal(p.n, F, slots, p.fcap, knob, fr.data(), d.host + 4 * (size_t)F, G, &info) != G) return -1;
+    for (int f = 0; f < F; ++f) { int* e = d.host + 4 * (size_t)f; e[0] = fr[f].first; e[1] = fr[f].k; e[2] = fr[f].rows; e[3] = 0; }
+    if (hipMemcpyAsync(d.dev, d.host, sizeof(int) * ints, hipMemcpyHostToDevice, s) != hipSuccess || hipStreamSynchronize(s) != hipSuccess) return -1;
+    d.info = info; d.gen = p.gen; d.knob = knob; d.num_cu = p.num_cu;
+    return (int)G;
+}
+typedef void (*FmKernel)(SweepArgs);
+#define PSG_FM_INSTANCE(K, args) \
+    (((args).rob.loss == 1 && !(args).im.u8) ? ((args).model == 0 ? (FmKernel)K<0, 1, 0> : (args).model == 1 ? (FmKernel)K<1, 1, 0> : (FmKernel)K<2, 1, 0>) \
+     : ((args).rob.loss == 1) ? ((args).model == 0 ? (FmKernel)K<0, 1, 1> : (args).model == 1 ? (FmKernel)K<1, 1, 1> : (FmKernel)K<2, 1, 1>) \
+     : ((args).model == 0 ? (FmKernel)K<0, -1, -1> : (args).model == 1 ? (FmKernel)K<1, -1, -1> : (FmKernel)K<2, -1, -1>))
+static int fm_launch(FmKernel fn, int kind, const SweepArgs& a0, FmPlan& p, hipStream_t s) {
+    const int G = fm_prepare(p, kind, (const void*)fn, a0.F, s);
+    if (G <= 0) return -1;
+    SweepArgs a = a0;
+    a.fm_fr = (const int4*)p.deal[kind].dev; a.fm_wg = (const int2*)(p.deal[kind].dev + 4 * (size_t)a.F);
+    hipLaunchKernelGGL(fn, dim3((unsigned)G), dim3(kBlock), 0, s, a);
+    return G;
 }
 
 template <int N> __device__ void solve_spd(const double* Hin, const double* bin, double* x);
@@ -272,7 +346,7 @@
 }
 
 template <int NV, int KIND, int MODEL>
-__device__ __forceinline__ void frame_rows_publish(const SweepArgs& a, int cx, int f, double* lds ) {
+__device__ __forceinline__ void frame_rows_publish(const SweepArgs& a, int cx, int f, int kf , double* lds ) {
     __shared__ int s_last;
     double* dst = a.acc.fpart + ((size_t)f * a.acc.fcap + cx) * kFrameRow;
     if (threadIdx.x < NV) {
@@ -282,7 +356,7 @@
     }
     if (threadIdx.x < 64) {
         asm volatile("s_waitcnt vmcnt(0)" ::: "memory");
-        if (threadIdx.x == 0) s_last = __hip_atomic_fetch_add(a.acc.fdone + f, 1, __ATOMIC_RELAXED, __HIP_MEMORY_SCOPE_AGENT) == (int)gridDim.x - 1;
+        if (threadIdx.x == 0) s_last = __hip_atomic_fetch_add(a.acc.fdone + f, 1, __ATOMIC_RELAXED, __HIP_MEMORY_SCOPE_AGENT) == kf - 1;
     }
     __syncthreads();
     if (!s_last) return;
@@ -291,10 +365,10 @@
     if (threadIdx.x < NV) {
         const double* p = a.acc.fpart + (size_t)f * a.acc.fcap * kFrameRow + threadIdx.x;
         double s = 0;
-        for (int c = 0; c < (int)gridDim.x; c += 16) {
+        for (int c = 0; c < kf; c += 16) {
             double v[16];
 #pragma unroll
-            for (int j = 0; j < 16; ++j) v[j] = c + j < (int)gridDim.x ? __hip_atomic_load(p + (size_t)(c + j) * kFrameRow, __ATOMIC_RELAXED, __HIP_MEMORY_SCOPE_AGENT) : 0.0;
+            for (int j = 0; j < 16; ++j) v[j] = c + j < kf ? __hip_atomic_load(p + (size_t)(c + j) * kFrameRow, __ATOMIC_RELAXED, __HIP_MEMORY_SCOPE_AGENT) : 0.0;
 #pragma unroll
             for (int j = 0; j < 16; ++j) s += v[j];
         }
@@ -318,7 +392,7 @@
     }
     if (threadIdx.x < 64) {
         asm volatile("s_waitcnt vmcnt(0)" ::: "memory");
-        if (threadIdx.x == 0) s_last = __hip_atomic_fetch_add(a.acc.fdone + a.F, 1, __ATOMIC_RELAXED, __HIP_MEMORY_SCOPE_AGENT) == (int)gridDim.y - 1;
+        if (threadIdx.x == 0) s_last = __hip_atomic_fetch_add(a.acc.fdone + a.F, 1, __ATOMIC_RELAXED, __HIP_MEMORY_SCOPE_AGENT) == a.F - 1;
     }
     __syncthreads();
     if (!s_last) return;
@@ -390,7 +464,7 @@
 }
 
 template <int MODEL, int LOSS, int IMG>
-__global__ void __launch_bounds__(kBlock) k_sweep_light(SweepArgs a, int rows) {
+__global__ void __launch_bounds__(kBlock) k_sweep_light(SweepArgs a) {
     { __shared__ double fred[kBlock / 64]; fold_pending(a, fred); }
     constexpr int NB = ModelTraits<MODEL>::NB;
     constexpr bool LED = ModelTraits<MODEL>::LED;
@@ -398,7 +472,7 @@
     constexpr int NV = NH + NB + 2;
     __shared__ FrameP sfp;
     __shared__ double lds[(kBlock / 64) * NV];
-    int cx, f; fm_ids(a, cx, f);
+    int cx, f, kf, rows; fm_ids(a, cx, f, kf, rows);
     if (threadIdx.x < (int)(sizeof(FrameP) / 4)) ((float*)&sfp)[threadIdx.x] = ((const float*)(a.frames + f))[threadIdx.x];
     __syncthreads();
     const Band& b = a.b;
@@ -487,27 +561,25 @@
     const int w = threadIdx.x >> 6;
     wave_sums_to<NV>(acc, lds + w * NV);
     __syncthreads();
-    frame_rows_publish<NV, 0, MODEL>(a, cx, f, lds);
-}
-int launch_sweep_light(const SweepArgs& a, hipStream_t s) {
+    frame_rows_publish<NV, 0, MODEL>(a, cx, f, kf, lds);
+}
+int launch_sweep_light(const SweepArgs& a, FmPlan& p, hipStream_t s) {
     if (a.b.S <= 0 || a.F <= 0 || a.b.obs_max <= 0) return 0;
-    const int rows = fm_rows(a, a.model == 1 ? 3 : ((PSG_FM_PIPE & 1) ? 4 : 5));
-    const int chunk = kBlock * rows;
-    dim3 g((a.b.obs_max + chunk - 1) / chunk, a.F), bl(kBlock);
-    PSG_LAUNCH_SWEEP(k_sweep_light, a, true, g, bl, 0, s, a, rows);
+    const int G = fm_launch(PSG_FM_INSTANCE(k_sweep_light, a), 0, a, p, s);
+    if (G <= 0) return G;
     if (a.xf && a.fm_solve) launch_frame_gather<0>(a, s);
-    return (int)g.x;
+    return G;
 }
 
 template <int MODEL, int LOSS, int IMG>
-__global__ void __launch_bounds__(kBlock, PSG_POSE_WAVES) k_sweep_pose(SweepArgs a, int rows) {
+__global__ void __launch_bounds__(kBlock, PSG_POSE_WAVES) k_sweep_pose(SweepArgs a) {
     { __shared__ double fred[kBlock / 64]; fold_pending(a, fred); }
     constexpr int NB = ModelTraits<MODEL>::NB;
     constexpr bool LED = ModelTraits<MODEL>::LED;
     constexpr int NV = 21 + 6 + 2;
     __shared__ FrameP sfp;
     __shared__ double lds[(kBlock / 64) * NV];
-    int cx, f; fm_ids(a, cx, f);
+    int cx, f, kf, rows; fm_ids(a, cx, f, kf, rows);
     if (threadIdx.x < (int)(sizeof(FrameP) / 4)) ((float*)&sfp)[threadIdx.x] = ((const float*)(a.frames + f))[threadIdx.x];
     __syncthreads();
     const Band& b = a.b;
@@ -650,16 +722,19 @@
     const int w = threadIdx.x >> 6;
     wave_sums_to<NV>(acc, lds + w * NV);
     __syncthreads();
-    frame_rows_publish<NV, 1, MODEL>(a, cx, f, lds);
-}
-int launch_sweep_pose(const SweepArgs& a, hipStream_t s) {
+    frame_rows_publish<NV, 1, MODEL>(a, cx, f, kf, lds);
+}
+void fm_plan_prepare(const SweepArgs& a, FmPlan& p, hipStream_t s) {
+    if (a.b.S <= 0 || a.F <= 0 || a.b.obs_max <= 0) return;
+    fm_prepare(p, 0, (const void*)PSG_FM_INSTANCE(k_sweep_light, a), a.F, s);
+    fm_prepare(p, 1, (const void*)PSG_FM_INSTANCE(k_sweep_pose, a), a.F, s);
+}
+int launch_sweep_pose(const SweepArgs& a, FmPlan& p, hipStream_t s) {
     if (a.b.S <= 0 || a.F <= 0 || a.b.obs_max <= 0) return 0;
-    const int rows = fm_rows(a, ((PSG_FM_PIPE & 2) && PSG_POSE_WAVES < 4) ? 3 : 4);
-    const int chunk = kBlock * rows;
-    dim3 g((a.b.obs_max + chunk - 1) / chunk, a.F), bl(kBlock);
-    PSG_LAUNCH_SWEEP(k_sweep_pose, a, true, g, bl, 0, s, a, rows);
+    const int G = fm_launch(PSG_FM_INSTANCE(k_sweep_pose, a), 1, a, p, s);
+    if (G <= 0) return G;
     if (a.xf && a.fm_solve) launch_frame_gather<1>(a, s);
-    return (int)g.x;
+    return G;
 }
 
 template <int N>
```

New measurement: 3189, median of 3. Within noise of the previous version (+0.2%).
